# whwu95/MVFNet

Hardware: AMD Instinct MI355X
Metric: clips/sec (fwd+bwd) MVFNet-R50 8x8 224^2 (higher is better)
Workload: dtype bf16; 1 GPU; MVFNet-ResNet50 8x8, 32 clips/GPU of 8x3x224x224, bf16, train step: fwd (batch-stat BN) + loss + bwd + clip + SGD-nesterov; all through the HIP C ABI (stem + 16 bottlenecks + MVF + TSN head); clips_per_gpu=32, frames_per_clip=8, parallelism=dp1: replicas, one flat gradient all-reduce per step

## Files before the change

include/mvfnet_hip.h:

```cpp
#ifndef MVFNET_HIP_H
#define MVFNET_HIP_H

#include <stddef.h>
#include <stdint.h>

#ifdef __cplusplus
extern "C" {
#endif

#define MVF_ABI_VERSION 2

enum { MVF_OK = 0, MVF_EINVAL = -1, MVF_ESHAPE = -2, MVF_EWS = -3, MVF_EHIP = -4, MVF_EUNSUPPORTED = -5 };
enum { MVF_F32 = 0, MVF_BF16 = 1 };
enum { MVF_NCHW = 0, MVF_NHWC = 1 };
enum { MVF_VIEW_T = 1, MVF_VIEW_H = 2, MVF_VIEW_W = 4 };

int mvf_abi_version(void);
const char* mvf_last_error(void);

typedef struct {
    int32_t nt, c, h, w;
    int32_t n_segment;
    int32_t cs;
    int32_t mode;
// ... 54 lines not shown
                                   size_t ws_bytes, void* stream);
int mvf_conv2d_nhwc_fwd_bnbwd_apply(const mvf_conv_desc_t* d, const void* x, const void* x2, const void* w_packed, const void* g,
                                    const unsigned char* sign_bits, const float* bn_gamma, const float* bn_mean, const float* bn_invstd,
                                    const float* dgamma, const float* dbeta, void* dz, void* ws, size_t ws_bytes, void* stream);
int mvf_conv2d_nhwc_fwd_resmask(const mvf_conv_desc_t* d, const void* x, const void* x2, const void* w_packed,
                                const float* bias, const void* residual, const unsigned char* res_sign_bits, void* y,
                                void* ws, size_t ws_bytes, void* stream);
int mvf_conv2d_nhwc_fwd_resmask_gate(const mvf_conv_desc_t* d, const void* x, const void* x2, const void* w_packed, const float* bias,
                                     const void* residual, const unsigned char* res_sign_bits, const unsigned char* out_gate_bits, void* y,
                                     void* ws, size_t ws_bytes, void* stream);
int mvf_conv2d_nhwc_fwd_resmask_gate_colsums(const mvf_conv_desc_t* d, const void* x, const void* x2, const void* w_packed, const void* residual,
                                             const unsigned char* res_sign_bits, const unsigned char* out_gate_bits, void* y, float* sums_part, void* ws,
                                             size_t ws_bytes, void* stream);
int mvf_conv2d_nhwc_dgrad_bnsums(const mvf_conv_desc_t* d, const void* dz, const void* w_packed_dgrad, void* y, const void* bn_z,
                                 const float* bn_mean, const float* bn_invstd, const float* bn_scale, const float* bn_shift,
                                 float* sums_part, void* ws, size_t ws_bytes, void* stream);
int mvf_bn_bwd_finalize(const float* sums_part, int nblk, int c, float* dgamma, float* dbeta, void* stream);
int mvf_conv2d_stats_rows(const mvf_conv_desc_t* d);
int mvf_conv2d_nhwc_fwd_stats(const mvf_conv_desc_t* d, const void* x, const void* x2, const void* w_packed, void* y,
                              float* stats_part, const float* stats_shift, void* ws, size_t ws_bytes, void* stream);

enum {
    MVF_CONV_FAM_NONE = 0,
    MVF_CONV_FAM_REG = 1,
    MVF_CONV_FAM_X3 = 2,
    MVF_CONV_FAM_LDS_DMA = 3,
    MVF_CONV_FAM_T256_2B = 4,
    MVF_CONV_FAM_T256_P4 = 5,
    MVF_CONV_FAM_DBUF = 6,
    MVF_CONV_FAM_DBUF_PF2 = 7,
    MVF_CONV_FAM_STREAMK = 8,
    MVF_CONV_FAM_GENERIC = 9,
    MVF_CONV_FAM_MVF_LOADER = 10,
    MVF_CONV_FAM_STEM_DIRECT = 11,
    MVF_CONV_FAM_PW_SUMS = 12,
    MVF_CONV_FAM_C3X3_C64 = 13
};
typedef struct {
    int32_t family;
    int32_t epi_asked;
    int32_t epi_run;
    int32_t pointwise;
    int32_t buffers;
    int32_t tile_m, tile_n;
    int32_t dtype;
    int32_t k_chunks;
    int32_t half_k;
    int32_t launches;
} mvf_conv_launch_info_t;
int mvf_conv2d_last_launch(mvf_conv_launch_info_t* out);

int mvf_pack_conv_weight(const float* w_oihw, int cout, int cin, int kh, int kw, int kw_pad, int cin_pad,
                         const float* scale, void* w_packed, int dtype, void* stream);
int mvf_bn_fold(const float* gamma, const float* beta, const float* mean, const float* var, float eps, int c,
                float* scale, float* shift, void* stream);

int mvf_stem_prep(const float* x_nchw, int n, int c, int h, int w, int pad, int wp, void* out, int dtype, void* stream);

int mvf_frames_prep_u8(const unsigned char* frames_hwc, int n, int hs, int ws, const int* window, int h, int w,
                       const float* mean3, const float* std3, int to_rgb, int div_255, int pad, int wp, void* out_stem,
                       float* out_nchw, int dtype, void* stream);
int mvf_frames_resample_u8(const unsigned char* frames_hwc, int n, int hs, int ws, const int* rows, int h, int w,
                           const float* mean3, const float* std3, int to_rgb, int div_255, int pad, int wp, void* out_stem,
                           float* out_nchw, int dtype, void* stream);
int mvf_frames_resample_color_u8(const unsigned char* frames_hwc, int n, int hs, int ws, const int* rows, const float* color, int h, int w,
                                 const float* mean3, const float* std3, int to_rgb, int div_255, int pad, int wp, void* out_stem,
                                 float* out_nchw, int dtype, void* stream);
int mvf_frames_gather_resample_u8(const unsigned char* frames_hwc, int n_src, int hs, int ws, const int* src_index, int n_out, const int* rows,
                                  const float* color, int h, int w, const float* mean3, const float* std3, int to_rgb, int div_255, int pad,
                                  int wp, void* out_stem, float* out_nchw, int dtype, void* stream);
int mvf_frames_yuv420_gather_resample_u8(const unsigned char* frames, int n_src, int hs, int ws, int pitch, int layout, int standard, int order,
                                         const int* src_index, int n_out, const int* rows, const float* color, int h, int w, const float* mean3,
                                         const float* std3, int to_rgb, int div_255, int pad, int wp, void* out_stem, float* out_nchw, int dtype,
                                         void* stream);
int mvf_frames_addressed_resample_u8(const unsigned char* frames, long long frames_bytes, int format, int standard, int order,
                                     int n_out, const int* rows, const int* addr, const float* color, int h, int w,
                                     const float* mean3, const float* std3, int to_rgb, int div_255, int pad, int wp,
                                     void* out_stem, float* out_nchw, int dtype, void* stream);

int mvf_maxpool3x3s2_nhwc(const void* x, int n, int h, int w, int c, void* y, int dtype, void* stream);

int mvf_head_pool_fc(const void* feat, int clips, int t, int hw, int c, const float* fc_w, const float* fc_b,
                     int classes, float* pooled_ws, float* scores, int dtype, void* stream);
int mvf_average_clip(const float* scores, int clips, int classes, int kind, float* out, void* stream);

int mvf_conv2d_nhwc_dgrad_bnsums_split(const mvf_conv_desc_t* d, const void* x, const void* x2, const void* w_packed, const float* bias, void* y,
                                       const void* bn_z, const float* bn_mean, const float* bn_invstd, const float* bn_scale, const float* bn_shift,
                                       float* sums_part, void* ws, size_t ws_bytes, void* stream);
int mvf_bn_bwd_dzfree_prep(const void* w_packed_dgrad, int c, int k, const float* gamma, const float* mean, const float* invstd, const float* dgamma,
                           const float* dbeta, long m, void* w_out, float* bias_out, int dtype, void* stream);
int mvf_bn_bwd_dzfree_wgrad(float* dw, const void* w_packed, const float* gram, const float* a_mean, const float* gamma, const float* mean,
                            const float* invstd, const float* dgamma, const float* dbeta, long m, int c, int k, int dtype, void* stream);
int mvf_bn_bwd_dzfree_sums(const float* q, const void* w_packed, int c, int k, const float* mean, const float* invstd, const float* part_lo, int rows_lo,
                           int c_split, const float* part_hi, int rows_hi, float* dgamma, float* dbeta, int dtype, void* stream);
size_t mvf_bn_workspace_bytes(long m, int c);
int mvf_bn_train_stats(const void* z, long m, int c, const float* gamma, const float* beta, float eps, float momentum,
                       float* running_mean, float* running_var, float* save_mean, float* save_invstd, float* scale,
                       float* shift, void* ws, size_t ws_bytes, int dtype, void* stream);
int mvf_bn_train_finalize(const float* part, int nblk, long m, int c, const float* gamma, const float* beta, float eps,
                          float momentum, float* running_mean, float* running_var, float* save_mean, float* save_invstd,
                          float* scale, float* shift, void* stream);
int mvf_bn_train_stats_gram(const float* gram, const float* a_mean, const void* w_packed, long m, int c, int k, const float* gamma, const float* beta,
                            float eps, float momentum, float* running_mean, float* running_var, float* save_mean, float* save_invstd, float* scale,
                            float* shift, int dtype, void* stream);
int mvf_bn_apply_colmeans(const void* z, long m, int c, const float* scale, const float* shift, int act, void* out, float* mean_out, void* ws,
                          size_t ws_bytes, int dtype, void* stream);
int mvf_bn_apply(const void* z, long m, int c, const float* scale, const float* shift, const void* residual,
                 const float* rscale, const float* rshift, int act, void* out, int dtype, void* stream);
int mvf_bn_bwd_reduce(const void* g, int g_pitch, const void* z, const void* ymask, long m, int c, const float* mean,
                      const float* invstd, const float* scale, const float* shift, int mask_mode, void* gm_out,
                      float* dgamma, float* dbeta, void* ws, size_t ws_bytes, int dtype, void* stream);
int mvf_bn_bwd_apply(const void* g, int g_pitch, const void* z, long m, int c, const float* gamma, const float* mean,
                     const float* invstd, const float* scale, const float* shift, const float* dgamma,
                     const float* dbeta, int mask_mode, void* dz, int dtype, void* stream);
int mvf_bn_apply_bits(const void* z, long m, int c, const float* scale, const float* shift, const void* residual,
                      const float* rscale, const float* rshift, int relu, void* out, unsigned char* sign_bits, int dtype,
                      void* stream);
int mvf_bn_bwd_apply_masked(const void* g, int g_pitch, const void* z, const void* ymask, long m, int c, const float* gamma,
                            const float* mean, const float* invstd, const float* scale, const float* shift,
                            const float* dgamma, const float* dbeta, int mask_mode, void* dz, int dtype, void* stream);
int mvf_bn_bwd_pair(const void* g, int g_pitch, const void* z_a, const void* z_b, const unsigned char* sign_bits, long m, int c,
                    const float* gamma_a, const float* mean_a, const float* invstd_a, float* dgamma_a, float* dbeta_a,
                    const float* gamma_b, const float* mean_b, const float* invstd_b, float* dgamma_b, float* dbeta_b,
                    void* dz_a, void* dz_b, void* ws, size_t ws_bytes, int dtype, void* stream);
int mvf_bn_bwd_wgrad_splits(long m, int c, int k, int nbn, int mask_mode);
size_t mvf_bn_bwd_wgrad_slab_bytes(long m, int c, int k, int nbn, int mask_mode);
int mvf_bn_bwd_apply_wgrad(const void* g, int g_pitch, const void* z, const void* ymask, long m, int c, const float* gamma, const float* mean,
                           const float* invstd, const float* scale, const float* shift, const float* dgamma, const float* dbeta, int mask_mode,
                           void* dz, const void* x, int x_pitch, int k, float* slabs, size_t slab_bytes, int dtype, void* stream);
int mvf_bn_bwd_pair_wgrad(const void* g, int g_pitch, const void* z_a, const void* z_b, const unsigned char* sign_bits, long m, int c,
                          const float* gamma_a, const float* mean_a, const float* invstd_a, float* dgamma_a, float* dbeta_a,
                          const float* gamma_b, const float* mean_b, const float* invstd_b, float* dgamma_b, float* dbeta_b,
                          void* dz_a, void* dz_b, const void* x_a, int xa_pitch, const void* x_b, int xb_pitch, int k,
                          float* slabs_a, float* slabs_b, size_t slab_bytes, void* ws, size_t ws_bytes, int dtype, void* stream);
int mvf_conv1x1_bwd_fused_splits(long m, int c, int k);
int mvf_conv1x1_bwd_fused(const void* a_in, int a_pitch, const void* w_packed, const void* g, int g_pitch, const unsigned char* sign_bits, long m, int c,
                          int k, const float* gamma, const float* mean, const float* invstd, const float* dgamma, const float* dbeta, const void* z_in,
                          const float* in_mean, const float* in_invstd, const float* in_scale, const float* in_shift, void* dx, float* sums_part,
                          int sums_rows, float* slabs, size_t slab_bytes, int dtype, void* stream);
int mvf_conv1x1_bnbwd_sums_pair(const void* a_in, int a_pitch, const void* w_a, const void* x_in, int x_pitch, const void* w_b, const void* g, int g_pitch,
                                const unsigned char* sign_bits, long m, int c, int k, const float* mean_a, const float* invstd_a, const float* mean_b,
                                const float* invstd_b, float* part_a, float* part_b, int rows, int dtype, void* stream);
int mvf_wgrad_slab_reduce(const float* slabs, int nsplit, int cout, int k, float* dw_oihw, void* stream);
int mvf_maxpool_bn_relu_fwd(const void* z, int n, int h, int w, int c, const float* scale, const float* shift, void* y,
                            unsigned char* argmax, int dtype, void* stream);
int mvf_maxpool_bn_relu_bwd(const unsigned char* argmax, const void* g, int n, int h, int w, int c, void* ga, int dtype,
                            void* stream);
int mvf_maxpool_bwd_sums_rows(int n, int h);
int mvf_maxpool_bn_relu_bwd_apply(const unsigned char* argmax, const void* g, int n, int h, int w, int c, const void* z, const float* gamma,
                                  const float* mean, const float* invstd, const float* scale, const float* shift, const float* dgamma,
                                  const float* dbeta, void* dz, int dtype, void* stream);
int mvf_maxpool_bn_relu_bwd_sums(const unsigned char* argmax, const void* g, int n, int h, int w, int c, void* ga, const void* z, const float* mean,
                                 const float* invstd, const float* scale, const float* shift, float* sums_part, int dtype, void* stream);
int mvf_head_train_fwd(const void* feat, int clips, int t, int hw, int c, const float* fc_w, const float* fc_b, int classes,
                       const long long* labels, const float* drop_mask ,
                       float* pooled, float* scores, float* dscores, float* loss_part, float* loss, int dtype, void* stream);
int mvf_ce_loss(const float* scores, const long long* labels, int clips, int classes, float* dscores, float* loss_part, float* loss,
                void* stream);
int mvf_head_train_bwd(const float* dscores, const float* pooled, const float* fc_w, const float* drop_mask, int clips, int t,
                       int hw, int c, int classes, float* dfc_w, float* dfc_b, float* dpool_ws , void* dfeat, int dtype,
                       void* stream);
int mvf_stem_blend(const void* xp, int clips, int t, int hp, int wp, int pad, const int* rows, const float* wts, void* out, int dtype, void* stream);
int mvf_soft_targets(const long long* labels, const int* rows, const float* wts, int clips, int classes, float eps, float* targets, void* stream);
int mvf_ce_loss_soft(const float* scores, const float* targets, int clips, int classes, float* dscores, float* loss_part, float* loss, void* stream);
int mvf_head_train_fwd_soft(const void* feat, int clips, int t, int hw, int c, const float* fc_w, const float* fc_b, int classes,
                            const float* targets, const float* drop_mask ,
                            float* pooled, float* scores, float* dscores, float* loss_part, float* loss, int dtype, void* stream);
int mvf_distill_loss(const float* scores, const float* teacher_scores, int clips, int classes, float temperature, float alpha,
                     float* dscores , float* loss_part , float* loss , float* terms ,
                     void* stream);
int mvf_stem_erase(void* xp, int planes, int hp, int wp, int pad, const int* boxes, int max_boxes, const float* fill, const unsigned int* key, int dtype,
                   void* stream);
#define MVF_RANDAUG_WS_PER_FRAME (3 * 256 + 16)
int mvf_frames_randaug_u8(const unsigned char* frames_hwc, int n, int hs, int ws, int t, int order, const int* sizes, const int* table, int layers,
                          unsigned stats_layers, unsigned char* out, unsigned char* tmp, void* workspace, long long workspace_bytes, void* stream);
size_t mvf_conv2d_wgrad_workspace_bytes(const mvf_conv_desc_t* d);
int mvf_conv2d_nhwc_wgrad(const mvf_conv_desc_t* d, const void* dz, const void* x, const void* x2, int kw_real,
                          int cin_real, int kw_packed, int cin_packed, float* dw_oihw, void* ws, size_t ws_bytes,
                          void* stream);
int mvf_conv2d_nhwc_wgrad_wgs(const mvf_conv_desc_t* d, const void* dz, const void* x, const void* x2, int kw_real,
                              int cin_real, int kw_packed, int cin_packed, float* dw_oihw, void* ws, size_t ws_bytes, int wgs, void* stream);
enum {
    MVF_WGRAD_FAM_NONE = 0,
    MVF_WGRAD_FAM_F32_REG = 1,
    MVF_WGRAD_FAM_F32_DMA = 2,
    MVF_WGRAD_FAM_X3 = 3,
    MVF_WGRAD_FAM_BF16_WIDEN = 4,
    MVF_WGRAD_FAM_BF16_REG = 5,
    MVF_WGRAD_FAM_BF16_DMA2 = 6,
    MVF_WGRAD_FAM_BF16_PIPE = 7,
    MVF_WGRAD_FAM_T256_2B = 8,
    MVF_WGRAD_FAM_T256_P4 = 9,
    MVF_WGRAD_FAM_C3X3_C64 = 10,
    MVF_WGRAD_FAM_STEM = 11
};
typedef struct {
    int32_t family;
    int32_t stages;
    int32_t tile_co, tile_k;
    int32_t dtype;
    int32_t nsplit;
    int32_t rows_per_split;
    int32_t xcd_rr;
    int32_t split_operand;
    int32_t gram;
    int32_t wgs_target;
    int32_t launches;
} mvf_wgrad_launch_info_t;
int mvf_conv2d_wgrad_last_launch(mvf_wgrad_launch_info_t* out);
typedef struct {
    const float* w;
    void* out;
    int cout, cin, kh, kw, kw_pad, cin_pad;
    int kind, first_block;
} mvf_pack_job_t;
int mvf_pack_conv_weights_batched(const mvf_pack_job_t* jobs_dev, int njobs, int total_blocks, int dtype, void* stream);

int mvf_pack_conv_weight_dgrad(const float* w_oihw, int cout, int cin, int kh, int kw, void* w_packed, int dtype,
                               void* stream);
int mvf_nhwc_stencil(const mvf_desc_t* d, const void* x, int x_c, void* out, int out_c, const float* w_t,
                     const float* w_h, const float* w_w, const float* scale, const float* shift, int flip,
                     const void* addend, int addend_c, const unsigned char* addend_sign_bits, void* stream);
int mvf_nhwc_stencil_gate(const mvf_desc_t* d, const void* x, int x_c, void* out, int out_c, const float* w_t,
                          const float* w_h, const float* w_w, const float* scale, const float* shift, int flip,
                          const void* addend, int addend_c, const unsigned char* addend_sign_bits,
                          const unsigned char* out_gate_bits, void* stream);
int mvf_nhwc_stencil_gate_colsums(const mvf_desc_t* d, const void* x, int x_c, void* out, int out_c, const float* w_t, const float* w_h,
                                  const float* w_w, int flip, const void* addend, int addend_c, const unsigned char* addend_sign_bits,
                                  const unsigned char* out_gate_bits, float* sums_part, void* stream);
int mvf_nhwc_stencil_stats_rows(const mvf_desc_t* d, int x_c, int out_c);
int mvf_nhwc_stencil_tile_plan(const mvf_desc_t* d, int x_c, int out_c, int* rows_per_band, int* chan_per_wg);
int mvf_nhwc_stencil_stats(const mvf_desc_t* d, const void* x, int x_c, void* out, int out_c, const float* w_t, const float* w_h,
                           const float* w_w, float* stats_part, const float* stats_shift, void* stream);
size_t mvf_nhwc_tapgrad_workspace_bytes(const mvf_desc_t* d);
int mvf_nhwc_tapgrad(const mvf_desc_t* d, const void* x, int x_c, const void* dy, int dy_c, float* dw_t, float* dw_h,
                     float* dw_w, void* ws, size_t ws_bytes, void* stream);
size_t mvf_sgd_workspace_bytes(long n);
int mvf_sgd_nesterov_step(float* params, const float* grads, float* momentum_buf, long n, float grad_scale, float max_norm,
                          float lr, float momentum, float weight_decay, int first_step, float* norm_out, void* ws,
                          size_t ws_bytes, void* stream);
typedef struct mvf_sgd_segment {
    long long first;
    float lr_mult, decay_mult;
} mvf_sgd_segment_t;
int mvf_sgd_step_segments(float* params, const float* grads, float* momentum_buf, long n, float grad_scale, float max_norm, float lr,
                          float momentum, float weight_decay, int first_step, int nesterov, const mvf_sgd_segment_t* segments, int nseg,
                          float* norm_out, void* ws, size_t ws_bytes, void* stream);
int mvf_grad_accumulate(float* acc, const float* g, long n, int first, void* stream);
int mvf_sgd_nesterov_step_ema(float* params, const float* grads, float* momentum_buf, long n, float grad_scale, float max_norm, float lr, float momentum,
                              float weight_decay, int first_step, float* ema, float ema_momentum, float* norm_out, void* ws, size_t ws_bytes, void* stream);
int mvf_sgd_step_segments_ema(float* params, const float* grads, float* momentum_buf, long n, float grad_scale, float max_norm, float lr, float momentum,
                              float weight_decay, int first_step, int nesterov, const mvf_sgd_segment_t* segments, int nseg, float* ema, float ema_momentum,
                              float* norm_out, void* ws, size_t ws_bytes, void* stream);
int mvf_ema_update(float* ema, const float* params, long n, float momentum, void* stream);
int mvf_ema_swap(float* a, float* b, long n, void* stream);
typedef struct mvf_stat_segment {
    float* ptr;
    long first;
} mvf_stat_segment_t;
int mvf_bn_stats_accumulate(const mvf_stat_segment_t* seg, int nseg, long n, double* acc, void* stream);
int mvf_bn_stats_finalize(const mvf_stat_segment_t* seg, int nseg, long n, const double* acc, long count, float* dst_flat_or_null, void* stream);
int mvf_bn_stats_exchange(const mvf_stat_segment_t* seg, int nseg, long n, float* flat, int mode, void* stream);
int mvf_sgd_step_guarded(float* params, const float* grads, float* momentum_buf, long n, float grad_scale, float max_norm, float lr, float momentum,
                         float weight_decay, int first_step, int nesterov, const mvf_sgd_segment_t* segments, int nseg, float* ema, float ema_momentum,
                         int* guard, float* norm_out, void* ws, size_t ws_bytes, void* stream);
int mvf_bn_stats_snapshot(const mvf_stat_segment_t* seg, int nseg, long n, float* flat, const long long* counters, long ncount, long long* counters_copy,
                          void* stream);
int mvf_bn_stats_restore(const mvf_stat_segment_t* seg, int nseg, long n, const float* flat, long long* counters, long ncount,
                         const long long* counters_copy, const int* guard, void* stream);
typedef struct mvf_adamw_hyper {
    double lr, beta1, beta2, eps, weight_decay;
    int decoupled;
} mvf_adamw_hyper_t;
size_t mvf_adamw_workspace_bytes(long n);
int mvf_adamw_step(float* params, const float* grads, float* exp_avg, float* exp_avg_sq, long n, float grad_scale, float max_norm,
                   const mvf_adamw_hyper_t* hyper, const mvf_sgd_segment_t* segments, int nseg, float* ema, float ema_momentum, int* guard,
                   long long* applied_steps, float* norm_out, void* ws, size_t ws_bytes, void* stream);
enum { MVF_METRICS_ROWS = 0, MVF_METRICS_BAD_LABEL = 1, MVF_METRICS_NAN_ROWS = 2, MVF_METRICS_HITS = 8, MVF_METRICS_MAX_K = 8, MVF_METRICS_CONFUSION = 16 };
size_t mvf_metrics_state_words(int classes, int with_confusion);
int mvf_metrics_update(const float* scores, int rows, int classes, const long long* labels, const int* ks, int nk, long long* state, int with_confusion,
                       int* rank_out, int* pred_out, void* stream);
typedef struct mvf_flat_stats {
    double sumsq;
    double absmax;
    long long n_nan;
    long long n_inf;
} mvf_flat_stats_t;
size_t mvf_flat_stats_workspace_bytes(long n, int nseg);
int mvf_flat_segment_stats(const float* x, const float* y_or_null, long n, const long long* first, int nseg, mvf_flat_stats_t* out, const int* guard_or_null,
                           long long* step_out_or_null, void* ws, size_t ws_bytes, void* stream);
int mvf_bn_stats_nonfinite(const mvf_stat_segment_t* seg, int nseg, long n, long long* counts, const int* guard_or_null, void* stream);

enum { MVF_PLAN_CALL = 0, MVF_PLAN_RECORD = 1, MVF_PLAN_WAIT = 2 };
typedef struct mvf_plan_op {
    int kind, n_int, n_flt, reserved;
    void* fn;
    long long word0, float0;
} mvf_plan_op_t;
int mvf_plan_run(const mvf_plan_op_t* ops, int n_ops, const unsigned long long* words, const float* floats, int* failed_op);

#ifdef __cplusplus
}
#endif
#endif
```

mvfnet_amd/_lib.py:

```python
import ctypes as C
import os

import torch

_HERE = os.path.dirname(os.path.abspath(__file__))
LIB_PATH = os.environ.get("MVF_LIB_PATH") or os.path.join(_HERE, "libmvfnet_hip.so")

MVF_F32, MVF_BF16 = 0, 1
MVF_NCHW, MVF_NHWC = 0, 1
VIEW_T, VIEW_H, VIEW_W = 1, 2, 4
MODE_BITS = {"T": 1, "TH": 3, "THW": 7}
METRICS_ROWS, METRICS_BAD_LABEL, METRICS_NAN_ROWS, METRICS_HITS, METRICS_MAX_K, METRICS_CONFUSION = 0, 1, 2, 8, 8, 16
ERRNAMES = {-1: "MVF_EINVAL", -2: "MVF_ESHAPE", -3: "MVF_EWS", -4: "MVF_EHIP", -5: "MVF_EUNSUPPORTED"}


class MvfDesc(C.Structure):
    _fields_ = [("nt", C.c_int32), ("c", C.c_int32), ("h", C.c_int32), ("w", C.c_int32), ("n_segment", C.c_int32),
                ("cs", C.c_int32), ("mode", C.c_int32), ("layout", C.c_int32), ("dtype", C.c_int32)]


class ConvDesc(C.Structure):
    _fields_ = [("n", C.c_int32), ("h", C.c_int32), ("w", C.c_int32), ("cin", C.c_int32), ("cout", C.c_int32),
                ("kh", C.c_int32), ("kw", C.c_int32), ("stride", C.c_int32), ("pad", C.c_int32),
                ("ho", C.c_int32), ("wo", C.c_int32), ("x_pix_stride", C.c_int32),
# ... 28 lines not shown

class PlanOp(C.Structure):
    _fields_ = [("kind", C.c_int32), ("n_int", C.c_int32), ("n_flt", C.c_int32), ("reserved", C.c_int32), ("fn", C.c_void_p), ("word0", C.c_longlong),
                ("float0", C.c_longlong)]


class SgdSegment(C.Structure):
    _fields_ = [("first", C.c_int64), ("lr_mult", C.c_float), ("decay_mult", C.c_float)]


class AdamwHyper(C.Structure):
    _fields_ = [("lr", C.c_double), ("beta1", C.c_double), ("beta2", C.c_double), ("eps", C.c_double), ("weight_decay", C.c_double), ("decoupled", C.c_int32)]


class StatSegment(C.Structure):
    _fields_ = [("ptr", C.c_void_p), ("first", C.c_long)]


def _load():
    if not os.path.exists(LIB_PATH):
        raise ImportError(
            "mvfnet_amd: %s not found. Build it with `python -m mvfnet_amd.build` (needs hipcc, "
            "--offload-arch=gfx950). There is no CPU or PyTorch fallback for the hot path." % LIB_PATH)
    lib = C.CDLL(LIB_PATH)
    vp, fp, sz, i32, f32 = C.c_void_p, C.c_void_p, C.c_size_t, C.c_int, C.c_float
    dp = C.POINTER(MvfDesc)
    lib.mvf_abi_version.restype = i32
    lib.mvf_abi_version.argtypes = []
    lib.mvf_last_error.restype = C.c_char_p
    lib.mvf_last_error.argtypes = []
    lib.mvf_fwd_infer.restype = i32
    lib.mvf_fwd_infer.argtypes = [dp, vp, vp, fp, fp, fp, fp, fp, vp]
    lib.mvf_fwd_train_workspace_bytes.restype = sz
    lib.mvf_fwd_train_workspace_bytes.argtypes = [dp]
    lib.mvf_fwd_train.restype = i32
    lib.mvf_fwd_train.argtypes = [dp, vp, vp, fp, fp, fp, fp, fp, f32, f32, fp, fp, fp, fp, vp, sz, vp]
    lib.mvf_bwd_workspace_bytes.restype = sz
    lib.mvf_bwd_workspace_bytes.argtypes = [dp]
    lib.mvf_bwd.restype = i32
    lib.mvf_bwd.argtypes = [dp, vp, vp, fp, fp, fp, fp, fp, fp, fp, i32, vp, fp, fp, fp, fp, fp, vp, sz, vp]
    lib.mvf_fwd_infer_slice.restype = i32
    lib.mvf_fwd_infer_slice.argtypes = [dp, vp, vp, fp, fp, fp, fp, fp, vp]
    cp = C.POINTER(ConvDesc)
    lib.mvf_conv2d_nhwc_fwd.restype = i32
    lib.mvf_conv2d_nhwc_fwd.argtypes = [cp, vp, vp, vp, fp, vp, vp, vp]
    lib.mvf_conv2d_workspace_bytes.restype = sz
    lib.mvf_conv2d_workspace_bytes.argtypes = [cp]
    lib.mvf_conv2d_nhwc_fwd_ws.restype = i32
    lib.mvf_conv2d_nhwc_fwd_ws.argtypes = [cp, vp, vp, vp, fp, vp, vp, vp, sz, vp]
    lib.mvf_conv2d_nhwc_dgrad_bnsums.restype = i32
    lib.mvf_conv2d_nhwc_dgrad_bnsums.argtypes = [cp, vp, vp, vp, vp, fp, fp, fp, fp, fp, vp, sz, vp]
    lib.mvf_bn_bwd_finalize.restype = i32
    lib.mvf_bn_bwd_finalize.argtypes = [fp, i32, i32, fp, fp, vp]
    lib.mvf_conv2d_nhwc_fwd_bnapply.restype = i32
    lib.mvf_conv2d_nhwc_fwd_bnapply.argtypes = [cp, vp, vp, vp, fp, fp, vp, fp, fp, vp, vp, vp, sz, vp]
    lib.mvf_conv2d_nhwc_fwd_bnbwd_sums.restype = i32
    lib.mvf_conv2d_nhwc_fwd_bnbwd_sums.argtypes = [cp, vp, vp, vp, vp, vp, fp, fp, fp, vp, sz, vp]
    lib.mvf_conv2d_nhwc_fwd_bnbwd_apply.restype = i32
    lib.mvf_conv2d_nhwc_fwd_bnbwd_apply.argtypes = [cp, vp, vp, vp, vp, vp, fp, fp, fp, fp, fp, vp, vp, sz, vp]
    lib.mvf_conv2d_nhwc_fwd_resmask.restype = i32
    lib.mvf_conv2d_nhwc_fwd_resmask.argtypes = [cp, vp, vp, vp, fp, vp, vp, vp, vp, sz, vp]
    i64_ = C.c_long
    lib.mvf_conv2d_nhwc_fwd_resmask_gate.restype = i32
    lib.mvf_conv2d_nhwc_fwd_resmask_gate.argtypes = [cp, vp, vp, vp, fp, vp, vp, vp, vp, vp, sz, vp]
    lib.mvf_conv2d_nhwc_fwd_resmask_gate_colsums.restype = i32
    lib.mvf_conv2d_nhwc_fwd_resmask_gate_colsums.argtypes = [cp, vp, vp, vp, vp, vp, vp, vp, fp, vp, sz, vp]
    lib.mvf_nhwc_stencil_gate_colsums.restype = i32
    lib.mvf_nhwc_stencil_gate_colsums.argtypes = [dp, vp, i32, vp, i32, fp, fp, fp, i32, vp, i32, vp, vp, fp, vp]
    lib.mvf_conv2d_nhwc_dgrad_bnsums_split.restype = i32
    lib.mvf_conv2d_nhwc_dgrad_bnsums_split.argtypes = [cp, vp, vp, vp, fp, vp, vp, fp, fp, fp, fp, fp, vp, sz, vp]
    lib.mvf_bn_bwd_dzfree_prep.restype = i32
    lib.mvf_bn_bwd_dzfree_prep.argtypes = [vp, i32, i32, fp, fp, fp, fp, fp, i64_, vp, fp, i32, vp]
    lib.mvf_bn_bwd_dzfree_wgrad.restype = i32
    lib.mvf_bn_bwd_dzfree_wgrad.argtypes = [fp, vp, fp, fp, fp, fp, fp, fp, fp, i64_, i32, i32, i32, vp]
    lib.mvf_bn_bwd_dzfree_sums.restype = i32
    lib.mvf_bn_bwd_dzfree_sums.argtypes = [fp, vp, i32, i32, fp, fp, fp, i32, i32, fp, i32, fp, fp, i32, vp]
    lib.mvf_nhwc_stencil_stats_rows.restype = i32
    lib.mvf_nhwc_stencil_stats_rows.argtypes = [dp, i32, i32]
    lib.mvf_nhwc_stencil_tile_plan.restype = i32
    lib.mvf_nhwc_stencil_tile_plan.argtypes = [dp, i32, i32, C.POINTER(C.c_int), C.POINTER(C.c_int)]
    lib.mvf_nhwc_stencil_stats.restype = i32
    lib.mvf_nhwc_stencil_stats.argtypes = [dp, vp, i32, vp, i32, fp, fp, fp, fp, fp, vp]
    lib.mvf_nhwc_stencil_gate.restype = i32
    lib.mvf_nhwc_stencil_gate.argtypes = [dp, vp, i32, vp, i32, fp, fp, fp, fp, fp, i32, vp, i32, vp, vp, vp]
    lib.mvf_conv2d_stats_rows.restype = i32
    lib.mvf_conv2d_stats_rows.argtypes = [cp]
    lib.mvf_conv2d_nhwc_fwd_stats.restype = i32
    lib.mvf_conv2d_nhwc_fwd_stats.argtypes = [cp, vp, vp, vp, vp, fp, fp, vp, sz, vp]
    lib.mvf_conv2d_last_launch.restype = i32
    lib.mvf_conv2d_last_launch.argtypes = [C.POINTER(ConvLaunchInfo)]
    lib.mvf_pack_conv_weight.restype = i32
    lib.mvf_pack_conv_weight.argtypes = [fp, i32, i32, i32, i32, i32, i32, fp, vp, i32, vp]
    lib.mvf_pack_conv_weights_batched.restype = i32
    lib.mvf_pack_conv_weights_batched.argtypes = [vp, i32, i32, i32, vp]
    lib.mvf_bn_fold.restype = i32
    lib.mvf_bn_fold.argtypes = [fp, fp, fp, fp, f32, i32, fp, fp, vp]
    lib.mvf_stem_prep.restype = i32
    lib.mvf_stem_prep.argtypes = [fp, i32, i32, i32, i32, i32, i32, vp, i32, vp]
    lib.mvf_frames_prep_u8.restype = i32
    lib.mvf_frames_prep_u8.argtypes = [vp, i32, i32, i32, vp, i32, i32, C.POINTER(C.c_float), C.POINTER(C.c_float),
                                       i32, i32, i32, i32, vp, vp, i32, vp]
    lib.mvf_frames_resample_u8.restype = i32
    lib.mvf_frames_resample_u8.argtypes = [vp, i32, i32, i32, vp, i32, i32, C.POINTER(C.c_float), C.POINTER(C.c_float),
                                           i32, i32, i32, i32, vp, vp, i32, vp]
    lib.mvf_frames_resample_color_u8.restype = i32
    lib.mvf_frames_resample_color_u8.argtypes = [vp, i32, i32, i32, vp, vp, i32, i32, C.POINTER(C.c_float), C.POINTER(C.c_float),
                                                 i32, i32, i32, i32, vp, vp, i32, vp]
    lib.mvf_frames_gather_resample_u8.restype = i32
    lib.mvf_frames_gather_resample_u8.argtypes = [vp, i32, i32, i32, vp, i32, vp, vp, i32, i32, C.POINTER(C.c_float), C.POINTER(C.c_float),
                                                  i32, i32, i32, i32, vp, vp, i32, vp]
    lib.mvf_frames_yuv420_gather_resample_u8.restype = i32
    lib.mvf_frames_yuv420_gather_resample_u8.argtypes = [vp, i32, i32, i32, i32, i32, i32, i32, vp, i32, vp, vp, i32, i32, C.POINTER(C.c_float),
                                                         C.POINTER(C.c_float), i32, i32, i32, i32, vp, vp, i32, vp]
    lib.mvf_frames_addressed_resample_u8.restype = i32
    lib.mvf_frames_addressed_resample_u8.argtypes = [vp, C.c_longlong, i32, i32, i32, i32, vp, vp, vp, i32, i32, C.POINTER(C.c_float), C.POINTER(C.c_float),
                                                     i32, i32, i32, i32, vp, vp, i32, vp]
    lib.mvf_maxpool3x3s2_nhwc.restype = i32
    lib.mvf_maxpool3x3s2_nhwc.argtypes = [vp, i32, i32, i32, i32, vp, i32, vp]
    lib.mvf_head_pool_fc.restype = i32
    lib.mvf_head_pool_fc.argtypes = [vp, i32, i32, i32, i32, fp, fp, i32, fp, fp, i32, vp]
    lib.mvf_average_clip.restype = i32
    lib.mvf_average_clip.argtypes = [fp, i32, i32, i32, fp, vp]
    i64, ll = C.c_long, C.c_void_p
    lib.mvf_bn_workspace_bytes.restype = sz
    lib.mvf_bn_workspace_bytes.argtypes = [i64, i32]
    lib.mvf_bn_train_stats.restype = i32
    lib.mvf_bn_train_stats.argtypes = [vp, i64, i32, fp, fp, f32, f32, fp, fp, fp, fp, fp, fp, vp, sz, i32, vp]
    lib.mvf_bn_train_finalize.restype = i32
    lib.mvf_bn_train_finalize.argtypes = [fp, i32, i64, i32, fp, fp, f32, f32, fp, fp, fp, fp, fp, fp, vp]
    lib.mvf_bn_train_stats_gram.restype = i32
    lib.mvf_bn_train_stats_gram.argtypes = [fp, fp, vp, i64, i32, i32, fp, fp, f32, f32, fp, fp, fp, fp, fp, fp, i32, vp]
    lib.mvf_bn_apply_colmeans.restype = i32
    lib.mvf_bn_apply_colmeans.argtypes = [vp, i64, i32, fp, fp, i32, vp, fp, vp, sz, i32, vp]
    lib.mvf_bn_apply.restype = i32
    lib.mvf_bn_apply.argtypes = [vp, i64, i32, fp, fp, vp, fp, fp, i32, vp, i32, vp]
    lib.mvf_bn_apply_bits.restype = i32
    lib.mvf_bn_apply_bits.argtypes = [vp, i64, i32, fp, fp, vp, fp, fp, i32, vp, vp, i32, vp]
    lib.mvf_bn_bwd_apply_masked.restype = i32
    lib.mvf_bn_bwd_apply_masked.argtypes = [vp, i32, vp, vp, i64, i32, fp, fp, fp, fp, fp, fp, fp, i32, vp, i32, vp]
    lib.mvf_bn_bwd_reduce.restype = i32
    lib.mvf_bn_bwd_reduce.argtypes = [vp, i32, vp, vp, i64, i32, fp, fp, fp, fp, i32, vp, fp, fp, vp, sz, i32, vp]
    lib.mvf_bn_bwd_apply.restype = i32
    lib.mvf_bn_bwd_apply.argtypes = [vp, i32, vp, i64, i32, fp, fp, fp, fp, fp, fp, fp, i32, vp, i32, vp]
    lib.mvf_maxpool_bn_relu_fwd.restype = i32
    lib.mvf_maxpool_bn_relu_fwd.argtypes = [vp, i32, i32, i32, i32, fp, fp, vp, vp, i32, vp]
    lib.mvf_maxpool_bn_relu_bwd.restype = i32
    lib.mvf_maxpool_bn_relu_bwd.argtypes = [vp, vp, i32, i32, i32, i32, vp, i32, vp]
    lib.mvf_maxpool_bwd_sums_rows.restype = i32
    lib.mvf_maxpool_bwd_sums_rows.argtypes = [i32, i32]
    lib.mvf_maxpool_bn_relu_bwd_apply.restype = i32
    lib.mvf_maxpool_bn_relu_bwd_apply.argtypes = [vp, vp, i32, i32, i32, i32, vp, fp, fp, fp, fp, fp, fp, fp, vp, i32, vp]
    lib.mvf_maxpool_bn_relu_bwd_sums.restype = i32
    lib.mvf_maxpool_bn_relu_bwd_sums.argtypes = [vp, vp, i32, i32, i32, i32, vp, vp, fp, fp, fp, fp, fp, i32, vp]
    lib.mvf_head_train_fwd.restype = i32
    lib.mvf_head_train_fwd.argtypes = [vp, i32, i32, i32, i32, fp, fp, i32, ll, fp, fp, fp, fp, fp, fp, i32, vp]
    lib.mvf_conv2d_nhwc_fwd_mvf.restype = i32
    lib.mvf_conv2d_nhwc_fwd_mvf.argtypes = [cp, vp, vp, fp, fp, i32, i32, i32, vp, vp, sz, vp]
    lib.mvf_bn_bwd_pair.restype = i32
    lib.mvf_bn_bwd_pair.argtypes = [vp, i32, vp, vp, vp, i64, i32, fp, fp, fp, fp, fp, fp, fp, fp, fp, fp, vp, vp, vp, sz, i32, vp]
    lib.mvf_bn_bwd_wgrad_splits.restype = i32
    lib.mvf_bn_bwd_wgrad_splits.argtypes = [i64, i32, i32, i32, i32]
    lib.mvf_bn_bwd_wgrad_slab_bytes.restype = sz
    lib.mvf_bn_bwd_wgrad_slab_bytes.argtypes = [i64, i32, i32, i32, i32]
    lib.mvf_bn_bwd_apply_wgrad.restype = i32
    lib.mvf_bn_bwd_apply_wgrad.argtypes = [vp, i32, vp, vp, i64, i32, fp, fp, fp, fp, fp, fp, fp, i32, vp, vp, i32, i32, fp, sz, i32, vp]
    lib.mvf_bn_bwd_pair_wgrad.restype = i32
    lib.mvf_bn_bwd_pair_wgrad.argtypes = [vp, i32, vp, vp, vp, i64, i32, fp, fp, fp, fp, fp, fp, fp, fp, fp, fp, vp, vp, vp, i32, vp, i32, i32,
                                          fp, fp, sz, vp, sz, i32, vp]
    lib.mvf_conv1x1_bwd_fused_splits.restype = i32
    lib.mvf_conv1x1_bwd_fused_splits.argtypes = [i64, i32, i32]
    lib.mvf_conv1x1_bwd_fused.restype = i32
    lib.mvf_conv1x1_bwd_fused.argtypes = [vp, i32, vp, vp, i32, vp, i64, i32, i32, fp, fp, fp, fp, fp, vp, fp, fp, fp, fp, vp, fp, i32, fp, sz, i32, vp]
    lib.mvf_conv1x1_bnbwd_sums_pair.restype = i32
    lib.mvf_conv1x1_bnbwd_sums_pair.argtypes = [vp, i32, vp, vp, i32, vp, vp, i32, vp, i64, i32, i32, fp, fp, fp, fp, fp, fp, i32, i32, vp]
    lib.mvf_wgrad_slab_reduce.restype = i32
    lib.mvf_wgrad_slab_reduce.argtypes = [fp, i32, i32, i32, fp, vp]
    lib.mvf_ce_loss.restype = i32
    lib.mvf_ce_loss.argtypes = [fp, ll, i32, i32, fp, fp, fp, vp]
    lib.mvf_stem_blend.restype = i32
    lib.mvf_stem_blend.argtypes = [vp, i32, i32, i32, i32, i32, vp, fp, vp, i32, vp]
    lib.mvf_stem_erase.restype = i32
    lib.mvf_stem_erase.argtypes = [vp, i32, i32, i32, i32, vp, i32, fp, vp, i32, vp]
    lib.mvf_frames_randaug_u8.restype = i32
    lib.mvf_frames_randaug_u8.argtypes = [vp, i32, i32, i32, i32, i32, vp, vp, i32, C.c_uint, vp, vp, vp, C.c_longlong, vp]
    lib.mvf_soft_targets.restype = i32
    lib.mvf_soft_targets.argtypes = [ll, vp, fp, i32, i32, f32, fp, vp]
    lib.mvf_ce_loss_soft.restype = i32
    lib.mvf_ce_loss_soft.argtypes = [fp, fp, i32, i32, fp, fp, fp, vp]
    lib.mvf_head_train_fwd_soft.restype = i32
    lib.mvf_head_train_fwd_soft.argtypes = [vp, i32, i32, i32, i32, fp, fp, i32, fp, fp, fp, fp, fp, fp, fp, i32, vp]
    lib.mvf_distill_loss.restype = i32
    lib.mvf_distill_loss.argtypes = [fp, fp, i32, i32, f32, f32, fp, fp, fp, fp, vp]
    lib.mvf_head_train_bwd.restype = i32
    lib.mvf_head_train_bwd.argtypes = [fp, fp, fp, fp, i32, i32, i32, i32, i32, fp, fp, fp, vp, i32, vp]
    lib.mvf_conv2d_wgrad_workspace_bytes.restype = sz
    lib.mvf_conv2d_wgrad_workspace_bytes.argtypes = [cp]
    lib.mvf_conv2d_nhwc_wgrad.restype = i32
    lib.mvf_conv2d_nhwc_wgrad.argtypes = [cp, vp, vp, vp, i32, i32, i32, i32, fp, vp, sz, vp]
    lib.mvf_conv2d_nhwc_wgrad_wgs.restype = i32
    lib.mvf_conv2d_nhwc_wgrad_wgs.argtypes = [cp, vp, vp, vp, i32, i32, i32, i32, fp, vp, sz, i32, vp]
    lib.mvf_conv2d_wgrad_last_launch.restype = i32
    lib.mvf_conv2d_wgrad_last_launch.argtypes = [C.POINTER(WgradLaunchInfo)]
    lib.mvf_pack_conv_weight_dgrad.restype = i32
    lib.mvf_pack_conv_weight_dgrad.argtypes = [fp, i32, i32, i32, i32, vp, i32, vp]
    lib.mvf_nhwc_stencil.restype = i32
    lib.mvf_nhwc_stencil.argtypes = [dp, vp, i32, vp, i32, fp, fp, fp, fp, fp, i32, vp, i32, vp, vp]
    lib.mvf_nhwc_tapgrad_workspace_bytes.restype = sz
    lib.mvf_nhwc_tapgrad_workspace_bytes.argtypes = [dp]
    lib.mvf_nhwc_tapgrad.restype = i32
    lib.mvf_nhwc_tapgrad.argtypes = [dp, vp, i32, vp, i32, fp, fp, fp, vp, sz, vp]
    lib.mvf_sgd_workspace_bytes.restype = sz
    lib.mvf_sgd_workspace_bytes.argtypes = [i64]
    lib.mvf_sgd_nesterov_step.restype = i32
    lib.mvf_sgd_nesterov_step.argtypes = [fp, fp, fp, i64, f32, f32, f32, f32, f32, i32, fp, vp, sz, vp]
    lib.mvf_sgd_step_segments.restype = i32
    lib.mvf_sgd_step_segments.argtypes = [fp, fp, fp, i64, f32, f32, f32, f32, f32, i32, i32, vp, i32, fp, vp, sz, vp]
    lib.mvf_grad_accumulate.restype = i32
    lib.mvf_grad_accumulate.argtypes = [fp, fp, i64, i32, vp]
    lib.mvf_sgd_nesterov_step_ema.restype = i32
    lib.mvf_sgd_nesterov_step_ema.argtypes = [fp, fp, fp, i64, f32, f32, f32, f32, f32, i32, fp, f32, fp, vp, sz, vp]
    lib.mvf_sgd_step_segments_ema.restype = i32
    lib.mvf_sgd_step_segments_ema.argtypes = [fp, fp, fp, i64, f32, f32, f32, f32, f32, i32, i32, vp, i32, fp, f32, fp, vp, sz, vp]
    lib.mvf_ema_update.restype = i32
    lib.mvf_ema_update.argtypes = [fp, fp, i64, f32, vp]
    lib.mvf_ema_swap.restype = i32
    lib.mvf_ema_swap.argtypes = [fp, fp, i64, vp]
    lib.mvf_bn_stats_accumulate.restype = i32
    lib.mvf_bn_stats_accumulate.argtypes = [vp, i32, i64, vp, vp]
    lib.mvf_bn_stats_finalize.restype = i32
    lib.mvf_bn_stats_finalize.argtypes = [vp, i32, i64, vp, i64, fp, vp]
    lib.mvf_bn_stats_exchange.restype = i32
    lib.mvf_bn_stats_exchange.argtypes = [vp, i32, i64, fp, i32, vp]
    lib.mvf_sgd_step_guarded.restype = i32
    lib.mvf_sgd_step_guarded.argtypes = [fp, fp, fp, i64, f32, f32, f32, f32, f32, i32, i32, vp, i32, fp, f32, vp, fp, vp, sz, vp]
    lib.mvf_bn_stats_snapshot.restype = i32
    lib.mvf_bn_stats_snapshot.argtypes = [vp, i32, i64, fp, vp, i64, vp, vp]
    lib.mvf_bn_stats_restore.restype = i32
    lib.mvf_bn_stats_restore.argtypes = [vp, i32, i64, fp, vp, i64, vp, vp, vp]
    lib.mvf_adamw_workspace_bytes.restype = sz
    lib.mvf_adamw_workspace_bytes.argtypes = [i64]
    lib.mvf_adamw_step.restype = i32
    lib.mvf_adamw_step.argtypes = [fp, fp, fp, fp, i64, f32, f32, C.POINTER(AdamwHyper), vp, i32, fp, f32, vp, vp, fp, vp, sz, vp]
    lib.mvf_metrics_state_words.restype = sz
    lib.mvf_metrics_state_words.argtypes = [i32, i32]
    lib.mvf_metrics_update.restype = i32
    lib.mvf_metrics_update.argtypes = [fp, i32, i32, ll, vp, i32, ll, i32, vp, vp, vp]
    lib.mvf_flat_stats_workspace_bytes.restype = sz
    lib.mvf_flat_stats_workspace_bytes.argtypes = [i64, i32]
    lib.mvf_flat_segment_stats.restype = i32
    lib.mvf_flat_segment_stats.argtypes = [fp, fp, i64, vp, i32, vp, vp, vp, vp, sz, vp]
    lib.mvf_bn_stats_nonfinite.restype = i32
    lib.mvf_bn_stats_nonfinite.argtypes = [vp, i32, i64, vp, vp, vp]
    lib.mvf_plan_run.restype = i32
    lib.mvf_plan_run.argtypes = [C.POINTER(PlanOp), i32, C.POINTER(C.c_ulonglong), C.POINTER(C.c_float), C.POINTER(C.c_int)]
    missing = [n for n in declared_symbols() if hasattr(lib, n) and getattr(lib, n).argtypes is None]
    if missing:
        raise ImportError("mvfnet_amd._lib: no argtypes declared for %s" % missing)
    return lib


def check(rc, what=""):
    if rc != 0:
        msg = lib.mvf_last_error().decode("utf-8", "replace")
        raise RuntimeError("%s failed: %s (%s)" % (what or "libmvfnet_hip", ERRNAMES.get(rc, rc), msg))


def declared_symbols():
    import re
    hdr = os.path.join(os.path.dirname(_HERE), "include", "mvfnet_hip.h")
    txt = open(hdr).read()
    txt = re.sub(r"/\*.*?\*/", "", txt, flags=re.S)
    return sorted(set(re.findall(r"\b((?:mvf|mvfnet)_[a-z0-9_]+)\s*\(", txt)))


lib = _load()
```

mvfnet_amd/csrc/common.h:

```cpp
#pragma once
#include <hip/hip_runtime.h>
#include <stdlib.h>
#include <string.h>
#include <strings.h>
#include <stdint.h>
#include <stdio.h>

#include "mvfnet_hip.h"

void mvf_set_error(const char* fmt, ...);

#define MVF_HIP_OK(call)                                                                        \
    do {                                                                                        \
        hipError_t e__ = (call);                                                                \
        if (e__ != hipSuccess) {                                                                \
            mvf_set_error("%s:%d: %s -> %s", __FILE__, __LINE__, #call, hipGetErrorString(e__)); \
            return MVF_EHIP;                                                                    \
        }                                                                                       \
    } while (0)

#define MVF_REQUIRE(cond, code, ...)    \
    do {                                \
        if (!(cond)) {                  \
            mvf_set_error(__VA_ARGS__); \
            return (code);              \
        }                               \
    } while (0)

#define MVF_LAUNCH_CHECK()                                                              \
    do {                                                                                \
        hipError_t e__ = hipGetLastError();                                             \
        if (e__ != hipSuccess) {                                                        \
            mvf_set_error("%s:%d: launch -> %s", __FILE__, __LINE__, hipGetErrorString(e__)); \
            return MVF_EHIP;                                                            \
        }                                                                               \
    } while (0)

struct bf16_t {
    uint16_t v;
};

__device__ __forceinline__ float bf16_to_f32(uint16_t v) { return __uint_as_float(((uint32_t)v) << 16); }
typedef __bf16 mvf_bf16x2 __attribute__((ext_vector_type(2)));
typedef float mvf_f32x2 __attribute__((ext_vector_type(2)));
__device__ __forceinline__ uint32_t pack_bf16x2(float lo, float hi) {
    const mvf_f32x2 v = {lo, hi};
    const mvf_bf16x2 b = __builtin_convertvector(v, mvf_bf16x2);
    uint32_t u;
    __builtin_memcpy(&u, &b, 4);
    return u;
}
__device__ __forceinline__ uint16_t f32_to_bf16(float f) { return (uint16_t)(pack_bf16x2(f, 0.f) & 0xffffu); }

__device__ __forceinline__ float ldf(const float* p) { return *p; }
__device__ __forceinline__ float ldf(const bf16_t* p) { return bf16_to_f32(p->v); }
__device__ __forceinline__ void stf(float* p, float v) { *p = v; }
__device__ __forceinline__ void stf(bf16_t* p, float v) { p->v = f32_to_bf16(v); }

__device__ __forceinline__ float4 ld4(const float* p) { return *reinterpret_cast<const float4*>(p); }
__device__ __forceinline__ float4 ld4(const bf16_t* p) {
    uint2 r = *reinterpret_cast<const uint2*>(p);
    return make_float4(__uint_as_float(r.x << 16), __uint_as_float(r.x & 0xffff0000u),
                       __uint_as_float(r.y << 16), __uint_as_float(r.y & 0xffff0000u));
}
__device__ __forceinline__ void st4(float* p, float4 v) { *reinterpret_cast<float4*>(p) = v; }
__device__ __forceinline__ void st4(bf16_t* p, float4 v) {
    uint2 r;
    r.x = pack_bf16x2(v.x, v.y);
    r.y = pack_bf16x2(v.z, v.w);
    *reinterpret_cast<uint2*>(p) = r;
}

__device__ __forceinline__ float ema_step(float e, float p, float m) { return m >= 1.0f ? p : fmaf(m, p - e, e); }

__device__ __forceinline__ float hswish_f(float u) { return u * fminf(fmaxf(u + 3.0f, 0.0f), 6.0f) * (1.0f / 6.0f); }
__device__ __forceinline__ float hswish_grad_f(float u) {
    float r6 = fminf(fmaxf(u + 3.0f, 0.0f), 6.0f);
    float inner = (u > -3.0f && u < 3.0f) ? 1.0f : 0.0f;
    return r6 * (1.0f / 6.0f) + u * inner * (1.0f / 6.0f);
}

static inline size_t align_up(size_t v, size_t a) { return (v + a - 1) / a * a; }

static inline bool mvf_policy_lookup(const char* name, long* out) {
    const char* p = getenv("MVF_POLICY");
    if (!p) return false;
    const size_t n = strlen(name);
    while (*p) {
        while (*p == ',' || *p == ';' || *p == ' ') ++p;
        const char* e = p;
        while (*e && *e != ',' && *e != ';') ++e;
        const char* eq = (const char*)memchr(p, '=', (size_t)(e - p));
        if (eq && (size_t)(eq - p) == n && strncasecmp(p, name, n) == 0) {
            *out = strtol(eq + 1, nullptr, 10);
            return true;
        }
        p = e;
    }
    return false;
}
static inline int mvf_policy_int(const char* name, int dflt) {
    long v;
    return mvf_policy_lookup(name, &v) ? (int)v : dflt;
}
static inline bool mvf_policy_has(const char* name) {
    long v;
    return mvf_policy_lookup(name, &v);
}

struct StemDirectArgs {
    const void* x;
    const void* w;
    void* y;
    const float* bias;
    float* stats_part;
    const float* stats_shift;
    int stats_rows, epi;
    int N, H, W, Ho, Wo;
    long wK;
};
struct Conv3x3C64Args {
    const void* x;
    const void* w;
    void* y;
    const float* bias;
    float* stats_part;
    const float* stats_shift;
    const void* bn_z;
    const float *bn_mean, *bn_invstd, *bn_scale, *bn_shift;
    int stats_rows, epi;
    int N, H, W, xps;
    long wK;
};
struct PwSumsArgs {
    const void* a;
    const void* w;
    const void* g;
    const unsigned char* bits;
    const float* c0;
    const float* c1;
    float* part;
    int rows, mode, M, N, K, xps;
};
struct Wgrad3x3C64Args {
    const void* dz;
    const void* x;
    float* part;
    int N, H, W, xps, nwg;
};
struct WgradStemArgs {
    const void* dz;
    const void* x;
    float* part;
    int N, H, W, Ho, Wo, nwg;
};
namespace mvf_internal {
struct BnBwdWgradArgs {
    const void* g;
    const void* z[2];
    const void* bits;
    const float *gamma[2], *mean[2], *invstd[2], *dgamma[2], *dbeta[2];
    const float *scale, *shift;
    void* dz[2];
    const void* x[2];
    int xps[2];
    float* part[2];
    int g_pitch, M, C, K;
    int rows_per_split, nsplit, ctiles, ktiles;
};
struct PwBwdFusedArgs {
    const void* a;
    const void* w;
    const void* g;
    const unsigned char* bits;
    const float *gamma, *mean, *invstd, *dgamma, *dbeta;
    const void* z_in;
    const float *in_scale, *in_shift, *in_mean, *in_invstd;
    void* dx;
    float* sums_part;
    float* part;
    int aps, g_pitch, M, sums_rows, rows_per_split, nsplit;
    int ablate;
};
struct PwSumsPairArgs {
    const void *a, *x;
    const void *w_a, *w_b;
    const void* g;
    const unsigned char* bits;
    const float *mean_a, *invstd_a, *mean_b, *invstd_b;
    float *part_a, *part_b;
    int aps, xps, g_pitch, M, rows, rows_per_split, nsplit;
};
int pw_sums_pair_launch(const PwSumsPairArgs& a, hipStream_t st);
int pw_bwd_fused_plan(long m, int c, int k, int* rows_per_split);
int pw_bwd_fused_launch(const PwBwdFusedArgs& a, hipStream_t st);
bool bnbwd_wgrad_tile(int c, int k, int nbn, int mask_mode, int* ct, int* kt);
int bnbwd_wgrad_plan(long m, int c, int k, int nbn, int mask_mode, int* rows_per_split, int* ctiles, int* ktiles);
int bnbwd_wgrad_launch(const BnBwdWgradArgs& a, int nbn, int mask_mode, hipStream_t st);
int wgrad_slab_reduce_launch(const float* part, int nsplit, int cout, int k, float* dw_oihw, hipStream_t st);
bool wgrad3x3_c64_ok(int n, int h, int w, int xps);
int wgrad3x3_c64_wgs(int n, int h);
int wgrad3x3_c64_launch(const Wgrad3x3C64Args& a, hipStream_t st);
bool wgrad_stem_ok(int n, int h, int w, int ho, int wo);
int wgrad_stem_wgs(int n, int ho);
int wgrad_stem_launch(const WgradStemArgs& a, hipStream_t st);
int stem_direct_launch(const StemDirectArgs& a, hipStream_t st);
int conv3x3_c64_launch(const Conv3x3C64Args& a, hipStream_t st);
int pw_sums_launch(const PwSumsArgs& a, hipStream_t st);
}

#ifdef __HIPCC__
typedef int i32x4 __attribute__((ext_vector_type(4)));
__device__ __forceinline__ i32x4 rsrc_words(const void* base, unsigned nbytes) {
    const unsigned long p = (unsigned long)base;
    i32x4 r;
    r.x = __builtin_amdgcn_readfirstlane((int)(unsigned)p);
    r.y = __builtin_amdgcn_readfirstlane((int)((unsigned)(p >> 32) & 0xffffu));
    r.z = __builtin_amdgcn_readfirstlane((int)nbytes);
    r.w = 0x00020000;
    return r;
}
__device__ __forceinline__ void glds16(const i32x4 rs, const unsigned lds_dst, const unsigned voff) {
    unsigned keep;
    asm volatile("s_mov_b32 %0, m0\n\ts_mov_b32 m0, %2\n\ts_nop 0\n\tbuffer_load_dwordx4 %1, %3, 0 offen lds\n\ts_mov_b32 m0, %0"
                 : "=&s"(keep) : "v"(voff), "s"(lds_dst), "s"(rs) : "memory");
}

#endif
```

mvfnet_amd/csrc/train_ops.hip:

```cpp
#include <algorithm>
#include <math.h>
#include <stdlib.h>

#include "common.h"

namespace {

constexpr int kThreads = 256;

struct ColPlan {
    int cqb;
    int rl;
    int gx;
    int gy;
    int rows;
};

ColPlan col_plan(long M, int C, int vn = 4, int blocks = 2048) {
    ColPlan p;
    const int cq = C / vn;
    int cqb = 1;
    while (cqb < cq && cqb < 64) cqb <<= 1;
    p.cqb = cqb;
    p.rl = kThreads / cqb;
// ... 566 lines not shown
    const float inv_m = 1.0f / (float)M;
    float aa[VN], da[VN], ka[VN], mua[VN], ab[VN], db_[VN], kb[VN], mub[VN];
    {
        float ga[VN], rs[VN], dg[VN], db[VN];
        ldp<VN>(gamma_a, c, ga); ldp<VN>(invstd_a, c, rs); ldp<VN>(dgamma_a, c, dg); ldp<VN>(dbeta_a, c, db); ldp<VN>(mean_a, c, mua);
#pragma unroll
        for (int j = 0; j < VN; ++j) { aa[j] = ga[j] * rs[j]; da[j] = db[j] * inv_m; ka[j] = rs[j] * dg[j] * inv_m; }
        ldp<VN>(gamma_b, c, ga); ldp<VN>(invstd_b, c, rs); ldp<VN>(dgamma_b, c, dg); ldp<VN>(dbeta_b, c, db); ldp<VN>(mean_b, c, mub);
#pragma unroll
        for (int j = 0; j < VN; ++j) { ab[j] = ga[j] * rs[j]; db_[j] = db[j] * inv_m; kb[j] = rs[j] * dg[j] * inv_m; }
    }
    const long r0 = (long)blockIdx.y * rows, r1 = min(M, r0 + rows);
    auto one = [&](long row, float (&gv)[VN], const float (&zav)[VN], const float (&zbv)[VN]) {
        bn_mask<ET, VN>(gv, zav, zav, mua, mua, 4, ld_maskbits<VN>(bits, row, C, c));
        float oa[VN], ob[VN];
#pragma unroll
        for (int j = 0; j < VN; ++j) {
            oa[j] = aa[j] * (gv[j] - da[j] - (zav[j] - mua[j]) * ka[j]);
            ob[j] = ab[j] * (gv[j] - db_[j] - (zbv[j] - mub[j]) * kb[j]);
        }
        stv<ET, VN>(dza + row * C + c, oa);
        stv<ET, VN>(dzb + row * C + c, ob);
    };
    long row = r0 + lane_r;
    for (; row + rl < r1; row += 2 * rl) {
        float g0[VN], g1[VN], x0[VN], x1[VN], y0[VN], y1[VN];
        ldv<ET, VN>(g + row * g_pitch + c, g0);
        ldv<ET, VN>(g + (row + rl) * g_pitch + c, g1);
        ldv<ET, VN>(za + row * C + c, x0);
        ldv<ET, VN>(za + (row + rl) * C + c, x1);
        ldv<ET, VN>(zb + row * C + c, y0);
        ldv<ET, VN>(zb + (row + rl) * C + c, y1);
        one(row, g0, x0, y0);
        one(row + rl, g1, x1, y1);
    }
    for (; row < r1; row += rl) {
        float g0[VN], x0[VN], y0[VN];
        ldv<ET, VN>(g + row * g_pitch + c, g0);
        ldv<ET, VN>(za + row * C + c, x0);
        ldv<ET, VN>(zb + row * C + c, y0);
        one(row, g0, x0, y0);
    }
}

template <typename ET>
__global__ void maxpool_bn_fwd_kernel(const ET* z, int n, int h, int w, int c, int ho, int wo, const float* scale,
                                      const float* shift, ET* y, unsigned char* amax) {
    const int c4 = c >> 2;
    const long total = (long)n * ho * wo * c4;
    for (long i = (long)blockIdx.x * blockDim.x + threadIdx.x; i < total; i += (long)gridDim.x * blockDim.x) {
        int cq, ow, oh, img;
        if (total <= 0x7fffffffL) {
            unsigned t = (unsigned)i;
            cq = (int)(t % (unsigned)c4); t /= (unsigned)c4;
            ow = (int)(t % (unsigned)wo); t /= (unsigned)wo;
            oh = (int)(t % (unsigned)ho);
            img = (int)(t / (unsigned)ho);
        } else {
            cq = (int)(i % c4);
            long t = i / c4;
            ow = (int)(t % wo); t /= wo;
            oh = (int)(t % ho);
            img = (int)(t / ho);
        }
        const float4 s = *reinterpret_cast<const float4*>(scale + cq * 4), b = *reinterpret_cast<const float4*>(shift + cq * 4);
        float4 m = make_float4(-INFINITY, -INFINITY, -INFINITY, -INFINITY);
        unsigned am[4] = {0, 0, 0, 0};
        float4 win[9];
#pragma unroll
        for (int k = 0; k < 9; ++k) {
            const int ih = oh * 2 - 1 + k / 3, iw = ow * 2 - 1 + k % 3;
            const int ihc = min(max(ih, 0), h - 1), iwc = min(max(iw, 0), w - 1);
            win[k] = ld4(z + (((long)img * h + ihc) * w + iwc) * c + cq * 4);
        }
#pragma unroll
        for (int k = 0; k < 9; ++k) {
            const int ih = oh * 2 - 1 + k / 3, iw = ow * 2 - 1 + k % 3;
            const bool in = (unsigned)ih < (unsigned)h && (unsigned)iw < (unsigned)w;
            float4 v = win[k];
            v.x = fmaxf(v.x * s.x + b.x, 0.f); v.y = fmaxf(v.y * s.y + b.y, 0.f);
            v.z = fmaxf(v.z * s.z + b.z, 0.f); v.w = fmaxf(v.w * s.w + b.w, 0.f);
            if (in && v.x > m.x) { m.x = v.x; am[0] = k; }
            if (in && v.y > m.y) { m.y = v.y; am[1] = k; }
            if (in && v.z > m.z) { m.z = v.z; am[2] = k; }
            if (in && v.w > m.w) { m.w = v.w; am[3] = k; }
        }
        const long oidx = (((long)img * ho + oh) * wo + ow) * c + cq * 4;
        st4(y + oidx, m);
        if (amax) *reinterpret_cast<unsigned*>(amax + oidx) = am[0] | (am[1] << 8) | (am[2] << 16) | (am[3] << 24);
    }
}

template <typename ET>
__global__ __launch_bounds__(256) void maxpool_bn_fwd_blk_kernel(const ET* z, int n, int h, int w, int c, int ho, int wo, const float* scale,
                                                                 const float* shift, ET* y, unsigned char* amax) {
    constexpr int VC = 16 / (int)sizeof(ET);
    const int ncg = c / VC, bwn = wo >> 1, bhn = ho >> 1;
    const long total = (long)n * bhn * bwn * ncg;
    for (long i = (long)blockIdx.x * blockDim.x + threadIdx.x; i < total; i += (long)gridDim.x * blockDim.x) {
        const int cq = (int)(i % ncg);
        long t = i / ncg;
        const int bw = (int)(t % bwn); t /= bwn;
        const int bh = (int)(t % bhn);
        const int img = (int)(t / bhn);
        float sc[VC], sh[VC];
#pragma unroll
        for (int j = 0; j < VC; ++j) { sc[j] = scale[cq * VC + j]; sh[j] = shift[cq * VC + j]; }
        float a[5][5][VC];
#pragma unroll
        for (int r = 0; r < 5; ++r)
#pragma unroll
            for (int q = 0; q < 5; ++q) {
                const int ih = 4 * bh - 1 + r, iw = 4 * bw - 1 + q;
                const int ihc = min(max(ih, 0), h - 1), iwc = min(max(iw, 0), w - 1);
                const uint4 u = *reinterpret_cast<const uint4*>(z + (((long)img * h + ihc) * w + iwc) * c + cq * VC);
                float f[VC];
                if constexpr (sizeof(ET) == 4) {
                    f[0] = __uint_as_float(u.x); f[1] = __uint_as_float(u.y); f[2] = __uint_as_float(u.z); f[3] = __uint_as_float(u.w);
                } else {
                    f[0] = __uint_as_float(u.x << 16); f[1] = __uint_as_float(u.x & 0xffff0000u); f[2] = __uint_as_float(u.y << 16); f[3] = __uint_as_float(u.y & 0xffff0000u);
                    f[4] = __uint_as_float(u.z << 16); f[5] = __uint_as_float(u.z & 0xffff0000u); f[6] = __uint_as_float(u.w << 16); f[7] = __uint_as_float(u.w & 0xffff0000u);
                }
#pragma unroll
                for (int j = 0; j < VC; ++j) a[r][q][j] = fmaxf(f[j] * sc[j] + sh[j], 0.f);
            }
#pragma unroll
        for (int p = 0; p < 4; ++p) {
            const int oh = 2 * bh + (p >> 1), ow = 2 * bw + (p & 1);
            float m[VC];
            unsigned am[VC];
#pragma unroll
            for (int j = 0; j < VC; ++j) { m[j] = -INFINITY; am[j] = 0; }
#pragma unroll
            for (int k = 0; k < 9; ++k) {
                const int r = 2 * (p >> 1) + k / 3, q = 2 * (p & 1) + k % 3;
                const int ih = oh * 2 - 1 + k / 3, iw = ow * 2 - 1 + k % 3;
                const bool in = (unsigned)ih < (unsigned)h && (unsigned)iw < (unsigned)w;
#pragma unroll
                for (int j = 0; j < VC; ++j)
                    if (in && a[r][q][j] > m[j]) { m[j] = a[r][q][j]; am[j] = k; }
            }
            const long oidx = (((long)img * ho + oh) * wo + ow) * c + cq * VC;
            uint4 u;
            if constexpr (sizeof(ET) == 4) u = make_uint4(__float_as_uint(m[0]), __float_as_uint(m[1]), __float_as_uint(m[2]), __float_as_uint(m[3]));
            else u = make_uint4(pack_bf16x2(m[0], m[1]), pack_bf16x2(m[2], m[3]), pack_bf16x2(m[4], m[5]), pack_bf16x2(m[6], m[7]));
            *reinterpret_cast<uint4*>(y + oidx) = u;
            if (amax) {
                if constexpr (VC == 8)
                    *reinterpret_cast<uint2*>(amax + oidx) = make_uint2(am[0] | (am[1] << 8) | (am[2] << 16) | (am[3] << 24), am[4] | (am[5] << 8) | (am[6] << 16) | (am[7] << 24));
                else
                    *reinterpret_cast<unsigned*>(amax + oidx) = am[0] | (am[1] << 8) | (am[2] << 16) | (am[3] << 24);
            }
        }
    }
}

template <typename ET>
__global__ void maxpool_bn_bwd_rows_kernel(const unsigned char* amax, const ET* g, int n, int h, int w, int c, int ho, int wo, ET* ga) {
    const int c4 = c >> 2;
    const int row = blockIdx.x, img = row / h, ih = row - img * h;
    const int per = w * c4;
    for (int i = threadIdx.x; i < per; i += blockDim.x) {
        const int iw = i / c4, cq = i - iw * c4;
        float acc[4] = {0.f, 0.f, 0.f, 0.f};
        unsigned amv[4];
        float4 gvv[4];
        bool okv[4];
        unsigned mev[4];
#pragma unroll
        for (int k = 0; k < 4; ++k) {
            const int oh = (ih + (k >> 1)) >> 1, ow = (iw + (k & 1)) >> 1;
            okv[k] = oh < ho && ow < wo && ((k >> 1) == 0 || (ih & 1)) && ((k & 1) == 0 || (iw & 1));
            const int ohc = min(oh, ho - 1), owc = min(ow, wo - 1);
            mev[k] = (unsigned)(ih - (oh * 2 - 1)) * 3u + (unsigned)(iw - (ow * 2 - 1));
            const long oidx = (((long)img * ho + ohc) * wo + owc) * c + cq * 4;
            amv[k] = *reinterpret_cast<const unsigned*>(amax + oidx);
            gvv[k] = ld4(g + oidx);
        }
#pragma unroll
        for (int k = 0; k < 4; ++k) {
            const unsigned am = amv[k], me = mev[k];
            if (okv[k] && (am & 255u) == me) acc[0] += gvv[k].x;
            if (okv[k] && ((am >> 8) & 255u) == me) acc[1] += gvv[k].y;
            if (okv[k] && ((am >> 16) & 255u) == me) acc[2] += gvv[k].z;
            if (okv[k] && (am >> 24) == me) acc[3] += gvv[k].w;
        }
        st4(ga + ((long)row * w + iw) * c + cq * 4, make_float4(acc[0], acc[1], acc[2], acc[3]));
    }
}

constexpr int kPoolRB = 8;
template <typename ET>
__global__ __launch_bounds__(256) void maxpool_bn_bwd_rows_sums_kernel(const unsigned char* amax, const ET* g, int n, int h, int w, int c, int ho, int wo, ET* ga,
                                                                       const ET* z, const float* mean, const float* invstd, const float* scale, const float* shift,
                                                                       float* part, int nblk) {
    __shared__ float red[256 * 8];
    const int c4 = c >> 2;
    const int per = w * c4;
    const int cq = threadIdx.x % c4;
    const float4 sc = *reinterpret_cast<const float4*>(scale + cq * 4), sh = *reinterpret_cast<const float4*>(shift + cq * 4);
    const float4 mu = *reinterpret_cast<const float4*>(mean + cq * 4), rs = *reinterpret_cast<const float4*>(invstd + cq * 4);
    float s1[4] = {0.f, 0.f, 0.f, 0.f}, s2[4] = {0.f, 0.f, 0.f, 0.f};
    const int row_end = min(n * h, ((int)blockIdx.x + 1) * kPoolRB);
    for (int row = blockIdx.x * kPoolRB; row < row_end; ++row) {
        const int img = row / h, ih = row - img * h;
        for (int i = threadIdx.x; i < per; i += 256) {
            const int iw = i / c4;
            float acc[4] = {0.f, 0.f, 0.f, 0.f};
            unsigned amv[4];
            float4 gvv[4];
            bool okv[4];
            unsigned mev[4];
            const long zi = ((long)row * w + iw) * c + cq * 4;
            const float4 zv = ld4(z + zi);
#pragma unroll
            for (int k = 0; k < 4; ++k) {
                const int oh = (ih + (k >> 1)) >> 1, ow = (iw + (k & 1)) >> 1;
                okv[k] = oh < ho && ow < wo && ((k >> 1) == 0 || (ih & 1)) && ((k & 1) == 0 || (iw & 1));
                const int ohc = min(oh, ho - 1), owc = min(ow, wo - 1);
                mev[k] = (unsigned)(ih - (oh * 2 - 1)) * 3u + (unsigned)(iw - (ow * 2 - 1));
                const long oidx = (((long)img * ho + ohc) * wo + owc) * c + cq * 4;
                amv[k] = *reinterpret_cast<const unsigned*>(amax + oidx);
                gvv[k] = ld4(g + oidx);
            }
#pragma unroll
            for (int k = 0; k < 4; ++k) {
                const unsigned am = amv[k], me = mev[k];
                if (okv[k] && (am & 255u) == me) acc[0] += gvv[k].x;
                if (okv[k] && ((am >> 8) & 255u) == me) acc[1] += gvv[k].y;
                if (okv[k] && ((am >> 16) & 255u) == me) acc[2] += gvv[k].z;
                if (okv[k] && (am >> 24) == me) acc[3] += gvv[k].w;
            }
            if (ga) st4(ga + zi, make_float4(acc[0], acc[1], acc[2], acc[3]));
            if constexpr (sizeof(ET) == 2) {
#pragma unroll
                for (int j = 0; j < 4; ++j) acc[j] = bf16_to_f32(f32_to_bf16(acc[j]));
            }
            const float zz[4] = {zv.x, zv.y, zv.z, zv.w};
            const float scv[4] = {sc.x, sc.y, sc.z, sc.w}, shv[4] = {sh.x, sh.y, sh.z, sh.w};
            const float muv[4] = {mu.x, mu.y, mu.z, mu.w}, rsv[4] = {rs.x, rs.y, rs.z, rs.w};
#pragma unroll
            for (int j = 0; j < 4; ++j) {
                const float gm = (zz[j] * scv[j] + shv[j]) > 0.f ? acc[j] : 0.f;
                s1[j] += gm;
                s2[j] += gm * ((zz[j] - muv[j]) * rsv[j]);
            }
        }
    }
#pragma unroll
    for (int j = 0; j < 4; ++j) {
        red[(2 * j) * 256 + threadIdx.x] = s1[j];
        red[(2 * j + 1) * 256 + threadIdx.x] = s2[j];
    }
    __syncthreads();
    if ((int)threadIdx.x < c4 * 4) {
        const int q = threadIdx.x >> 2, j = threadIdx.x & 3;
        float a = 0.f, b = 0.f;
        for (int t = q; t < 256; t += c4) {
            a += red[(2 * j) * 256 + t];
            b += red[(2 * j + 1) * 256 + t];
        }
        reinterpret_cast<float2*>(part)[(long)(q * 4 + j) * nblk + blockIdx.x] = make_float2(a, b);
    }
}

template <typename ET>
__global__ __launch_bounds__(256) void maxpool_bn_bwd_rows_apply_kernel(const unsigned char* amax, const ET* g, int n, int h, int w, int c, int ho, int wo,
                                                                        const ET* z, const float* gamma, const float* mean, const float* invstd,
                                                                        const float* scale, const float* shift, const float* dgamma, const float* dbeta,
                                                                        float inv_m, ET* dz) {
    const int c4 = c >> 2;
    const int per = w * c4;
    const int cq = threadIdx.x % c4;
    float av[4], d0[4], kx[4], muv[4], scv[4], shv[4];
    {
        const float4 ga_ = *reinterpret_cast<const float4*>(gamma + cq * 4), rs = *reinterpret_cast<const float4*>(invstd + cq * 4);
        const float4 dg = *reinterpret_cast<const float4*>(dgamma + cq * 4), db = *reinterpret_cast<const float4*>(dbeta + cq * 4);
        const float4 mu = *reinterpret_cast<const float4*>(mean + cq * 4);
        const float4 sc = *reinterpret_cast<const float4*>(scale + cq * 4), sh = *reinterpret_cast<const float4*>(shift + cq * 4);
        const float gav[4] = {ga_.x, ga_.y, ga_.z, ga_.w}, rsv[4] = {rs.x, rs.y, rs.z, rs.w}, dgv[4] = {dg.x, dg.y, dg.z, dg.w}, dbv[4] = {db.x, db.y, db.z, db.w};
        const float mu_[4] = {mu.x, mu.y, mu.z, mu.w}, sc_[4] = {sc.x, sc.y, sc.z, sc.w}, sh_[4] = {sh.x, sh.y, sh.z, sh.w};
#pragma unroll
        for (int j = 0; j < 4; ++j) {
            av[j] = gav[j] * rsv[j];
            d0[j] = dbv[j] * inv_m;
            kx[j] = rsv[j] * dgv[j] * inv_m;
            muv[j] = mu_[j]; scv[j] = sc_[j]; shv[j] = sh_[j];
        }
    }
    const int row_end = min(n * h, ((int)blockIdx.x + 1) * kPoolRB);
    for (int row = blockIdx.x * kPoolRB; row < row_end; ++row) {
        const int img = row / h, ih = row - img * h;
        for (int i = threadIdx.x; i < per; i += 256) {
            const int iw = i / c4;
            float acc[4] = {0.f, 0.f, 0.f, 0.f};
            unsigned amv[4];
            float4 gvv[4];
            bool okv[4];
            unsigned mev[4];
            const long zi = ((long)row * w + iw) * c + cq * 4;
            const float4 zv = ld4(z + zi);
#pragma unroll
            for (int k = 0; k < 4; ++k) {
                const int oh = (ih + (k >> 1)) >> 1, ow = (iw + (k & 1)) >> 1;
                okv[k] = oh < ho && ow < wo && ((k >> 1) == 0 || (ih & 1)) && ((k & 1) == 0 || (iw & 1));
                const int ohc = min(oh, ho - 1), owc = min(ow, wo - 1);
// ... 822 lines not shown
    MVF_LAUNCH_CHECK();
    return MVF_OK;
}

int mvf_bn_bwd_wgrad_splits(long m, int c, int k, int nbn, int mask_mode) {
    int rows, ct, kt;
    if (m <= 0 || c <= 0 || k <= 0 || m * (long)std::max(c, k) * 2 >= 0x7ffffff0L) return 0;
    return mvf_internal::bnbwd_wgrad_plan(m, c, k, nbn, mask_mode, &rows, &ct, &kt);
}

size_t mvf_bn_bwd_wgrad_slab_bytes(long m, int c, int k, int nbn, int mask_mode) {
    return align_up((size_t)mvf_bn_bwd_wgrad_splits(m, c, k, nbn, mask_mode) * c * k * sizeof(float), 256);
}

static int bnwg_fill(mvf_internal::BnBwdWgradArgs& a, long m, int c, int k, int nbn, int mask_mode, size_t slab_bytes) {
    a.M = (int)m; a.C = c; a.K = k;
    a.nsplit = mvf_internal::bnbwd_wgrad_plan(m, c, k, nbn, mask_mode, &a.rows_per_split, &a.ctiles, &a.ktiles);
    MVF_REQUIRE(a.nsplit > 0, MVF_EUNSUPPORTED, "bn backward + weight gradient: shape c=%d k=%d (BatchNorms %d, mask mode %d) is not built; use the separate calls", c, k, nbn, mask_mode);
    MVF_REQUIRE(slab_bytes >= (size_t)a.nsplit * c * k * sizeof(float), MVF_EWS, "bn backward + weight gradient: slab buffer too small (mvf_bn_bwd_wgrad_slab_bytes)");
    return MVF_OK;
}

int mvf_bn_bwd_apply_wgrad(const void* g, int g_pitch, const void* z, const void* ymask, long m, int c, const float* gamma, const float* mean,
                           const float* invstd, const float* scale, const float* shift, const float* dgamma, const float* dbeta, int mask_mode,
                           void* dz, const void* x, int x_pitch, int k, float* slabs, size_t slab_bytes, int dtype, void* stream) {
    MVF_REQUIRE(g && z && gamma && mean && invstd && dgamma && dbeta && dz && x && slabs && m > 0 && c > 0 && k > 0 && g_pitch >= c && x_pitch >= k,
                MVF_EINVAL, "bn_bwd_apply_wgrad: bad argument");
    MVF_REQUIRE(dtype == MVF_BF16, MVF_EUNSUPPORTED, "bn_bwd_apply_wgrad: bf16 storage only");
    MVF_REQUIRE(mask_mode == 2 || mask_mode == 4, MVF_EUNSUPPORTED, "bn_bwd_apply_wgrad: mask mode 2 (scale * z + shift > 0) or 4 (sign bits)");
    MVF_REQUIRE(mask_mode == 2 ? (scale && shift) : (ymask != nullptr), MVF_EINVAL, "bn_bwd_apply_wgrad: the mask operand of mode %d is missing", mask_mode);
    MVF_REQUIRE(g_pitch % 8 == 0 && x_pitch % 8 == 0 && al16(g) && al16(z) && al16(dz) && al16(x) && ((uintptr_t)ymask & 1) == 0 &&
                    m * (long)std::max(g_pitch, x_pitch) * 2 < 0x7ffffff0L, MVF_ESHAPE, "bn_bwd_apply_wgrad: alignment / 2 GB addressing");
    mvf_internal::BnBwdWgradArgs a = {};
    if (int rc = bnwg_fill(a, m, c, k, 1, mask_mode, slab_bytes)) return rc;
    a.g = g; a.g_pitch = g_pitch; a.z[0] = z; a.bits = ymask;
    a.gamma[0] = gamma; a.mean[0] = mean; a.invstd[0] = invstd; a.dgamma[0] = dgamma; a.dbeta[0] = dbeta;
    a.scale = scale; a.shift = shift;
    a.dz[0] = dz; a.x[0] = x; a.xps[0] = x_pitch; a.part[0] = slabs;
    return mvf_internal::bnbwd_wgrad_launch(a, 1, mask_mode, (hipStream_t)stream);
}

int mvf_bn_bwd_pair_wgrad(const void* g, int g_pitch, const void* z_a, const void* z_b, const unsigned char* sign_bits, long m, int c,
                          const float* gamma_a, const float* mean_a, const float* invstd_a, float* dgamma_a, float* dbeta_a,
                          const float* gamma_b, const float* mean_b, const float* invstd_b, float* dgamma_b, float* dbeta_b,
                          void* dz_a, void* dz_b, const void* x_a, int xa_pitch, const void* x_b, int xb_pitch, int k,
                          float* slabs_a, float* slabs_b, size_t slab_bytes, void* ws, size_t ws_bytes, int dtype, void* stream) {
    MVF_REQUIRE(g && z_a && z_b && sign_bits && gamma_a && mean_a && invstd_a && dgamma_a && dbeta_a && gamma_b && mean_b && invstd_b && dgamma_b && dbeta_b &&
                    dz_a && dz_b && x_a && slabs_a && (!x_b || slabs_b) && m > 0 && c > 0 && k > 0 && g_pitch >= c && xa_pitch >= k && (!x_b || xb_pitch >= k),
                MVF_EINVAL, "bn_bwd_pair_wgrad: bad argument");
    MVF_REQUIRE(dtype == MVF_BF16, MVF_EUNSUPPORTED, "bn_bwd_pair_wgrad: bf16 storage only");
    MVF_REQUIRE(ws && ws_bytes >= 2 * mvf_bn_workspace_bytes(m, c), MVF_EWS, "bn_bwd_pair_wgrad: workspace too small (2 x mvf_bn_workspace_bytes)");
    MVF_REQUIRE(g_pitch % 8 == 0 && xa_pitch % 8 == 0 && (!x_b || xb_pitch % 8 == 0) && al16(g) && al16(z_a) && al16(z_b) && al16(dz_a) && al16(dz_b) &&
                    al16(x_a) && (!x_b || al16(x_b)) && ((uintptr_t)sign_bits & 1) == 0 &&
                    m * (long)std::max(g_pitch, std::max(xa_pitch, x_b ? xb_pitch : 0)) * 2 < 0x7ffffff0L, MVF_ESHAPE, "bn_bwd_pair_wgrad: alignment / 2 GB addressing");
    mvf_internal::BnBwdWgradArgs a = {};
    if (int rc = bnwg_fill(a, m, c, k, 2, 4, slab_bytes)) return rc;
    MVF_REQUIRE(x_b || a.ktiles == 1, MVF_EUNSUPPORTED, "bn_bwd_pair_wgrad: k tiles");
    int kt_, ct_;
    MVF_REQUIRE(mvf_internal::bnbwd_wgrad_tile(c, k, 2, 4, &ct_, &kt_) && (!x_b || kt_ == 64), MVF_EUNSUPPORTED,
                "bn_bwd_pair_wgrad: both convs are contracted for k = 64 only (k = 128: pass x_b = NULL)");
    hipStream_t st = (hipStream_t)stream;
    float* part_a = (float*)ws;
    float* part_b = (float*)((char*)ws + mvf_bn_workspace_bytes(m, c));
    {
        const bool wide = false;
        const int gy = col_plan(m, c, 4).gy;
        MVF_BN_DISPATCH(bn_bwd_reduce2_kernel, wide, 2048, (const ET*)g, g_pitch, (const ET*)z_a, (const ET*)z_b, (const void*)sign_bits, m, c, mean_a, invstd_a,
                        mean_b, invstd_b, p.cqb, p.rows, part_a, part_b);
        MVF_LAUNCH_CHECK();
        const int gA = (c + kFinCh - 1) / kFinCh;
        hipLaunchKernelGGL(bn_bwd_finalize2_kernel, dim3(2 * gA), dim3(256), 0, st, c, gy, part_a, part_b, dgamma_a, dbeta_a, dgamma_b, dbeta_b);
        MVF_LAUNCH_CHECK();
    }
    a.g = g; a.g_pitch = g_pitch; a.z[0] = z_a; a.z[1] = z_b; a.bits = sign_bits;
    a.gamma[0] = gamma_a; a.mean[0] = mean_a; a.invstd[0] = invstd_a; a.dgamma[0] = dgamma_a; a.dbeta[0] = dbeta_a;
    a.gamma[1] = gamma_b; a.mean[1] = mean_b; a.invstd[1] = invstd_b; a.dgamma[1] = dgamma_b; a.dbeta[1] = dbeta_b;
    a.dz[0] = dz_a; a.dz[1] = dz_b; a.x[0] = x_a; a.x[1] = x_b; a.xps[0] = xa_pitch; a.xps[1] = xb_pitch;
    a.part[0] = slabs_a; a.part[1] = slabs_b;
    return mvf_internal::bnbwd_wgrad_launch(a, 2, 4, st);
}

int mvf_conv1x1_bwd_fused_splits(long m, int c, int k) { return mvf_internal::pw_bwd_fused_plan(m, c, k, nullptr); }

int mvf_conv1x1_bwd_fused(const void* a_in, int a_pitch, const void* w_packed, const void* g, int g_pitch, const unsigned char* sign_bits, long m, int c,
                          int k, const float* gamma, const float* mean, const float* invstd, const float* dgamma, const float* dbeta, const void* z_in,
                          const float* in_mean, const float* in_invstd, const float* in_scale, const float* in_shift, void* dx, float* sums_part,
                          int sums_rows, float* slabs, size_t slab_bytes, int dtype, void* stream) {
    MVF_REQUIRE(a_in && w_packed && g && sign_bits && gamma && mean && invstd && dgamma && dbeta && dx && slabs && m > 0 && a_pitch >= k && g_pitch >= c &&
                    (!z_in || (in_mean && in_invstd && in_scale && in_shift && sums_part)), MVF_EINVAL, "conv1x1_bwd_fused: bad argument");
    MVF_REQUIRE(dtype == MVF_BF16, MVF_EUNSUPPORTED, "conv1x1_bwd_fused: bf16 storage only");
    mvf_internal::PwBwdFusedArgs a = {};
    a.nsplit = mvf_internal::pw_bwd_fused_plan(m, c, k, &a.rows_per_split);
    MVF_REQUIRE(a.nsplit > 0, MVF_EUNSUPPORTED, "conv1x1_bwd_fused: built for 64 -> 256 channels (c=%d k=%d); use the separate calls", c, k);
    MVF_REQUIRE(!z_in || sums_rows == 2 * a.nsplit, MVF_EINVAL, "conv1x1_bwd_fused: sums_rows must be 2 x mvf_conv1x1_bwd_fused_splits (%d), got %d", 2 * a.nsplit, sums_rows);
    MVF_REQUIRE(slab_bytes >= (size_t)a.nsplit * c * k * sizeof(float), MVF_EWS, "conv1x1_bwd_fused: slab buffer too small (splits x c x k floats)");
    MVF_REQUIRE(a_pitch % 8 == 0 && g_pitch % 8 == 0 && al16(a_in) && al16(w_packed) && al16(g) && (!z_in || al16(z_in)) && al16(dx) && ((uintptr_t)sign_bits & 15) == 0 &&
                    m * (long)std::max(g_pitch, a_pitch) * 2 < 0x7ffffff0L, MVF_ESHAPE, "conv1x1_bwd_fused: alignment / 2 GB addressing");
    a.a = a_in; a.aps = a_pitch; a.w = w_packed; a.g = g; a.g_pitch = g_pitch; a.bits = sign_bits; a.M = (int)m;
    a.gamma = gamma; a.mean = mean; a.invstd = invstd; a.dgamma = dgamma; a.dbeta = dbeta;
    a.z_in = z_in; a.in_mean = in_mean; a.in_invstd = in_invstd; a.in_scale = in_scale; a.in_shift = in_shift;
    a.dx = dx; a.sums_part = sums_part; a.sums_rows = sums_rows; a.part = slabs;
    return mvf_internal::pw_bwd_fused_launch(a, (hipStream_t)stream);
}

int mvf_conv1x1_bnbwd_sums_pair(const void* a_in, int a_pitch, const void* w_a, const void* x_in, int x_pitch, const void* w_b, const void* g, int g_pitch,
                                const unsigned char* sign_bits, long m, int c, int k, const float* mean_a, const float* invstd_a, const float* mean_b,
                                const float* invstd_b, float* part_a, float* part_b, int rows, int dtype, void* stream) {
    MVF_REQUIRE(a_in && w_a && g && sign_bits && mean_a && invstd_a && part_a && m > 0 && a_pitch >= k && g_pitch >= c &&
                    (!x_in || (w_b && mean_b && invstd_b && part_b && x_pitch >= k)), MVF_EINVAL, "conv1x1_bnbwd_sums_pair: bad argument");
    MVF_REQUIRE(dtype == MVF_BF16, MVF_EUNSUPPORTED, "conv1x1_bnbwd_sums_pair: bf16 storage only");
    mvf_internal::PwSumsPairArgs a = {};
    a.nsplit = mvf_internal::pw_bwd_fused_plan(m, c, k, &a.rows_per_split);
    MVF_REQUIRE(a.nsplit > 0, MVF_EUNSUPPORTED, "conv1x1_bnbwd_sums_pair: built for 64 -> 256 channels (c=%d k=%d); use the separate calls", c, k);
    MVF_REQUIRE(rows == 2 * a.nsplit, MVF_EINVAL, "conv1x1_bnbwd_sums_pair: rows must be 2 x mvf_conv1x1_bwd_fused_splits (%d), got %d", 2 * a.nsplit, rows);
    MVF_REQUIRE(a_pitch % 8 == 0 && g_pitch % 8 == 0 && al16(a_in) && al16(w_a) && al16(g) && (!x_in || (x_pitch % 8 == 0 && al16(x_in) && al16(w_b))) &&
                    ((uintptr_t)sign_bits & 15) == 0 && m * (long)std::max(g_pitch, std::max(a_pitch, x_in ? x_pitch : 0)) * 2 < 0x7ffffff0L, MVF_ESHAPE,
                "conv1x1_bnbwd_sums_pair: alignment / 2 GB addressing");
    a.a = a_in; a.aps = a_pitch; a.x = x_in; a.xps = x_pitch; a.w_a = w_a; a.w_b = w_b; a.g = g; a.g_pitch = g_pitch; a.bits = sign_bits; a.M = (int)m;
    a.mean_a = mean_a; a.invstd_a = invstd_a; a.mean_b = mean_b; a.invstd_b = invstd_b; a.part_a = part_a; a.part_b = part_b; a.rows = rows;
    return mvf_internal::pw_sums_pair_launch(a, (hipStream_t)stream);
}

int mvf_wgrad_slab_reduce(const float* slabs, int nsplit, int cout, int k, float* dw_oihw, void* stream) {
    MVF_REQUIRE(slabs && dw_oihw && nsplit > 0 && cout > 0 && k > 0, MVF_EINVAL, "wgrad_slab_reduce: bad argument");
    return mvf_internal::wgrad_slab_reduce_launch(slabs, nsplit, cout, k, dw_oihw, (hipStream_t)stream);
}

int mvf_maxpool_bn_relu_fwd(const void* z, int n, int h, int w, int c, const float* scale, const float* shift, void* y,
                            unsigned char* argmax, int dtype, void* stream) {
    MVF_REQUIRE(z && y && scale && shift && n > 0 && h > 0 && w > 0 && c > 0 && c % 4 == 0, MVF_EINVAL, "maxpool_bn_relu_fwd: bad argument");
    const int ho = (h - 1) / 2 + 1, wo = (w - 1) / 2 + 1;
    const long total = (long)n * ho * wo * (c / 4);
    {
        static const int blk_on = mvf_policy_int("pool_fwd_block", 1);
        const int vc = dtype == MVF_F32 ? 4 : 8;
        if (blk_on && h % 4 == 0 && w % 4 == 0 && c % vc == 0 && ((uintptr_t)z | (uintptr_t)y) % 16 == 0 && (uintptr_t)argmax % 8 == 0) {
            const long tb = (long)n * (ho / 2) * (wo / 2) * (c / vc);
            if (dtype == MVF_F32)
                hipLaunchKernelGGL(maxpool_bn_fwd_blk_kernel<float>, dim3(grid_for(tb, 256 * 8)), dim3(256), 0, (hipStream_t)stream, (const float*)z, n, h, w, c, ho, wo, scale, shift, (float*)y, argmax);
            else
                hipLaunchKernelGGL(maxpool_bn_fwd_blk_kernel<bf16_t>, dim3(grid_for(tb, 256 * 8)), dim3(256), 0, (hipStream_t)stream, (const bf16_t*)z, n, h, w, c, ho, wo, scale, shift, (bf16_t*)y, argmax);
            MVF_LAUNCH_CHECK();
            return MVF_OK;
        }
    }
    if (dtype == MVF_F32)
        hipLaunchKernelGGL(maxpool_bn_fwd_kernel<float>, dim3(grid_for(total, 256 * 32)), dim3(256), 0, (hipStream_t)stream, (const float*)z, n, h, w, c, ho, wo, scale, shift, (float*)y, argmax);
    else
        hipLaunchKernelGGL(maxpool_bn_fwd_kernel<bf16_t>, dim3(grid_for(total, 256 * 32)), dim3(256), 0, (hipStream_t)stream, (const bf16_t*)z, n, h, w, c, ho, wo, scale, shift, (bf16_t*)y, argmax);
    MVF_LAUNCH_CHECK();
    return MVF_OK;
}

int mvf_maxpool_bn_relu_bwd(const unsigned char* argmax, const void* g, int n, int h, int w, int c, void* ga, int dtype, void* stream) {
    MVF_REQUIRE(argmax && g && ga && n > 0 && h > 0 && w > 0 && c > 0 && c % 4 == 0, MVF_EINVAL, "maxpool_bn_relu_bwd: bad argument");
    const int ho = (h - 1) / 2 + 1, wo = (w - 1) / 2 + 1;
    const long total = (long)n * h * w * (c / 4);
    if ((long)n * h < (1L << 31) && (long)w * (c / 4) >= 256) {
        if (dtype == MVF_F32)
            hipLaunchKernelGGL(maxpool_bn_bwd_rows_kernel<float>, dim3(n * h), dim3(256), 0, (hipStream_t)stream, argmax, (const float*)g, n, h, w, c, ho, wo, (float*)ga);
        else
            hipLaunchKernelGGL(maxpool_bn_bwd_rows_kernel<bf16_t>, dim3(n * h), dim3(256), 0, (hipStream_t)stream, argmax, (const bf16_t*)g, n, h, w, c, ho, wo, (bf16_t*)ga);
        MVF_LAUNCH_CHECK();
        return MVF_OK;
    }
    if (dtype == MVF_F32)
        hipLaunchKernelGGL(maxpool_bn_bwd_kernel<float>, dim3(grid_for(total, 256 * 64)), dim3(256), 0, (hipStream_t)stream, argmax, (const float*)g, n, h, w, c, ho, wo, (float*)ga);
    else
        hipLaunchKernelGGL(maxpool_bn_bwd_kernel<bf16_t>, dim3(grid_for(total, 256 * 64)), dim3(256), 0, (hipStream_t)stream, argmax, (const bf16_t*)g, n, h, w, c, ho, wo, (bf16_t*)ga);
    MVF_LAUNCH_CHECK();
    return MVF_OK;
}

static bool pool_blk_ok(const void* amax, const void* g, const void* ga, const void* z, const void* dz, int h, int w, int c, int dtype) {
    static const int on = mvf_policy_int("pool_bwd_block", 1);
    const int vc = dtype == MVF_F32 ? 4 : 8;
    return on && h % 2 == 0 && w % 2 == 0 && c % vc == 0 && 256 % (c / vc) == 0 && c <= 256 && (uintptr_t)amax % 8 == 0 &&
           ((uintptr_t)g | (uintptr_t)(ga ? ga : g) | (uintptr_t)z | (uintptr_t)(dz ? dz : z)) % 16 == 0;
}

int mvf_maxpool_bwd_sums_rows(int n, int h) { return n > 0 && h > 0 ? (int)(((long)n * h + kPoolRB - 1) / kPoolRB) : 0; }

int mvf_maxpool_bn_relu_bwd_sums(const unsigned char* argmax, const void* g, int n, int h, int w, int c, void* ga, const void* z, const float* mean,
                                 const float* invstd, const float* scale, const float* shift, float* sums_part, int dtype, void* stream) {
    MVF_REQUIRE(argmax && g && z && mean && invstd && scale && shift && sums_part && n > 0 && h > 0 && w > 0 && c > 0 && c % 4 == 0, MVF_EINVAL,
                "maxpool_bn_relu_bwd_sums: bad argument");
    MVF_REQUIRE(256 % (c / 4) == 0 && (long)n * h < (1L << 31), MVF_EUNSUPPORTED, "maxpool_bn_relu_bwd_sums: needs c/4 to divide 256 (use the two-pass form)");
    const int ho = (h - 1) / 2 + 1, wo = (w - 1) / 2 + 1, nblk = mvf_maxpool_bwd_sums_rows(n, h);
    if (pool_blk_ok(argmax, g, ga, z, nullptr, h, w, c, dtype)) {
        if (dtype == MVF_F32)
            hipLaunchKernelGGL((maxpool_bn_bwd_blk_kernel<float, 0>), dim3(nblk), dim3(256), 0, (hipStream_t)stream, argmax, (const float*)g, n, h, w, c, ho, wo, (float*)ga,
                               (const float*)z, nullptr, mean, invstd, scale, shift, nullptr, nullptr, 0.f, sums_part, nblk, nullptr);
        else
            hipLaunchKernelGGL((maxpool_bn_bwd_blk_kernel<bf16_t, 0>), dim3(nblk), dim3(256), 0, (hipStream_t)stream, argmax, (const bf16_t*)g, n, h, w, c, ho, wo, (bf16_t*)ga,
                               (const bf16_t*)z, nullptr, mean, invstd, scale, shift, nullptr, nullptr, 0.f, sums_part, nblk, nullptr);
        MVF_LAUNCH_CHECK();
        return MVF_OK;
    }
    if (dtype == MVF_F32)
        hipLaunchKernelGGL(maxpool_bn_bwd_rows_sums_kernel<float>, dim3(nblk), dim3(256), 0, (hipStream_t)stream, argmax, (const float*)g, n, h, w, c, ho, wo, (float*)ga,
                           (const float*)z, mean, invstd, scale, shift, sums_part, nblk);
    else
        hipLaunchKernelGGL(maxpool_bn_bwd_rows_sums_kernel<bf16_t>, dim3(nblk), dim3(256), 0, (hipStream_t)stream, argmax, (const bf16_t*)g, n, h, w, c, ho, wo, (bf16_t*)ga,
                           (const bf16_t*)z, mean, invstd, scale, shift, sums_part, nblk);
    MVF_LAUNCH_CHECK();
    return MVF_OK;
}

int mvf_maxpool_bn_relu_bwd_apply(const unsigned char* argmax, const void* g, int n, int h, int w, int c, const void* z, const float* gamma,
                                  const float* mean, const float* invstd, const float* scale, const float* shift, const float* dgamma,
                                  const float* dbeta, void* dz, int dtype, void* stream) {
    MVF_REQUIRE(argmax && g && z && gamma && mean && invstd && scale && shift && dgamma && dbeta && dz && n > 0 && h > 0 && w > 0 && c > 0 && c % 4 == 0,
                MVF_EINVAL, "maxpool_bn_relu_bwd_apply: bad argument");
    MVF_REQUIRE(256 % (c / 4) == 0 && (long)n * h < (1L << 31), MVF_EUNSUPPORTED, "maxpool_bn_relu_bwd_apply: needs c/4 to divide 256 (use the two-pass form)");
    const int ho = (h - 1) / 2 + 1, wo = (w - 1) / 2 + 1, nblk = mvf_maxpool_bwd_sums_rows(n, h);
    const float inv_m = 1.0f / (float)((long)n * h * w);
    if (pool_blk_ok(argmax, g, nullptr, z, dz, h, w, c, dtype)) {
        if (dtype == MVF_F32)
            hipLaunchKernelGGL((maxpool_bn_bwd_blk_kernel<float, 1>), dim3(nblk), dim3(256), 0, (hipStream_t)stream, argmax, (const float*)g, n, h, w, c, ho, wo, (float*)nullptr,
                               (const float*)z, gamma, mean, invstd, scale, shift, dgamma, dbeta, inv_m, nullptr, nblk, (float*)dz);
        else
            hipLaunchKernelGGL((maxpool_bn_bwd_blk_kernel<bf16_t, 1>), dim3(nblk), dim3(256), 0, (hipStream_t)stream, argmax, (const bf16_t*)g, n, h, w, c, ho, wo, (bf16_t*)nullptr,
                               (const bf16_t*)z, gamma, mean, invstd, scale, shift, dgamma, dbeta, inv_m, nullptr, nblk, (bf16_t*)dz);
        MVF_LAUNCH_CHECK();
        return MVF_OK;
    }
    if (dtype == MVF_F32)
        hipLaunchKernelGGL(maxpool_bn_bwd_rows_apply_kernel<float>, dim3(nblk), dim3(256), 0, (hipStream_t)stream, argmax, (const float*)g, n, h, w, c, ho, wo,
                           (const float*)z, gamma, mean, invstd, scale, shift, dgamma, dbeta, inv_m, (float*)dz);
    else
        hipLaunchKernelGGL(maxpool_bn_bwd_rows_apply_kernel<bf16_t>, dim3(nblk), dim3(256), 0, (hipStream_t)stream, argmax, (const bf16_t*)g, n, h, w, c, ho, wo,
                           (const bf16_t*)z, gamma, mean, invstd, scale, shift, dgamma, dbeta, inv_m, (bf16_t*)dz);
    MVF_LAUNCH_CHECK();
    return MVF_OK;
}

int mvf_head_train_fwd(const void* feat, int clips, int t, int hw, int c, const float* fc_w, const float* fc_b, int classes,
                       const long long* labels, const float* drop_mask, float* pooled, float* scores, float* dscores, float* loss_part, float* loss,
                       int dtype, void* stream);
int mvf_head_train_bwd(const float* dscores, const float* pooled, const float* fc_w, const float* drop_mask, int clips, int t, int hw, int c, int classes,
                       float* dfc_w, float* dfc_b, float* dpool_ws, void* dfeat, int dtype, void* stream);

}

namespace {
constexpr int kHeadSplit = 25;
__global__ __launch_bounds__(256) void head_fc_seg_kernel(const float* pooled, const float* w, const float* b, int clips, int T, int c, int classes, float* scores) {
    extern __shared__ float pc[];
    const int clip = blockIdx.x, part = blockIdx.y, tid = threadIdx.x, lane = tid & 63, wave = tid >> 6;
    const float inv = 1.f / (float)T;
    for (int i = tid; i < c; i += 256) {
        float s = 0.f;
        for (int t = 0; t < T; ++t) s += pooled[((long)clip * T + t) * c + i];
        pc[i] = s * inv;
    }
    __syncthreads();
    const int per = (classes + kHeadSplit - 1) / kHeadSplit;
    const int k_end = min(classes, (part + 1) * per);
    const int kb = part * per + wave;
    float s[4] = {0.f, 0.f, 0.f, 0.f};
    for (int i = lane; i < c; i += 64) {
        const float f = pc[i];
#pragma unroll
        for (int u = 0; u < 4; ++u) {
            const int k = kb + 4 * u;
            s[u] += f * w[(long)(k < k_end ? k : kb < k_end ? kb : 0) * c + i];
        }
    }
    for (int u0 = 0; u0 * 16 < per; ++u0) {
        if (u0 > 0) {
#pragma unroll
            for (int u = 0; u < 4; ++u) s[u] = 0.f;
            for (int i = lane; i < c; i += 64) {
                const float f = pc[i];
#pragma unroll
                for (int u = 0; u < 4; ++u) {
                    const int k = kb + 16 * u0 + 4 * u;
                    s[u] += f * w[(long)(k < k_end ? k : 0) * c + i];
                }
            }
        }
#pragma unroll
        for (int u = 0; u < 4; ++u) {
            float v = s[u];
            for (int off = 32; off > 0; off >>= 1) v += __shfl_xor(v, off, 64);
            const int k = kb + 16 * u0 + 4 * u;
            if (lane == 0 && k < k_end) scores[(long)clip * classes + k] = v + (b ? b[k] : 0.f);
        }
    }
}
}

extern "C" {

int mvf_head_train_fwd(const void* feat, int clips, int t, int hw, int c, const float* fc_w, const float* fc_b, int classes,
                       const long long* labels, const float* drop_mask, float* pooled, float* scores, float* dscores, float* loss_part, float* loss,
                       int dtype, void* stream) {
    MVF_REQUIRE(feat && fc_w && labels && pooled && scores && dscores && loss_part && loss && clips > 0 && t > 0 && hw > 0 && c > 0 && classes > 0, MVF_EINVAL, "head_train_fwd: bad argument");
    hipStream_t st = (hipStream_t)stream;
    dim3 g((c + 255) / 256, clips * t);
    if (dtype == MVF_F32) hipLaunchKernelGGL(frame_pool_kernel<float>, g, dim3(256), 0, st, (const float*)feat, hw, c, drop_mask, pooled);
    else hipLaunchKernelGGL(frame_pool_kernel<bf16_t>, g, dim3(256), 0, st, (const bf16_t*)feat, hw, c, drop_mask, pooled);
    MVF_LAUNCH_CHECK();
    MVF_REQUIRE((size_t)c * sizeof(float) <= 160 * 1024, MVF_EUNSUPPORTED, "head_train_fwd: c=%d does not fit the LDS feature buffer", c);
    hipLaunchKernelGGL(head_fc_seg_kernel, dim3(clips, kHeadSplit), dim3(256), (size_t)c * sizeof(float), st, pooled, fc_w, fc_b, clips, t, c, classes, scores);
    MVF_LAUNCH_CHECK();
// ... 177 lines not shown
```

mvfnet_amd/csrc/wgrad_nhwc.hip:

```cpp
#include <algorithm>

#include <stdlib.h>

#include "common.h"

namespace {

constexpr int kThreads = 256;
constexpr int BMR = 32;
typedef float f32x16 __attribute__((ext_vector_type(16)));

struct WgArgs {
    const void* dz;
    const void* x;
    const void* x2;
    float* part;
    int N, H, W, Cin, Cout, KH, KW, stride, pad, Ho, Wo, xps, split_c, x2ps;
    int M, K, rows_per_split, tiles_k;
    int tiles, nsplit;
    unsigned fd_hw_mul, fd_hw_shr, fd_w_mul, fd_w_shr;
    int xcd_rr;
    int abl;
};

// ... 1135 lines not shown

static bool wg_direct3x3(const mvf_conv_desc_t* d) {
    return d->dtype == MVF_BF16 && d->cin == 64 && d->cout == 64 && d->kh == 3 && d->kw == 3 && d->stride == 1 && d->pad == 1 && d->split_c == 0 &&
           d->ho == d->h && d->wo == d->w && mvf_internal::wgrad3x3_c64_ok(d->n, d->h, d->w, d->x_pix_stride);
}

static bool wg_direct_stem(const mvf_conv_desc_t* d) {
    return d->dtype == MVF_BF16 && d->cin == 32 && d->cout == 64 && d->kh == 7 && d->kw == 1 && d->stride == 2 && d->pad == 0 && d->split_c == 0 &&
           d->x_pix_stride == 4 && mvf_internal::wgrad_stem_ok(d->n, d->h, d->w, d->ho, d->wo);
}

size_t mvf_conv2d_wgrad_workspace_bytes(const mvf_conv_desc_t* d) {
    if (!d || d->cout <= 0 || d->cin <= 0) return 0;
    const int M = d->n * d->ho * d->wo, K = d->kh * d->kw * d->cin;
    const WgTile t = pick_tile(d->cout, K);
    const int tiles = ((d->cout + t.bco - 1) / t.bco) * ((K + t.bk - 1) / t.bk);
    const int rows = plan_split(M, tiles);
    int nsplit = (M + rows - 1) / rows;
    if (wg_big_shape(d)) nsplit = std::max(nsplit, (M + wg_big_rows(d) - 1) / wg_big_rows(d));
    if (wg_direct3x3(d)) nsplit = std::max(nsplit, mvf_internal::wgrad3x3_c64_wgs(d->n, d->h));
    if (wg_direct_stem(d)) nsplit = std::max(nsplit, mvf_internal::wgrad_stem_wgs(d->n, d->ho));
    return align_up((size_t)nsplit * d->cout * K * sizeof(float), 256);
}

}
static int wgrad_impl(const mvf_conv_desc_t* d, const void* dz, const void* x, const void* x2, int kw_real, int cin_real,
                      int kw_packed, int cin_packed, float* dw_oihw, void* ws, size_t ws_bytes, void* stream, int wgs_target) {
    t_last_wgrad = mvf_wgrad_launch_info_t{};
    MVF_REQUIRE(d && dz && x && dw_oihw, MVF_EINVAL, "wgrad: NULL argument");
    MVF_REQUIRE(d->dtype == MVF_F32 || d->dtype == MVF_BF16, MVF_EINVAL, "wgrad: bad dtype");
    MVF_REQUIRE(d->cin % 4 == 0 && d->cout % 4 == 0 && d->x_pix_stride > 0, MVF_ESHAPE, "wgrad: cin/cout must be multiples of 4");
    MVF_REQUIRE(kw_packed * cin_packed == d->kw * d->cin && kw_real <= kw_packed && cin_real <= cin_packed, MVF_EINVAL, "wgrad: packed extents inconsistent");
    MVF_REQUIRE(ws && ws_bytes >= mvf_conv2d_wgrad_workspace_bytes(d), MVF_EWS, "wgrad: workspace too small");
    if (d->split_c) MVF_REQUIRE(x2 && d->kh == 1 && d->kw == 1 && d->split_c % 4 == 0, MVF_EINVAL, "wgrad: bad split_c");
    hipStream_t st0 = (hipStream_t)stream;
    if (wg_direct3x3(d) && kw_real == 3 && cin_real == 64 && kw_packed == 3 && cin_packed == 64 && ((uintptr_t)dz | (uintptr_t)x) % 16 == 0) {
        Wgrad3x3C64Args w = {dz, x, (float*)ws, d->n, d->h, d->w, d->x_pix_stride, mvf_internal::wgrad3x3_c64_wgs(d->n, d->h)};
        const int rc = mvf_internal::wgrad3x3_c64_launch(w, st0);
        if (rc != MVF_OK) return rc;
        t_last_wgrad = mvf_wgrad_launch_info_t{MVF_WGRAD_FAM_C3X3_C64, 0, 64, 576, MVF_BF16, w.nwg, 0, 0, 0, 0, 0, 1};
        const int rr = launch_wgrad_reduce((const float*)ws, w.nwg, 64, 64, 3, 3, 3, 64, dw_oihw, st0);
        if (rr == MVF_OK) t_last_wgrad.launches = 2;
        return rr;
    }
    if (wg_direct_stem(d) && kw_real == 7 && cin_real == 3 && kw_packed == 8 && cin_packed == 4 && ((uintptr_t)dz | (uintptr_t)x) % 16 == 0) {
        WgradStemArgs w = {dz, x, (float*)ws, d->n, d->h, d->w, d->ho, d->wo, mvf_internal::wgrad_stem_wgs(d->n, d->ho)};
        const int rc = mvf_internal::wgrad_stem_launch(w, st0);
        if (rc != MVF_OK) return rc;
        t_last_wgrad = mvf_wgrad_launch_info_t{MVF_WGRAD_FAM_STEM, 0, 64, 224, MVF_BF16, w.nwg, 0, 0, 0, 0, 0, 1};
        const int rr = launch_wgrad_reduce((const float*)ws, w.nwg, 64, 3, 7, 7, 8, 4, dw_oihw, st0);
        if (rr == MVF_OK) t_last_wgrad.launches = 2;
        return rr;
    }
    WgArgs a = {};
    a.dz = dz; a.x = x; a.x2 = x2; a.part = (float*)ws;
    a.N = d->n; a.H = d->h; a.W = d->w; a.Cin = d->cin; a.Cout = d->cout; a.KH = d->kh; a.KW = d->kw;
    a.stride = d->stride; a.pad = d->pad; a.Ho = d->ho; a.Wo = d->wo; a.xps = d->x_pix_stride;
    a.split_c = d->split_c; a.x2ps = d->x2_pix_stride;
    a.M = d->n * d->ho * d->wo; a.K = d->kh * d->kw * d->cin;
    WgTile t = pick_tile(d->cout, a.K);
    static const int gram_env = std::max(8, mvf_policy_int("gram_wgs", 32));
    const bool gram = wgs_target <= 0 && dz == x && !x2 && d->kh == 1 && d->kw == 1 && d->cin == d->cout;
    const int gram_wgs = wgs_target > 0 ? wgs_target : gram ? gram_env : 0;
    bool big = wg_big_shape(d) && wgs_target <= 0 && ((uintptr_t)dz | (uintptr_t)x | (uintptr_t)(x2 ? x2 : x)) % 16 == 0 &&
               (long)a.N * a.H * a.W * std::max(a.xps, a.x2ps) * 2 < 0x7ffffff0L;
    if (big) {
        const int rows = wg_big_rows(d, gram_wgs);
        big = rows >= 4 * 64 && ((long)rows + 6 * 64) * d->cout * 2 < 0x7ffffff0L;
        if (big) t = WgTile{256, 256};
    }
    a.tiles_k = (a.K + t.bk - 1) / t.bk;
    const int tiles = ((d->cout + t.bco - 1) / t.bco) * a.tiles_k;
    static const int x3_env = (mvf_policy_int("f32_x3", 1) != 0) && (mvf_policy_int("wgrad_x3", 1) != 0);
    bool x3 = d->dtype == MVF_F32 && x3_env && d->cin % 4 == 0 && d->cout % 4 == 0 && d->x_pix_stride % 4 == 0 && d->split_c % 4 == 0 &&
              (d->x2_pix_stride % 4 == 0 || !d->split_c) && ((uintptr_t)dz | (uintptr_t)x | (uintptr_t)(x2 ? x2 : x)) % 16 == 0;
    static const bool wgs_forced = mvf_policy_has("wgrad_wgs");
    const int bf16_wgs = (d->dtype == MVF_BF16 && !wgs_forced) ? 256 : 0;
    int target_used = 0;
    a.rows_per_split = big ? wg_big_rows(d, gram_wgs, &target_used) : plan_split(a.M, tiles, gram_wgs ? gram_wgs : (x3 && !wgs_forced ? 768 : bf16_wgs), &target_used);
    if (wgs_target > 0) {
        const long fit = std::max<long>(1, (long)(mvf_conv2d_wgrad_workspace_bytes(d) / ((size_t)d->cout * a.K * sizeof(float))));
        if ((a.M + a.rows_per_split - 1) / a.rows_per_split > fit) a.rows_per_split = std::max(a.rows_per_split, (int)(((a.M + fit - 1) / fit + 63) / 64 * 64));
    }
    x3 = x3 && ((long)a.rows_per_split + 64) * d->cout * 4 < 0x7ffffff0L;
    if (d->dtype == MVF_F32 && !x3 && !wgs_forced && !gram_wgs) a.rows_per_split = plan_split(a.M, tiles, 0, &target_used);
    const int nsplit = (a.M + a.rows_per_split - 1) / a.rows_per_split;
    MVF_REQUIRE(ws_bytes >= (size_t)nsplit * d->cout * a.K * sizeof(float), MVF_EWS, "wgrad: workspace too small for %d slabs", nsplit);
    a.tiles = tiles;
    a.nsplit = nsplit;
    a.xcd_rr = nsplit % 8 == 0;
#ifdef MVF_WGRAD_ABLATE
    a.abl = mvf_policy_int("wgrad_abl", 0);
#endif
    wg_fd_make((unsigned)(a.Ho * a.Wo), a.fd_hw_mul, a.fd_hw_shr);
    wg_fd_make((unsigned)a.Wo, a.fd_w_mul, a.fd_w_shr);
    hipStream_t st = (hipStream_t)stream;
    static const int dma32_env = mvf_policy_int("wgrad_dma_f32", 1);
    const bool dma32 = d->dtype == MVF_F32 && dma32_env && d->cin % 4 == 0 && d->cout % 4 == 0 && d->x_pix_stride % 4 == 0 &&
                       (a.split_c == 0 || (a.split_c % t.bk == 0 && a.Cin % t.bk == 0)) &&
                       ((uintptr_t)dz | (uintptr_t)x | (uintptr_t)(x2 ? x2 : x)) % 16 == 0 &&
                       (long)a.N * a.H * a.W * std::max(a.xps, a.x2ps) * 4 < 0x7ffffff0L && ((long)a.rows_per_split + 64) * d->cout * 4 < 0x7ffffff0L;
    int fam = MVF_WGRAD_FAM_NONE, stages = 0;
    if (x3) {
        fam = MVF_WGRAD_FAM_X3;
        if (t.bco == 64) hipLaunchKernelGGL((wgrad_x3_kernel<1, 2>), dim3(nsplit * tiles), dim3(256), 0, st, a);
        else if (t.bk == 64) hipLaunchKernelGGL((wgrad_x3_kernel<2, 1>), dim3(nsplit * tiles), dim3(256), 0, st, a);
        else hipLaunchKernelGGL((wgrad_x3_kernel<2, 2>), dim3(nsplit * tiles), dim3(256), 0, st, a);
    } else if (dma32) {
        fam = MVF_WGRAD_FAM_F32_DMA; stages = 2;
        if (t.bco == 64) hipLaunchKernelGGL((wgrad_kernel<float, 1, 2, true>), dim3(nsplit * tiles), dim3(kThreads), 0, st, a);
        else if (t.bk == 64) hipLaunchKernelGGL((wgrad_kernel<float, 2, 1, true>), dim3(nsplit * tiles), dim3(kThreads), 0, st, a);
        else hipLaunchKernelGGL((wgrad_kernel<float, 2, 2, true>), dim3(nsplit * tiles), dim3(kThreads), 0, st, a);
    } else if (d->dtype == MVF_F32) {
        fam = MVF_WGRAD_FAM_F32_REG;
        if (t.bco == 64) hipLaunchKernelGGL((wgrad_kernel<float, 1, 2>), dim3(nsplit * tiles), dim3(kThreads), 0, st, a);
        else if (t.bk == 64) hipLaunchKernelGGL((wgrad_kernel<float, 2, 1>), dim3(nsplit * tiles), dim3(kThreads), 0, st, a);
        else hipLaunchKernelGGL((wgrad_kernel<float, 2, 2>), dim3(nsplit * tiles), dim3(kThreads), 0, st, a);
    } else if (d->cin % 8 == 0 && d->cout % 8 == 0 && d->x_pix_stride % 4 == 0 && (d->split_c % 8) == 0 &&
               ((uintptr_t)dz | (uintptr_t)x | (uintptr_t)(x2 ? x2 : x)) % 16 == 0 &&
               ((long)a.rows_per_split + 6 * 64) * d->cout * 2 < 0x7ffffff0L) {
        int rc;
        if (big) rc = launch_wgrad_bf16_big(a, tiles, nsplit, st, fam, stages);
        else if (t.bco == 64) rc = launch_wgrad_bf16<1, 2>(a, tiles, nsplit, st, fam, stages);
        else if (t.bk == 64) rc = launch_wgrad_bf16<2, 1>(a, tiles, nsplit, st, fam, stages);
        else rc = launch_wgrad_bf16<2, 2>(a, tiles, nsplit, st, fam, stages);
        if (rc) return rc;
    } else {
        fam = MVF_WGRAD_FAM_BF16_WIDEN;
        if (t.bco == 64) hipLaunchKernelGGL((wgrad_kernel<bf16_t, 1, 2>), dim3(nsplit * tiles), dim3(kThreads), 0, st, a);
        else if (t.bk == 64) hipLaunchKernelGGL((wgrad_kernel<bf16_t, 2, 1>), dim3(nsplit * tiles), dim3(kThreads), 0, st, a);
        else hipLaunchKernelGGL((wgrad_kernel<bf16_t, 2, 2>), dim3(nsplit * tiles), dim3(kThreads), 0, st, a);
    }
    MVF_LAUNCH_CHECK();
    t_last_wgrad = mvf_wgrad_launch_info_t{fam, stages, t.bco, t.bk, d->dtype, nsplit, a.rows_per_split, a.xcd_rr, a.split_c > 0 ? 1 : 0, gram ? 1 : 0, target_used, 1};
    const int kh_p = d->kh * d->kw * d->cin / (kw_packed * cin_packed);
    const int rr = launch_wgrad_reduce(a.part, nsplit, d->cout, cin_real, kh_p, kw_real, kw_packed, cin_packed, dw_oihw, st);
    if (rr == MVF_OK) t_last_wgrad.launches = 2;
    return rr;
}
extern "C" {

int mvf_conv2d_nhwc_wgrad(const mvf_conv_desc_t* d, const void* dz, const void* x, const void* x2, int kw_real, int cin_real,
                          int kw_packed, int cin_packed, float* dw_oihw, void* ws, size_t ws_bytes, void* stream) {
    return wgrad_impl(d, dz, x, x2, kw_real, cin_real, kw_packed, cin_packed, dw_oihw, ws, ws_bytes, stream, 0);
}

int mvf_conv2d_nhwc_wgrad_wgs(const mvf_conv_desc_t* d, const void* dz, const void* x, const void* x2, int kw_real, int cin_real,
                              int kw_packed, int cin_packed, float* dw_oihw, void* ws, size_t ws_bytes, int wgs, void* stream) {
    t_last_wgrad = mvf_wgrad_launch_info_t{};
    MVF_REQUIRE(wgs >= 8 && wgs <= 4096, MVF_EINVAL, "wgrad_wgs: wgs=%d outside 8 .. 4096", wgs);
    return wgrad_impl(d, dz, x, x2, kw_real, cin_real, kw_packed, cin_packed, dw_oihw, ws, ws_bytes, stream, wgs);
}

int mvf_conv2d_wgrad_last_launch(mvf_wgrad_launch_info_t* out) {
    MVF_REQUIRE(out, MVF_EINVAL, "conv2d_wgrad_last_launch: NULL argument");
    *out = t_last_wgrad;
    return MVF_OK;
}

int mvf_pack_conv_weights_batched(const mvf_pack_job_t* jobs_dev, int njobs, int total_blocks, int dtype, void* stream) {
    MVF_REQUIRE(jobs_dev && njobs > 0 && total_blocks > 0 && (dtype == MVF_F32 || dtype == MVF_BF16), MVF_EINVAL, "pack_conv_weights_batched: bad argument");
    if (dtype == MVF_F32)
        hipLaunchKernelGGL(pack_batched_kernel<float>, dim3(total_blocks), dim3(256), 0, (hipStream_t)stream, jobs_dev, njobs);
    else
        hipLaunchKernelGGL(pack_batched_kernel<bf16_t>, dim3(total_blocks), dim3(256), 0, (hipStream_t)stream, jobs_dev, njobs);
    MVF_LAUNCH_CHECK();
    return MVF_OK;
}

int mvf_pack_conv_weight_dgrad(const float* w_oihw, int cout, int cin, int kh, int kw, void* w_packed, int dtype, void* stream) {
    MVF_REQUIRE(w_oihw && w_packed && cout > 0 && cin > 0 && kh > 0 && kw > 0, MVF_EINVAL, "pack_conv_weight_dgrad: bad argument");
    const long total = (long)cout * cin * kh * kw;
    const int blocks = (int)std::min<long>((total + 255) / 256, 4096);
    if (dtype == MVF_F32)
        hipLaunchKernelGGL(pack_dgrad_weight_kernel<float>, dim3(blocks), dim3(256), 0, (hipStream_t)stream, w_oihw, cout, cin, kh, kw, (float*)w_packed);
    else
        hipLaunchKernelGGL(pack_dgrad_weight_kernel<bf16_t>, dim3(blocks), dim3(256), 0, (hipStream_t)stream, w_oihw, cout, cin, kh, kw, (bf16_t*)w_packed);
    MVF_LAUNCH_CHECK();
    return MVF_OK;
}

}
```

mvfnet_amd/csrc/wgrad_stem.hip:

```cpp
#include <algorithm>
#include <stdlib.h>

#include "common.h"

namespace {

typedef float f32x16 __attribute__((ext_vector_type(16)));
typedef short bf16x8_t __attribute__((ext_vector_type(8)));

struct KArgs {
    const char* dz;
    const char* x;
    float* part;
    int N, H, W, Ho, Wo;
    int bands_per_frame, bands;
    int rowb;
    int xbytes, dpix;
    int ksr;
    unsigned fd_bpf_mul, fd_bpf_shr, fd_ksr_mul, fd_ksr_shr;
};

__device__ __forceinline__ int fdiv(int n, unsigned mul, unsigned shr) { return (int)((__umulhi((unsigned)n, mul) + (unsigned)n) >> shr); }
__device__ __forceinline__ int swzf(int pixel) { return ((pixel >> 1) & 1) << 2; }

template <int kR>
__global__ __launch_bounds__(256, 2) void wgrad_stem_kernel(KArgs a) {
    extern __shared__ __attribute__((aligned(16))) char smem[];
    char* Xs = smem;
    char* Ds = smem + (a.xbytes + 1023) / 1024 * 1024;
    const int tid = threadIdx.x, lane = tid & 63;
    const int wave = __builtin_amdgcn_readfirstlane(tid >> 6);
    const int wm = wave & 1, kg = wave >> 1;
    constexpr unsigned kOOB = 0x80000000u;
    const i32x4 gs_x = rsrc_words(a.x, (unsigned)((long)a.N * a.H * a.rowb));
    const i32x4 gs_d = rsrc_words(a.dz, (unsigned)((long)a.N * a.Ho * a.Wo * 128));
    const unsigned lds_x = (unsigned)__builtin_amdgcn_readfirstlane((int)(unsigned)(size_t)(__attribute__((address_space(3))) char*)Xs);
    const unsigned lds_d = (unsigned)__builtin_amdgcn_readfirstlane((int)(unsigned)(size_t)(__attribute__((address_space(3))) char*)Ds);
    const int nx = (a.xbytes + 1023) >> 10, nd = a.dpix >> 3;
    const int lp = lane >> 3, lu = lane & 7;

    const int tg = lane >> 4, ti = lane & 15;
    const int trow = (ti >> 2) + 8 * (tg >> 1);
    const int tunit = 2 * (tg & 1) + ((ti & 3) >> 1), thalf = ti & 1;
    const int offA = trow * 128 + (((wm * 4 + tunit) ^ swzf(trow)) << 4) + thalf * 8;
    const int offB = 16 * trow + 32 * (tg & 1) + 8 * (ti & 3);
    typedef short v4s __attribute__((ext_vector_type(4)));
    typedef __attribute__((address_space(3))) v4s* lds_v4s;
    auto gather = [&](const char* lo_p, const char* hi_p) {
        const v4s lo = __builtin_amdgcn_ds_read_tr16_b64_v4i16((lds_v4s)(lo_p));
        const v4s hi = __builtin_amdgcn_ds_read_tr16_b64_v4i16((lds_v4s)(hi_p));
        bf16x8_t v;
        v[0] = lo[0]; v[1] = lo[1]; v[2] = lo[2]; v[3] = lo[3];
        v[4] = hi[0]; v[5] = hi[1]; v[6] = hi[2]; v[7] = hi[3];
        return v;
    };

    f32x16 acc[4];
#pragma unroll
    for (int t = 0; t < 4; ++t)
#pragma unroll
        for (int r = 0; r < 16; ++r) acc[t][r] = 0.f;

    const int nks = a.dpix >> 4;
    for (int b = blockIdx.x; b < a.bands; b += gridDim.x) {
        const int img = fdiv(b, a.fd_bpf_mul, a.fd_bpf_shr);
        const int oh0 = (b - img * a.bands_per_frame) * kR;
        __syncthreads();
        {
            const long xbase = ((long)img * a.H + 2 * oh0) * a.rowb;
            for (int i = wave; i < nx; i += 4) {
                const int o = i * 1024 + lane * 16;
                glds16(gs_x, lds_x + (unsigned)(i * 1024), o < a.xbytes ? (unsigned)(xbase + o) : kOOB);
            }
            const long dbase = ((long)img * a.Ho + oh0) * a.Wo * 128;
            for (int i = wave; i < nd; i += 4) {
                const int p = i * 8 + lp;
                glds16(gs_d, lds_d + (unsigned)(i * 1024), (unsigned)(dbase + p * 128 + ((lu ^ swzf(p)) << 4)));
            }
        }
        asm volatile("s_waitcnt vmcnt(0)" ::: "memory");
        __syncthreads();
        for (int ks = 0; ks < nks; ++ks) {
            const int r = fdiv(ks, a.fd_ksr_mul, a.fd_ksr_shr), ow0 = (ks - r * a.ksr) * 16;
            const bf16x8_t fa = gather(Ds + ks * 2048 + offA, Ds + ks * 2048 + offA + 4 * 128);
            const char* xb = Xs + (2 * r + 4 * kg) * a.rowb + ow0 * 16 + offB;
            bf16x8_t fb[4];
#pragma unroll
            for (int t = 0; t < 4; ++t) {
                if (t < 3 || kg == 0) fb[t] = gather(xb + t * a.rowb, xb + t * a.rowb + 64);
            }
#pragma unroll
            for (int t = 0; t < 4; ++t) {
                if (t < 3 || kg == 0) acc[t] = __builtin_amdgcn_mfma_f32_32x32x16_bf16(fa, fb[t], acc[t], 0, 0, 0);
            }
        }
    }
    const int lr = lane >> 5, lc = lane & 31;
    float* out = a.part + (long)blockIdx.x * 64 * 224;
#pragma unroll
    for (int t = 0; t < 4; ++t) {
        if (t < 3 || kg == 0) {
            const int col = (4 * kg + t) * 32 + lc;
#pragma unroll
            for (int r = 0; r < 16; ++r) {
                const int row = wm * 32 + (r & 3) + 8 * (r >> 2) + 4 * lr;
                out[row * 224 + col] = acc[t][r];
            }
        }
    }
}

inline void fd_make(unsigned d, unsigned& mul, unsigned& shr) {
    unsigned l = 0;
    while ((1ull << l) < d) ++l;
    mul = (unsigned)((((1ull << l) - d) << 32) / d + 1);
    shr = l;
}

static int band_rows() {
    static const int r = mvf_policy_int("wgrad_stem_r", 2);
    return r == 1 ? 1 : 2;
}

}

namespace mvf_internal {

bool wgrad_stem_ok(int n, int h, int w, int ho, int wo) {
    static const bool on = (mvf_policy_int("wgrad_stem_direct", 1) != 0);
    return on && n > 0 && wo >= 16 && wo % 16 == 0 && ho % 2 == 0 && (w * 8) % 16 == 0 && 2 * (ho - 1) + 6 < h && 2 * (wo - 1) + 7 < w &&
           (long)n * h * w * 8 < 0x7ffffff0L && (long)n * ho * wo * 128 < 0x7ffffff0L &&
           (2 * 2 + 5) * w * 8 + 1024 + 2 * wo * 128 <= 72 * 1024;
}

int wgrad_stem_wgs(int n, int ho) {
    static const int env = std::max(1, mvf_policy_int("wgrad_stem_wgs", 768));
    return (int)std::min<long>(env, (long)n * (ho / band_rows()));
}

int wgrad_stem_launch(const WgradStemArgs& w, hipStream_t st) {
    KArgs a = {};
    a.dz = (const char*)w.dz; a.x = (const char*)w.x; a.part = w.part;
    a.N = w.N; a.H = w.H; a.W = w.W; a.Ho = w.Ho; a.Wo = w.Wo;
    const int kR = band_rows();
    a.bands_per_frame = w.Ho / kR;
    a.bands = w.N * a.bands_per_frame;
    a.rowb = w.W * 8;
    a.xbytes = (2 * kR + 5) * a.rowb;
    a.dpix = kR * w.Wo;
    a.ksr = w.Wo / 16;
    fd_make((unsigned)a.bands_per_frame, a.fd_bpf_mul, a.fd_bpf_shr);
    fd_make((unsigned)a.ksr, a.fd_ksr_mul, a.fd_ksr_shr);
    const int lds = (a.xbytes + 1023) / 1024 * 1024 + a.dpix * 128;
    static bool attr = false;
    if (!attr) {
        MVF_HIP_OK(hipFuncSetAttribute((const void*)wgrad_stem_kernel<1>, hipFuncAttributeMaxDynamicSharedMemorySize, 72 * 1024));
        MVF_HIP_OK(hipFuncSetAttribute((const void*)wgrad_stem_kernel<2>, hipFuncAttributeMaxDynamicSharedMemorySize, 72 * 1024));
        attr = true;
    }
    if (kR == 1) hipLaunchKernelGGL(wgrad_stem_kernel<1>, dim3(w.nwg), dim3(256), lds, st, a);
    else hipLaunchKernelGGL(wgrad_stem_kernel<2>, dim3(w.nwg), dim3(256), lds, st, a);
    MVF_LAUNCH_CHECK();
    return MVF_OK;
}

}
```

mvfnet_amd/train_engine.py:

```python
import ctypes as C
import os

import torch

from . import _lib
from ._lib import ConvDesc, MvfDesc, check, lib

F32 = _lib.MVF_F32

_ConvDescT, _MvfDescT = ConvDesc, MvfDesc
_DESC_CACHE = {}


def ConvDesc(*a):
    d = _DESC_CACHE.get(a)
    if d is None:
        d = _DESC_CACHE[a] = _ConvDescT(*a)
    return d


def MvfDesc(*a):
    k = ("mvf",) + a
    d = _DESC_CACHE.get(k)
    if d is None:
# ... 817 lines not shown
            self.gated_out, self.sums_out = og is not None, (gs["sums"] if gs is not None else False)
            if self.split_ok:
                self.c1.wgrad(dz1, s["x"], nt, h, w, h, w, eng, x_pitch=c, x2=s["o"], split_c=self.mvf.cs)
            else:
                self.c1.wgrad(dz1, s["xin"], nt, h, w, h, w, eng, x_pitch=c)
            self.mvf.backward(dxp, s["x"], s["y"], nt, h, w, c, eng, addend=resid if fuse else None, addend_bits=rbits if fuse else None, out_gate=og, gsum=gs)
            if not fuse:
                if rbits is not None:
                    resid = resid * (s["out"] > 0).to(resid.dtype)
                dx = eng.add(dxp, resid, key=id(self))
            else:
                dx = dxp
        if eng.keep_io:
            self.io = dict(x=s["x"], out=s["out"], g=g, dx=dx, h=h, w=w, c=c, ho=ho, wo=wo, g_gated=g_gated, dx_gated=self.gated_out)
        self.saved = None
        eng.flush_side(late=True)
        return dx


class _StatTable(object):

    def __init__(self, eng, bns):
        names = {id(m_): n_ for n_, m_ in eng.model.named_modules()}
        segs, self.keys, self.slices, first = [], [], [], 0
        for bn in bns:
            for attr in ("running_mean", "running_var"):
                t = getattr(bn.mod, attr)
                segs.append(_lib.StatSegment(t.data_ptr(), first))
                self.keys.append("%s.%s" % (names[id(bn.mod)], attr))
                self.slices.append((first, t.numel(), tuple(t.shape)))
                first += t.numel()
        self.bns, self.nseg, self.n = list(bns), len(segs), first
        arr = (_lib.StatSegment * len(segs))(*segs)
        self.dev = torch.frombuffer(bytearray(bytes(arr)), dtype=torch.uint8).to(eng.device)
        self.acc = torch.zeros(first, dtype=torch.float64, device=eng.device)
        self.shadow = torch.empty(first, dtype=torch.float32, device=eng.device)

    def accumulate(self):
        check(lib.mvf_bn_stats_accumulate(_p(self.dev), self.nseg, self.n, _p(self.acc), _st()), "bn stats accumulate")

    def finalize(self, count, dst=None):
        check(lib.mvf_bn_stats_finalize(_p(self.dev), self.nseg, self.n, _p(self.acc), count, _p(dst), _st()), "bn stats finalize")

    def exchange(self, flat, mode):
        check(lib.mvf_bn_stats_exchange(_p(self.dev), self.nseg, self.n, _p(flat), mode, _st()), "bn stats exchange")


class _ParamStore(object):

    def _init_store(self, model, dtype=torch.float32, rehome=True):
        if dtype not in (torch.float32, torch.bfloat16):
            raise TypeError("training dtype must be float32 or bfloat16 (activation storage; weights/statistics/gradients stay fp32)")
        self.tdtype = dtype
        self.dt = _lib.MVF_F32 if dtype == torch.float32 else _lib.MVF_BF16
        dev = next(model.parameters()).device
        if dev.type != "cuda":
            raise RuntimeError("the HIP training engine needs the model on an MI355X device; no CPU fallback")
        self.model, self.device = model, dev
        self._side_pending = []
        self._side_keep = []
        params = [p for p in model.parameters()]
        n = sum(p.numel() for p in params)
        pad = lambda k: (k + 3) // 4 * 4
        total = sum(pad(p.numel()) for p in params)
        self.rehomed = bool(rehome)
        self.flat_params = torch.zeros(total, device=dev) if rehome else None
        self.flat_grads = torch.zeros(total, device=dev)
        self.flat_mom = torch.zeros(total, device=dev) if rehome else None
        self._grad_view = {}
        off = 0
        with torch.no_grad():
            for p in params:
                k = p.numel()
                if rehome:
                    v = self.flat_params[off:off + k].view(p.shape)
                    v.copy_(p.data.float())
                    p.data = v
                elif p.dtype != torch.float32 or not p.is_contiguous() or p.device != dev:
                    raise TypeError("stand-alone block: parameters must be contiguous float32 tensors on %s" % dev)
                gv = self.flat_grads[off:off + k].view(p.shape)
                self._grad_view[id(p)] = gv
                off += pad(k)
        self.n_params = n
        if rehome:
            for m_ in model.modules():
                if hasattr(m_, "invalidate_engine"):
                    m_.invalidate_engine()
        self._ws = None
        self.norm_out = torch.zeros(2, device=dev)
        self.steps = 0
        self.ema_momentum, self.ema_warmup_steps, self.ema_updates = None, 0, 0
        self._ones = {}
        self._bufs = {}
        self._caps = {}
        self._last_shape = {}

    def grad_of(self, p):
        return self._grad_view[id(p)]

    def buf(self, key, shape, dtype=None):
        dt = dtype or self.tdtype
        shape = tuple(shape)
        k = (key, shape, dt)
        step = getattr(self, "forward_count", None)
        if step is not None:
            last = self._last_shape.get((key, dt))
            if last is not None and last[0] == step and last[1] != shape:
                raise RuntimeError("engine buffer %r requested with shapes %s and %s inside one step: they would share storage" % (key, last[1], shape))
            self._last_shape[(key, dt)] = (step, shape)
        t = self._bufs.get(k)
        if t is None:
            n = 1
            for v in shape:
                n *= int(v)
            ck = (key, dt)
            flat = self._caps.get(ck)
            if flat is None or flat.numel() < n:
                if flat is not None:
                    self._side_keep.append(flat)
                    self._storage_epoch += 1
                    for kk in [kk for kk in self._bufs if kk[0] == key and kk[2] == dt]:
                        del self._bufs[kk]
                flat = torch.empty(max(n, 1), device=self.device, dtype=dt)
                self._caps[ck] = flat
            t = flat[:n].view(shape)
            self._bufs[k] = t
        return t

    def workspace(self, nbytes, side=False):
        key = "_ws_side" if side else "_ws"
        ws = getattr(self, key, None)
        if ws is None or ws.numel() < nbytes:
            if ws is not None:
                self._storage_epoch += 1
            ws = torch.empty(max(int(nbytes), 1 << 20), dtype=torch.uint8, device=self.device)
            setattr(self, key, ws)
        return ws

    _storage_epoch = 0

    overlap_wgrad = True
    keep_io = False
    fuse_stats = True
    overlap_downsample = _policy("side_downsample", 1) != 0
    z3_free = _policy("z3_free", 1)
    fuse_bn3_apply = _policy("fuse_bn3_apply", 1)
    fuse_bn_bwd_sums = _policy("fuse_bn_bwd", 1) != 0
    fuse_bn_bwd_strided = _policy("fuse_bn_bwd_strided", 1) != 0
    pair_bn_bwd = _policy("pair_bn_bwd", 1) != 0
    fuse_bnwg = _policy("fuse_bnwg", 7)
    pair_ds_sums = _policy("pair_ds_sums", 3)
    z3_free_ds = _policy("z3_free_ds", 1)
    fuse_c3_bwd = _policy("fuse_c3_bwd", 1)
    fuse_mvf_stats = _policy("fuse_mvf_stats", 1) != 0
    dzfree = _policy("dzfree", 2)
    gate_producer = _policy("gate_producer", 1) != 0
    dzfree_q = _policy("dzfree_q", 1)
    dzfree_q_wgs = _policy("dzfree_q_wgs", 256)
    dzfree_q_maxk = _policy("dzfree_q_maxk", 256)
    dzfree_q_mink = _policy("dzfree_q_mink", 0)
    gram_stats = _policy("gram_stats", 1) != 0
    gram_stats_wgs = _policy("gram_stats_wgs", 256)
    gram_colsums = _policy("gram_colsums", 1) != 0

    def side_stream(self):
        if not self.overlap_wgrad:
            return None
        if getattr(self, "_side", None) is None:
            from .streams import concurrent_stream
            self._side = concurrent_stream(self.main_stream())
        return self._side

    def main_stream(self):
        ms = getattr(self, "_main", None)
        return ms if ms is not None else torch.cuda.current_stream()

    _rec = None

    def _wait(self, dst, src):
        if self._rec is not None:
            self._rec.wait(dst, src)
        else:
            dst.wait_stream(src)

    def _mark(self, stream):
        if self._rec is not None:
            return self._rec.mark(stream)
        ev = torch.cuda.Event()
        ev.record(stream)
        return ev

    def _wait_mark(self, stream, ev):
        if self._rec is not None:
            self._rec.wait_mark(stream, ev)
        else:
            stream.wait_event(ev)

    def on_side(self, launch):
        self._side_keep.append(launch)
        self._side_pending.append(launch)


    def flush_side(self, late=False):
        pend = getattr(self, "_side_pending", None)
        marked = getattr(self, "_side_marked", None)
        if late and pend:
            ev = self._mark(self.main_stream())
            if marked is None:
                marked = self._side_marked = []
            marked.append((ev, list(pend)))
            del pend[:]
            return
        self.issue_marked()
        if pend:
            self._wait(self._side, self.main_stream())
            with _on_stream(self._side):
                for launch in pend:
                    launch()
            del pend[:]

    def issue_marked(self):
        marked = getattr(self, "_side_marked", None)
        if marked:
            for ev, launches in marked:
                self._wait_mark(self._side, ev)
                with _on_stream(self._side):
                    for launch in launches:
                        launch()
            del marked[:]

    def join_side(self):
        self.flush_side()
        if getattr(self, "_side", None) is not None:
            self._wait(self.main_stream(), self._side)
        del self._side_keep[:]

    def add(self, a, b, key=None):
        m, c = a.shape
        if c not in self._ones:
            self._ones[c] = (torch.ones(c, device=a.device), torch.zeros(c, device=a.device))
        one, zero = self._ones[c]
        out = self.buf((key or id(a), "add"), a.shape, a.dtype) if key is not None else torch.empty_like(a)
        check(lib.mvf_bn_apply(_p(a), m, c, _p(one), _p(zero), _p(b), None, None, 0, _p(out), self.dt, _st()), "add")
        return out

    lr, momentum, weight_decay, max_norm = 0.015, 0.9, 1e-4, 40.0

    def trainable_offset(self):
        params = list(self.model.parameters())
        flags = [p.requires_grad for p in params]
        k = flags.index(True) if True in flags else len(flags)
        self._scattered_frozen = not all(flags[k:])
        return self._grad_view[id(params[k])].storage_offset() if k < len(params) else self.flat_grads.numel()

    nesterov = True
    param_options = None

    def set_param_options(self, options):
        self.param_options = {id(p): (float(a), float(b)) for p, (a, b) in options.items()} if options else None
        self._seg_tables = {}

    def _segments(self, off):
        tabs = self.__dict__.setdefault("_seg_tables", {})
        key = (off, tuple(p.requires_grad for p in self.model.parameters()))
        if key not in tabs:
            segs, last = [], None
            for p in self.model.parameters():
                first = self._grad_view[id(p)].storage_offset()
                if first + p.numel() <= off:
                    continue
                mult = (self.param_options or {}).get(id(p), (1.0, 1.0)) if p.requires_grad else (-1.0, 0.0)
                if mult != last:
                    segs.append(_lib.SgdSegment(max(first - off, 0) if segs else 0, mult[0], mult[1]))
                    last = mult
            arr = (_lib.SgdSegment * len(segs))(*segs)
            tabs[key] = (torch.frombuffer(bytearray(bytes(arr)), dtype=torch.uint8).to(self.device), len(segs))
        return tabs[key]

    def apply_sgd(self, lr=None, world=1):
        return self._apply_optimizer(self.flat_grads, 1.0 / world, lr)

    def _apply_optimizer(self, grads, grad_scale, lr=None):
        ls = self._lstats
        if ls is not None:
            ls["grads"], ls["scale"] = grads, float(grad_scale)
            measured = self._layer_stats_before(grads)
        if self._adam is not None:
            out = self._apply_adamw(grads, grad_scale, lr)
        else:
            out = self._apply_sgd(grads, grad_scale, lr)
        if ls is not None:
            ls["grads"] = None
            if measured and out is not None:
                self._layer_stats_after()
        return out

    _lstats = None

    def _flat_stats(self, x, y, out, guard=None, step_out=None):
        ls = self._lstats
        check(lib.mvf_flat_segment_stats(_p(x), _p(y), x.numel(), _p(ls["first"]), ls["nseg"], _p(out), _p(guard), _p(step_out), _p(ls["ws"]), ls["ws"].numel(),
                                         _st()), "flat segment stats")

    def _layer_stats_before(self, grads):
        ls = self._lstats
        if not ls["armed"] or not self.rehomed:
# ... 513 lines not shown
            if self.input_pipeline is None:
                raise RuntimeError("uint8 frames need engine.input_pipeline = preprocess.FramePipeline(...)")
            h, w = self.input_pipeline.crop_hw
        else:
            h, w = imgs.shape[3:]
        return int(h), int(w)

    _TABLE_STAGES = 4

    def _upload_table(self, name, parts):
        import numpy as np
        n = sum(int(p.size) for p in parts)
        table = self.buf(name, (n,), torch.int32)
        ring = self.__dict__.setdefault("_table_stages", {}).get((name, n))
        if ring is None:
            ring = self._table_stages[(name, n)] = dict(next=0, used=set(), slots=[(torch.empty(n, dtype=torch.int32).pin_memory(), torch.cuda.Event())
                                                                                   for _ in range(self._TABLE_STAGES)])
        k = ring["next"]
        ring["next"] = (k + 1) % self._TABLE_STAGES
        host, ev = ring["slots"][k]
        if k in ring["used"]:
            ev.synchronize()
        hn = host.numpy()
        views, off = [], 0
        for p in parts:
            hn[off:off + p.size] = p.reshape(-1).view(np.int32)
            views.append(table[off:off + p.size])
            off += p.size
        table.copy_(host, non_blocking=True)
        ev.record()
        ring["used"].add(k)
        return views

    def _upload_blend_table(self, rows, wts, b):
        import numpy as np
        rows_d, wts_d = self._upload_table("blend_table", [np.ascontiguousarray(rows, dtype=np.int32), np.ascontiguousarray(wts, dtype=np.float32)])
        return rows_d.view(b, 5), wts_d.view(torch.float32).view(b, 2)

    def _upload_erase_table(self, boxes, fill, key):
        import numpy as np
        key_d, boxes_d, fill_d = self._upload_table("erase_table", [np.ascontiguousarray(key, dtype=np.uint32), np.ascontiguousarray(boxes, dtype=np.int32),
                                                                    np.ascontiguousarray(fill, dtype=np.float32)])
        return boxes_d, fill_d, key_d, int(boxes.shape[1])

    def _randaug_refusals(self, imgs):
        from .preprocess import AddressedFramePipeline, Yuv420FramePipeline
        if imgs.dtype != torch.uint8:
            raise ValueError("TrainEngine: randaug augments uint8 frames (engine.input_pipeline = preprocess.FramePipeline(...)); float images are "
                             "normalised already -- augment them before Normalize, or set engine.randaug = None")
        pipe = self.input_pipeline
        if isinstance(pipe, (Yuv420FramePipeline, AddressedFramePipeline)):
            raise ValueError("TrainEngine: randaug takes packed (B, T, Hs, Ws, 3) frames; %s input (decoder-native planes) is out of scope" % type(pipe).__name__)
        if pipe is not None and (imgs.dim() != 5 or imgs.shape[-1] != 3):
            raise ValueError("TrainEngine: randaug takes (B, T, Hs, Ws, 3) uint8 frames, got %s" % (tuple(imgs.shape),))

    def _distill_refusals(self):
        chk = getattr(self.distill, "check_step", None)
        if chk is not None:
            chk(self.model, self.tdtype)

    def _draw_randaug(self, imgs):
        import numpy as np
        from .preprocess import ResamplingFramePipeline, JITTER_COLS, RESAMPLE_COLS
        from .randaug import check_randaug_table, stats_mask
        self._randaug_refusals(imgs)
        self._input_hw(imgs)
        pipe = self.input_pipeline
        b, t, hs, ws = (int(v) for v in imgs.shape[:4])
        order = 0 if pipe.to_rgb else 1
        sizes_d, sizes_h = None, (hs, ws)
        if isinstance(pipe, ResamplingFramePipeline):
            rows = pipe._as_table(self.input_window)
            if rows.shape[1] not in (RESAMPLE_COLS, JITTER_COLS) or rows.shape[0] != b * t:
                raise ValueError("TrainEngine: randaug needs one 11- / 23-column row per frame (%d frames), got a table %s" % (b * t, tuple(rows.shape)))
            sizes_d = rows[:, :2].contiguous()
            sizes_h = sizes_d.cpu().numpy()
            if (sizes_h < 1).any() or (sizes_h[:, 0] > hs).any() or (sizes_h[:, 1] > ws).any():
                raise ValueError("TrainEngine: a frame size of the window table lies outside the %dx%d frames" % (hs, ws))
        table, _ = self.randaug.draw(b, t, sizes_h, order)
        check_randaug_table(table, b)
        table = np.ascontiguousarray(table, dtype=np.int32)
        (table_d,) = self._upload_table("randaug_table", [table])
        return table_d, sizes_d, int(table.shape[1]), stats_mask(table), order

    def _randaug_frames(self, imgs):
        from .randaug import WS_PER_FRAME
        table_d, sizes_d, layers, mask, order = self._randaug_table
        f = imgs.reshape((-1,) + tuple(imgs.shape[-3:])).contiguous()
        n, hs, ws = (int(v) for v in f.shape[:3])
        out, tmp = self.buf("randaug_out", tuple(f.shape), torch.uint8), self.buf("randaug_tmp", tuple(f.shape), torch.uint8)
        wsb = self.buf("randaug_ws", (n * WS_PER_FRAME,), torch.uint8)
        check(lib.mvf_frames_randaug_u8(_p(f), n, hs, ws, int(imgs.shape[1]), order, _p(sizes_d), _p(table_d), layers, mask, _p(out), _p(tmp), _p(wsb),
                                        wsb.numel(), _st()), "frames_randaug")
        return out.view(imgs.shape)

    def _soft_labels(self, imgs, labels):
        return labels.is_floating_point() and labels.dim() == 2 and tuple(labels.shape) == (imgs.shape[0], self.num_classes)

    def _uses_soft_head(self, lab):
        return self.blending is not None or self.label_smooth_eps > 0.0 or lab.is_floating_point()

    def set_options(self, lr=None, momentum=None, weight_decay=None, max_norm=None, dtype=None, optimizer=None, betas=None, eps=None):
        if dtype is not None and dtype != self.tdtype:
            raise RuntimeError("the model's train engine was built with dtype %s; it cannot be switched to %s" % (self.tdtype, dtype))
        for k, v in (("lr", lr), ("momentum", momentum), ("weight_decay", weight_decay), ("max_norm", max_norm)):
            if v is not None:
                setattr(self, k, v)
        if optimizer is not None or betas is not None or eps is not None:
            self.set_optimizer(optimizer if optimizer is not None else self.optimizer, betas=betas, eps=eps)

    def _forward(self, imgs, labels, stages=None, prepared=None):
        b, t = imgs.shape[0], imgs.shape[1]
        lab, mask, loss = prepared if prepared is not None else self._step_tensors(imgs, labels)
        u8 = imgs.dtype == torch.uint8
        h, w = self._input_hw(imgs)
        if u8:
            x = None
            nt = b * t
        else:
            x = imgs.reshape((-1, 3) + tuple(imgs.shape[3:])).contiguous()
            nt = x.shape[0]
        self._pack_all(0)
        side = self.side_stream()
        if side is not None:
            self._wait(side, self.main_stream())
        with _on_stream(side if side is not None else self.main_stream()):
            self._pack_all(1)
        self._packs_on_side = side is not None
        hp, wp = h + 6, (w + 6 + 2 + 1) // 2 * 2
        xp = self.buf("xp", (nt, hp, wp, 4))
        if u8:
            if self.randaug is not None:
                imgs = self._randaug_frames(imgs)
            self.input_pipeline.to_stem(imgs, self.input_window, 3, wp, self.tdtype, out=xp)
        else:
            check(lib.mvf_stem_prep(_p(x), nt, 3, h, w, 3, wp, _p(xp), self.dt, _st()), "stem_prep")
        if self.erasing is not None:
            boxes_d, fill_d, key_d, max_boxes = self._erase_table
            check(lib.mvf_stem_erase(_p(xp), nt, hp, wp, 3, _p(boxes_d), max_boxes, _p(fill_d), _p(key_d), self.dt, _st()), "stem_erase")
        if self.blending is not None:
            rows_d, wts_d = self._blend_table
            xb = self.buf("xp_blend", (nt, hp, wp, 4))
            check(lib.mvf_stem_blend(_p(xp), b, t, hp, wp, 3, _p(rows_d), _p(wts_d), _p(xb), self.dt, _st()), "stem_blend")
            xp = xb
        teacher_scores = None
        if self.distill is not None:
            teacher_scores = self.buf("teacher_scores", (b, self.num_classes), torch.float32)
            self.distill.teacher_scores(xp, b, t, h, w, out=teacher_scores)
        ho, wo = (h + 6 - 7) // 2 + 1, (w + 6 - 7) // 2 + 1
        z0, _, _ = self.stem.forward(xp, nt, hp, wp, ho=ho, wo=wo, bn=self.stem_bn)
        h2, w2 = (ho - 1) // 2 + 1, (wo - 1) // 2 + 1
        p0 = self.buf("p0", (nt * h2 * w2, 64))
        amax = self.buf("amax", (nt * h2 * w2, 64), torch.uint8)
        check(lib.mvf_maxpool_bn_relu_fwd(_p(z0), nt, ho, wo, 64, _p(self.stem_bn.scale), _p(self.stem_bn.shift), _p(p0), _p(amax), self.dt, _st()), "maxpool fwd")
        self.saved = dict(xp=xp, z0=z0, amax=amax, nt=nt, hp=hp, wp=wp, ho=ho, wo=wo, t=t, b=b)
        if stages is not None:
            stages["maxpool"] = p0.view(nt, h2, w2, 64)
        xcur, hc, wc, cc = p0, h2, w2, 64
        ends, k = [], 0
        for name in self.model.backbone.res_layers:
            k += len(getattr(self.model.backbone, name))
            ends.append(k)
        for i, blk in enumerate(self.blocks):
            xcur, hc, wc, cc = blk.forward(xcur, nt, hc, wc, cc, self)
            if stages is not None and (i + 1) in ends:
                stages["layer%d" % (ends.index(i + 1) + 1)] = xcur.view(nt, hc, wc, cc)
        dev = imgs.device
        f32 = torch.float32
        pooled = self.buf("pooled", (nt, cc), f32)
        scores = self.buf("scores", (b, self.num_classes), f32)
        dscores = self.buf("dscores", (b, self.num_classes), f32)
        loss_part = self.buf("loss_part", (b,), f32)
        if self._uses_soft_head(lab):
            if lab.is_floating_point():
                targets = lab
            else:
                rows_d, wts_d = self._blend_table if self.blending is not None else (None, None)
                targets = self.buf("soft_targets", (b, self.num_classes), f32)
                check(lib.mvf_soft_targets(_p(lab), _p(rows_d), _p(wts_d), b, self.num_classes, C.c_float(self.label_smooth_eps), _p(targets), _st()),
                      "soft_targets")
            check(lib.mvf_head_train_fwd_soft(_p(xcur), b, t, hc * wc, cc, _p(self.fc_w), _p(self.fc_b), self.num_classes, _p(targets), _p(mask), _p(pooled),
                                              _p(scores), _p(dscores), _p(loss_part), _p(loss), self.dt, _st()), "head fwd (soft targets)")
        else:
            check(lib.mvf_head_train_fwd(_p(xcur), b, t, hc * wc, cc, _p(self.fc_w), _p(self.fc_b), self.num_classes, _p(lab), _p(mask), _p(pooled),
                                         _p(scores), _p(dscores), _p(loss_part), _p(loss), self.dt, _st()), "head fwd")
        if teacher_scores is not None:
            terms = self._distill_terms = self.buf("distill_terms", (2,), f32)
            check(lib.mvf_distill_loss(_p(scores), _p(teacher_scores), b, self.num_classes, C.c_float(self.distill.temperature), C.c_float(self.distill.alpha),
                                       _p(dscores), _p(loss_part), _p(loss), _p(terms), _st()), "distill loss")
            self.saved.update(teacher_scores=teacher_scores)
        self.saved.update(pooled=pooled, dscores=dscores, mask=mask, hw=hc * wc, c=cc, feat_shape=xcur.shape, scores=scores)
        if self._nbt_touched:
            self._count_batches()
        return loss

    def distill_terms(self):
        if self._distill_terms is None:
            raise RuntimeError("distill_terms: no step has run with engine.distill set (train_cfg['distill'], distill.KnowledgeDistillation)")
        ce, kd = self._distill_terms.tolist()
        return dict(loss_ce=ce, loss_kd=kd)

    def _count_batches(self):
        key = tuple(m_.training for m_ in self._nbt_mods)
        if all(key):
            self._nbt_flat += 1
        else:
            if key not in self._nbt_inc:
                self._nbt_inc[key] = torch.tensor([int(k) for k in key] or [0], dtype=torch.int64, device=self.device)
            self._nbt_flat += self._nbt_inc[key]
        self._nbt_touched = False

    def backward(self, exchange=False):
        self._main = torch.cuda.current_stream()
        self._exchange = bool(exchange)
        with _on_stream(self._main, main=True):
            self._backward()

    def _backward(self):
        s = self.saved
        if getattr(self, "_packs_on_side", False):
            self._wait(self.main_stream(), self._side)
        nt, b, t = s["nt"], s["b"], s["t"]
        dpool = self.buf("dpool", (b, s["c"]), torch.float32)
        g = self.buf("gfeat", tuple(s["feat_shape"]))
        check(lib.mvf_head_train_bwd(_p(s["dscores"]), _p(s["pooled"]), _p(self.fc_w), _p(s["mask"]), b, t, s["hw"], s["c"], self.num_classes,
                                     _p(self.dfc_w), _p(self.dfc_b), _p(dpool), _p(g), self.dt, _st()), "head bwd")
        gated = sums = False
        for i in range(len(self.blocks) - 1, -1, -1):
            req = self.blocks[i - 1].wants_gated_gradient(self) if i > 0 else None
            g = self.blocks[i].backward(g, nt, self, g_gated=gated, gate=req, sums_done=sums)
            gated, sums = self.blocks[i].gated_out, self.blocks[i].sums_out
            if i == self._tail_block:
                self._launch_tail_allreduce()
        ho, wo = s["ho"], s["wo"]
        bn = self.stem_bn
        rows = lib.mvf_maxpool_bwd_sums_rows(nt, ho)
        part = self.buf("stem_bnsums", (64, rows, 2), torch.float32)
        check(lib.mvf_maxpool_bn_relu_bwd_sums(_p(s["amax"]), _p(g), nt, ho, wo, 64, None, _p(s["z0"]), _p(bn.mean), _p(bn.invstd),
                                               _p(bn.scale), _p(bn.shift), _p(part), self.dt, _st()), "maxpool bwd + bn sums")
        check(lib.mvf_bn_bwd_finalize(_p(part), rows, 64, _p(bn.dgamma), _p(bn.dbeta), _st()), "bn bwd finalize")
        dz0 = self.buf((id(bn), "dz"), s["z0"].shape, s["z0"].dtype)
        sg, sb = (bn._zero, bn._zero) if bn.frozen else (bn.dgamma, bn.dbeta)
        check(lib.mvf_maxpool_bn_relu_bwd_apply(_p(s["amax"]), _p(g), nt, ho, wo, 64, _p(s["z0"]), _p(bn.gamma), _p(bn.mean), _p(bn.invstd), _p(bn.scale),
                                                _p(bn.shift), _p(sg), _p(sb), _p(dz0), self.dt, _st()), "maxpool bwd + bn apply")
        self.flush_side()
        self.stem.wgrad(dz0, s["xp"], nt, s["hp"], s["wp"], ho, wo, self, on_main=True)
        self.join_side()
        if self.keep_io:
            self.io = dict(p0=self.buf("p0", (g.shape[0], 64)), g_p0=g, gfeat=self.buf("gfeat", tuple(s["feat_shape"])), nt=nt, b=b, t=t)
        self.saved = None

    exchange_enabled = True

    def _ddp_active(self):
        import torch.distributed as dist
        return self.exchange_enabled and dist.is_available() and dist.is_initialized() and (dist.get_world_size() > 1 or self.force_allreduce)

    overlap_allreduce = _policy("ddp_overlap", 1) != 0

    def _launch_tail_allreduce(self):
        self._tail_launched = False
        if not (getattr(self, "_exchange", False) and self.overlap_allreduce and self._tail_off and self._ddp_active() and self.overlap_wgrad):
            return
        import torch.distributed as dist
        side = self.side_stream()
        self.flush_side()
        if getattr(self, "_comm", None) is None:
            from .streams import concurrent_stream
            self._comm = concurrent_stream(self.main_stream(), avoid=[side])

        def exchange():
            comm = self._comm
            comm.wait_stream(side)
            comm.wait_stream(self.main_stream())
            with torch.cuda.stream(comm):
                dist.all_reduce(self.flat_grads[self._tail_off:])
            self._tail_launched = True
        if self._rec is not None:
            self._rec.py_op(exchange)
        else:
            exchange()

    def allreduce_grads(self):
        import torch.distributed as dist
        if not self._ddp_active():
            return 1
        if self._tail_launched:
            torch.cuda.current_stream().wait_stream(self._comm)
            dist.all_reduce(self.flat_grads[:self._tail_off])
            self._tail_launched = False
        else:
            dist.all_reduce(self.flat_grads)
        return dist.get_world_size()

    force_allreduce = False

    def step(self, lr=None):
        with _on_stream(torch.cuda.current_stream(), main=True):
            return self._step(lr)

    def _step(self, lr=None):
        world = self.allreduce_grads()
        if self.apply_sgd(lr, world) is None:
            return self.norm_out
        for m_ in (self.model.backbone, self.model.cls_head):
            if hasattr(m_, "invalidate_engine"):
                m_.invalidate_engine()
        return self.norm_out

    use_plan = _policy("plan", 1) != 0
    plan_warmup = 2

    def _plan_key(self, imgs, labels):
        if not (self.use_plan and imgs.dtype == torch.float32 and imgs.is_contiguous() and not self.keep_io and self.input_pipeline is None):
            return None
        if not all(m_.training for m_ in self._nbt_mods):
            return None
        if self.erasing is not None and getattr(self.erasing, "max_boxes", None) is None:
            return None
        if self.distill is not None:
            return None
        sw = self.__dict__.get("_switch_names")
        if sw is None:
            sw = self._switch_names = sorted(k for c_ in type(self).__mro__ for k, v in vars(c_).items()
                                             if not k.startswith("_") and isinstance(v, (bool, int, float, str)) and k not in ("lr", "momentum", "weight_decay", "max_norm"))
        return (tuple(imgs.shape), tuple(labels.shape), labels.dtype, str(imgs.device), torch.cuda.current_stream().cuda_stream, self._ddp_active(),
                self.dropout > 0.0, tuple(p.requires_grad for p in self.model.parameters()), tuple(getattr(self, k) for k in sw),
                self.blending is not None, float(self.label_smooth_eps), self._soft_labels(imgs, labels)) + (
                    (("erasing", int(self.erasing.max_boxes)),) if self.erasing is not None else ())

    def _record_step(self, imgs, labels, prepared):
        from . import launch_plan
        import sys
        mod = sys.modules[__name__]
        rec = launch_plan.Recorder()
        allocs0 = torch.cuda.memory_stats(imgs.device).get("allocation.all.allocated", 0)
        real_lib, self._rec = mod.lib, rec
        mod.lib = launch_plan.RecordingLib(rec)
        try:
            loss = self.forward(imgs, labels, _prepared=prepared)
            self.backward(exchange=True)
        finally:
            mod.lib, self._rec = real_lib, None
        if torch.cuda.memory_stats(imgs.device).get("allocation.all.allocated", 0) != allocs0:
            rec.unsupported = "the step allocates device memory"
        if rec.unsupported:
            return loss, None
        lab, mask, _ = prepared
        plan = launch_plan.Plan(rec, dict(imgs=imgs.data_ptr(), labels=lab.data_ptr(), mask=mask.data_ptr() if mask is not None else 0, loss=loss.data_ptr()))
        plan.storage_epoch = self._storage_epoch
        return loss, plan

    def train_step(self, imgs, labels, lr=None):
        loss = self._forward_backward(imgs, labels, exchange=True)
        self.step(lr)
        return loss

    def _forward_backward(self, imgs, labels, exchange):
        if self.randaug is not None:
            self._randaug_refusals(imgs)
        if self.distill is not None:
            self._distill_refusals()
        if self._ema_swapped:
            self._ema_live("a training step")
        if self._guard is not None:
            self._guard_snapshot()
        key = self._plan_key(imgs, labels) if imgs.is_cuda else None
        if not exchange and self._ddp_active():
            key = None
        if key is None:
            loss = self.forward(imgs, labels)
            self.backward(exchange=exchange)
        else:
            loss = self._planned_forward_backward(imgs, labels, key)
        if self._train_acc is not None:
            self._count_train_accuracy(imgs, labels)
        return loss

    def _planned_forward_backward(self, imgs, labels, key):
        st = self.__dict__.setdefault("_plans", {}).setdefault(key, dict(eager=0, tries=0, cand=None, plan=None))
        prepared = self._step_tensors(imgs, labels)
        plan = st["plan"]
        if plan is not None and plan.storage_epoch != self._storage_epoch:
            plan = st["plan"] = st["cand"] = None
            st["tries"] = 0
        if plan is not None:
            lab, mask, loss = prepared
            self._main = torch.cuda.current_stream()
            self.forward_count += 1
            self._exchange = True
            self._count_batches()
            plan.run(dict(imgs=imgs.data_ptr(), labels=lab.data_ptr(), mask=mask.data_ptr() if mask is not None else 0, loss=loss.data_ptr()))
        elif st["eager"] < self.plan_warmup or st["tries"] >= 4:
            st["eager"] += 1
            loss = self.forward(imgs, labels, _prepared=prepared)
            self.backward(exchange=True)
        else:
            st["tries"] += 1
            loss, cand = self._record_step(imgs, labels, prepared)
# ... 323 lines not shown
```

Before: 1787 clips/s.

## Compute stem BN backward sums from pooled tensors; add fused stem wgrad+BN apply

```diff
diff --git a/include/mvfnet_hip.h b/include/mvfnet_hip.h
--- a/include/mvfnet_hip.h
+++ b/include/mvfnet_hip.h
@@ -230,6 +230,15 @@
                                   const float* dbeta, void* dz, int dtype, void* stream);
 int mvf_maxpool_bn_relu_bwd_sums(const unsigned char* argmax, const void* g, int n, int h, int w, int c, void* ga, const void* z, const float* mean,
                                  const float* invstd, const float* scale, const float* shift, float* sums_part, int dtype, void* stream);
+int mvf_maxpool_bwd_sums_pooled_rows(int n, int h, int w, int c, int dtype);
+int mvf_maxpool_bn_relu_fwd_pz(const void* z, int n, int h, int w, int c, const float* scale, const float* shift, void* y, unsigned char* argmax, void* pz, int dtype,
+                               void* stream);
+int mvf_maxpool_bn_relu_bwd_sums_pooled(const void* g, const void* pz, int n, int h, int w, int c, const float* mean, const float* invstd, const float* scale,
+                                        const float* shift, float* sums_part, int dtype, void* stream);
+size_t mvf_stem_wgrad_bnapply_workspace_bytes(int n, int h, int w, int ho, int wo, int c, int dtype);
+int mvf_stem_wgrad_bnapply(const unsigned char* argmax, const void* g, const void* z, const void* x, int n, int h, int w, int ho, int wo, int c, const float* gamma,
+                           const float* mean, const float* invstd, const float* scale, const float* shift, const float* dgamma, const float* dbeta, float* dw_oihw,
+                           void* ws, size_t ws_bytes, int dtype, void* stream);
 int mvf_head_train_fwd(const void* feat, int clips, int t, int hw, int c, const float* fc_w, const float* fc_b, int classes,
                        const long long* labels, const float* drop_mask ,
                        float* pooled, float* scores, float* dscores, float* loss_part, float* loss, int dtype, void* stream);
diff --git a/mvfnet_amd/_lib.py b/mvfnet_amd/_lib.py
--- a/mvfnet_amd/_lib.py
+++ b/mvfnet_amd/_lib.py
@@ -204,6 +204,16 @@
     lib.mvf_maxpool_bn_relu_bwd_apply.argtypes = [vp, vp, i32, i32, i32, i32, vp, fp, fp, fp, fp, fp, fp, fp, vp, i32, vp]
     lib.mvf_maxpool_bn_relu_bwd_sums.restype = i32
     lib.mvf_maxpool_bn_relu_bwd_sums.argtypes = [vp, vp, i32, i32, i32, i32, vp, vp, fp, fp, fp, fp, fp, i32, vp]
+    lib.mvf_maxpool_bwd_sums_pooled_rows.restype = i32
+    lib.mvf_maxpool_bwd_sums_pooled_rows.argtypes = [i32, i32, i32, i32, i32]
+    lib.mvf_maxpool_bn_relu_fwd_pz.restype = i32
+    lib.mvf_maxpool_bn_relu_fwd_pz.argtypes = [vp, i32, i32, i32, i32, fp, fp, vp, vp, vp, i32, vp]
+    lib.mvf_maxpool_bn_relu_bwd_sums_pooled.restype = i32
+    lib.mvf_maxpool_bn_relu_bwd_sums_pooled.argtypes = [vp, vp, i32, i32, i32, i32, fp, fp, fp, fp, fp, i32, vp]
+    lib.mvf_stem_wgrad_bnapply_workspace_bytes.restype = sz
+    lib.mvf_stem_wgrad_bnapply_workspace_bytes.argtypes = [i32, i32, i32, i32, i32, i32, i32]
+    lib.mvf_stem_wgrad_bnapply.restype = i32
+    lib.mvf_stem_wgrad_bnapply.argtypes = [vp, vp, vp, vp, i32, i32, i32, i32, i32, i32, fp, fp, fp, fp, fp, fp, fp, fp, vp, sz, i32, vp]
     lib.mvf_head_train_fwd.restype = i32
     lib.mvf_head_train_fwd.argtypes = [vp, i32, i32, i32, i32, fp, fp, i32, ll, fp, fp, fp, fp, fp, fp, i32, vp]
     lib.mvf_conv2d_nhwc_fwd_mvf.restype = i32
diff --git a/mvfnet_amd/csrc/common.h b/mvfnet_amd/csrc/common.h
--- a/mvfnet_amd/csrc/common.h
+++ b/mvfnet_amd/csrc/common.h
@@ -154,6 +154,11 @@
     float* part;
     int N, H, W, Ho, Wo, nwg;
 };
+struct WgradStemBnArgs {
+    const unsigned char* amax;
+    const void* g;
+    const float *gamma, *mean, *invstd, *scale, *shift, *dgamma, *dbeta;
+};
 namespace mvf_internal {
 struct BnBwdWgradArgs {
     const void* g;
@@ -204,6 +209,8 @@
 bool wgrad_stem_ok(int n, int h, int w, int ho, int wo);
 int wgrad_stem_wgs(int n, int ho);
 int wgrad_stem_launch(const WgradStemArgs& a, hipStream_t st);
+bool wgrad_stem_bn_ok(int n, int h, int w, int ho, int wo);
+int wgrad_stem_bn_launch(const WgradStemArgs& a, const WgradStemBnArgs* bn, hipStream_t st);
 int stem_direct_launch(const StemDirectArgs& a, hipStream_t st);
 int conv3x3_c64_launch(const Conv3x3C64Args& a, hipStream_t st);
 int pw_sums_launch(const PwSumsArgs& a, hipStream_t st);
diff --git a/mvfnet_amd/csrc/train_ops.hip b/mvfnet_amd/csrc/train_ops.hip
--- a/mvfnet_amd/csrc/train_ops.hip
+++ b/mvfnet_amd/csrc/train_ops.hip
@@ -742,6 +742,143 @@
                     *reinterpret_cast<unsigned*>(amax + oidx) = am[0] | (am[1] << 8) | (am[2] << 16) | (am[3] << 24);
             }
         }
+    }
+}
+
+template <typename ET>
+__global__ __launch_bounds__(256) void maxpool_bn_fwd_blk_pz_kernel(const ET* z, int n, int h, int w, int c, int ho, int wo, const float* scale,
+                                                                    const float* shift, ET* y, unsigned char* amax, ET* pz) {
+    constexpr int VC = 16 / (int)sizeof(ET);
+    const int ncg = c / VC, bwn = wo >> 1, bhn = ho >> 1;
+    const long total = (long)n * bhn * bwn * ncg;
+    for (long i = (long)blockIdx.x * blockDim.x + threadIdx.x; i < total; i += (long)gridDim.x * blockDim.x) {
+        const int cq = (int)(i % ncg);
+        long t = i / ncg;
+        const int bw = (int)(t % bwn); t /= bwn;
+        const int bh = (int)(t % bhn);
+        const int img = (int)(t / bhn);
+        float sc[VC], sh[VC];
+#pragma unroll
+        for (int j = 0; j < VC; ++j) { sc[j] = scale[cq * VC + j]; sh[j] = shift[cq * VC + j]; }
+        uint4 u[5][5];
+#pragma unroll
+        for (int r = 0; r < 5; ++r)
+#pragma unroll
+            for (int q = 0; q < 5; ++q) {
+                const int ih = 4 * bh - 1 + r, iw = 4 * bw - 1 + q;
+                const int ihc = min(max(ih, 0), h - 1), iwc = min(max(iw, 0), w - 1);
+                u[r][q] = *reinterpret_cast<const uint4*>(z + (((long)img * h + ihc) * w + iwc) * c + cq * VC);
+            }
+#pragma unroll
+        for (int p = 0; p < 4; ++p) {
+            const int oh = 2 * bh + (p >> 1), ow = 2 * bw + (p & 1);
+            float m[VC], zf[VC];
+            unsigned am[VC];
+#pragma unroll
+            for (int j = 0; j < VC; ++j) { m[j] = -INFINITY; am[j] = 0; zf[j] = 0.f; }
+#pragma unroll
+            for (int k = 0; k < 9; ++k) {
+                const int r = 2 * (p >> 1) + k / 3, q = 2 * (p & 1) + k % 3;
+                const int ih = oh * 2 - 1 + k / 3, iw = ow * 2 - 1 + k % 3;
+                const bool in = (unsigned)ih < (unsigned)h && (unsigned)iw < (unsigned)w;
+                const uint4 v = u[r][q];
+                float f[VC];
+                if constexpr (sizeof(ET) == 4) {
+                    f[0] = __uint_as_float(v.x); f[1] = __uint_as_float(v.y); f[2] = __uint_as_float(v.z); f[3] = __uint_as_float(v.w);
+                } else {
+                    f[0] = __uint_as_float(v.x << 16); f[1] = __uint_as_float(v.x & 0xffff0000u); f[2] = __uint_as_float(v.y << 16); f[3] = __uint_as_float(v.y & 0xffff0000u);
+                    f[4] = __uint_as_float(v.z << 16); f[5] = __uint_as_float(v.z & 0xffff0000u); f[6] = __uint_as_float(v.w << 16); f[7] = __uint_as_float(v.w & 0xffff0000u);
+                }
+#pragma unroll
+                for (int j = 0; j < VC; ++j) {
+                    const float act = fmaxf(f[j] * sc[j] + sh[j], 0.f);
+                    if (k == 0) zf[j] = f[j];
+                    if (in && act > m[j]) { m[j] = act; am[j] = k; zf[j] = f[j]; }
+                }
+            }
+            const long oidx = (((long)img * ho + oh) * wo + ow) * c + cq * VC;
+            uint4 uy, uz;
+            if constexpr (sizeof(ET) == 4) {
+                uy = make_uint4(__float_as_uint(m[0]), __float_as_uint(m[1]), __float_as_uint(m[2]), __float_as_uint(m[3]));
+                uz = make_uint4(__float_as_uint(zf[0]), __float_as_uint(zf[1]), __float_as_uint(zf[2]), __float_as_uint(zf[3]));
+            } else {
+                uy = make_uint4(pack_bf16x2(m[0], m[1]), pack_bf16x2(m[2], m[3]), pack_bf16x2(m[4], m[5]), pack_bf16x2(m[6], m[7]));
+                uz = make_uint4((__float_as_uint(zf[0]) >> 16) | (__float_as_uint(zf[1]) & 0xffff0000u), (__float_as_uint(zf[2]) >> 16) | (__float_as_uint(zf[3]) & 0xffff0000u),
+                                (__float_as_uint(zf[4]) >> 16) | (__float_as_uint(zf[5]) & 0xffff0000u), (__float_as_uint(zf[6]) >> 16) | (__float_as_uint(zf[7]) & 0xffff0000u));
+            }
+            *reinterpret_cast<uint4*>(y + oidx) = uy;
+            *reinterpret_cast<uint4*>(pz + oidx) = uz;
+            if constexpr (VC == 8)
+                *reinterpret_cast<uint2*>(amax + oidx) = make_uint2(am[0] | (am[1] << 8) | (am[2] << 16) | (am[3] << 24), am[4] | (am[5] << 8) | (am[6] << 16) | (am[7] << 24));
+            else
+                *reinterpret_cast<unsigned*>(amax + oidx) = am[0] | (am[1] << 8) | (am[2] << 16) | (am[3] << 24);
+        }
+    }
+}
+
+constexpr int kPoolSumRows = 512;
+template <typename ET>
+__global__ __launch_bounds__(256) void maxpool_bn_bwd_pooled_sums_kernel(const ET* g, const ET* pz, long m, int c, const float* mean, const float* invstd,
+                                                                         const float* scale, const float* shift, float* part, int nblk) {
+    constexpr int VC = 16 / (int)sizeof(ET);
+    __shared__ float red[256 * 2 * VC];
+    const int ncg = c / VC, rl = 256 / ncg;
+    const int cq = threadIdx.x % ncg, lr = threadIdx.x / ncg;
+    float scv[VC], shv[VC], muv[VC], rsv[VC], s1[VC], s2[VC];
+#pragma unroll
+    for (int j = 0; j < VC; ++j) {
+        const int ch = cq * VC + j;
+        scv[j] = scale[ch]; shv[j] = shift[ch]; muv[j] = mean[ch]; rsv[j] = invstd[ch];
+        s1[j] = 0.f; s2[j] = 0.f;
+    }
+    auto ldv = [](const ET* p, float (&f)[VC]) {
+        const uint4 u = *reinterpret_cast<const uint4*>(p);
+        if constexpr (sizeof(ET) == 4) {
+            f[0] = __uint_as_float(u.x); f[1] = __uint_as_float(u.y); f[2] = __uint_as_float(u.z); f[3] = __uint_as_float(u.w);
+        } else {
+            f[0] = __uint_as_float(u.x << 16); f[1] = __uint_as_float(u.x & 0xffff0000u); f[2] = __uint_as_float(u.y << 16); f[3] = __uint_as_float(u.y & 0xffff0000u);
+            f[4] = __uint_as_float(u.z << 16); f[5] = __uint_as_float(u.z & 0xffff0000u); f[6] = __uint_as_float(u.w << 16); f[7] = __uint_as_float(u.w & 0xffff0000u);
+        }
+    };
+    auto add = [&](const float (&gv)[VC], const float (&zv)[VC]) {
+#pragma unroll
+        for (int j = 0; j < VC; ++j) {
+            const float gm = (zv[j] * scv[j] + shv[j]) > 0.f ? gv[j] : 0.f;
+            s1[j] += gm;
+            s2[j] += gm * ((zv[j] - muv[j]) * rsv[j]);
+        }
+    };
+    const long r0 = (long)blockIdx.x * kPoolSumRows, r1 = min(m, r0 + kPoolSumRows);
+    long row = r0 + lr;
+    for (; row + rl < r1; row += 2 * rl) {
+        float g0[VC], z0[VC], g1[VC], z1[VC];
+        ldv(g + row * c + cq * VC, g0);
+        ldv(pz + row * c + cq * VC, z0);
+        ldv(g + (row + rl) * c + cq * VC, g1);
+        ldv(pz + (row + rl) * c + cq * VC, z1);
+        add(g0, z0);
+        add(g1, z1);
+    }
+    for (; row < r1; row += rl) {
+        float g0[VC], z0[VC];
+        ldv(g + row * c + cq * VC, g0);
+        ldv(pz + row * c + cq * VC, z0);
+        add(g0, z0);
+    }
+#pragma unroll
+    for (int j = 0; j < VC; ++j) {
+        red[(2 * j) * 256 + threadIdx.x] = s1[j];
+        red[(2 * j + 1) * 256 + threadIdx.x] = s2[j];
+    }
+    __syncthreads();
+    if ((int)threadIdx.x < c) {
+        const int q = threadIdx.x / VC, j = threadIdx.x - q * VC;
+        float a = 0.f, b = 0.f;
+        for (int t = q; t < 256; t += ncg) {
+            a += red[(2 * j) * 256 + t];
+            b += red[(2 * j + 1) * 256 + t];
+        }
+        reinterpret_cast<float2*>(part)[(long)threadIdx.x * nblk + blockIdx.x] = make_float2(a, b);
     }
 }
 
@@ -1870,6 +2007,53 @@
     return MVF_OK;
 }
 
+static bool pool_pz_ok(int n, int h, int w, int c, int dtype) {
+    static const int on = mvf_policy_int("pool_fwd_block", 1);
+    const int vc = dtype == MVF_F32 ? 4 : 8;
+    return on && (dtype == MVF_F32 || dtype == MVF_BF16) && n > 0 && h > 0 && w > 0 && c > 0 && h % 4 == 0 && w % 4 == 0 && c % vc == 0 && 256 % (c / vc) == 0 && c <= 256;
+}
+
+int mvf_maxpool_bwd_sums_pooled_rows(int n, int h, int w, int c, int dtype) {
+    if (!pool_pz_ok(n, h, w, c, dtype)) return 0;
+    const long rows = ((long)n * (h / 2) * (w / 2) + kPoolSumRows - 1) / kPoolSumRows;
+    return rows < (1L << 31) ? (int)rows : 0;
+}
+
+int mvf_maxpool_bn_relu_fwd_pz(const void* z, int n, int h, int w, int c, const float* scale, const float* shift, void* y, unsigned char* argmax, void* pz, int dtype,
+                               void* stream) {
+    MVF_REQUIRE(z && y && argmax && pz && scale && shift && n > 0 && h > 0 && w > 0 && c > 0 && c % 4 == 0, MVF_EINVAL, "maxpool_bn_relu_fwd_pz: bad argument");
+    MVF_REQUIRE(pool_pz_ok(n, h, w, c, dtype) && ((uintptr_t)z | (uintptr_t)y | (uintptr_t)pz) % 16 == 0 && (uintptr_t)argmax % 8 == 0, MVF_EUNSUPPORTED,
+                "maxpool_bn_relu_fwd_pz: needs h, w multiples of 4 and 16-byte channel groups that divide 256 (n=%d h=%d w=%d c=%d): use mvf_maxpool_bn_relu_fwd", n, h, w, c);
+    const int ho = h / 2, wo = w / 2, vc = dtype == MVF_F32 ? 4 : 8;
+    const long tb = (long)n * (ho / 2) * (wo / 2) * (c / vc);
+    if (dtype == MVF_F32)
+        hipLaunchKernelGGL(maxpool_bn_fwd_blk_pz_kernel<float>, dim3(grid_for(tb, 256 * 8)), dim3(256), 0, (hipStream_t)stream, (const float*)z, n, h, w, c, ho, wo, scale, shift,
+                           (float*)y, argmax, (float*)pz);
+    else
+        hipLaunchKernelGGL(maxpool_bn_fwd_blk_pz_kernel<bf16_t>, dim3(grid_for(tb, 256 * 8)), dim3(256), 0, (hipStream_t)stream, (const bf16_t*)z, n, h, w, c, ho, wo, scale, shift,
+                           (bf16_t*)y, argmax, (bf16_t*)pz);
+    MVF_LAUNCH_CHECK();
+    return MVF_OK;
+}
+
+int mvf_maxpool_bn_relu_bwd_sums_pooled(const void* g, const void* pz, int n, int h, int w, int c, const float* mean, const float* invstd, const float* scale,
+                                        const float* shift, float* sums_part, int dtype, void* stream) {
+    MVF_REQUIRE(g && pz && mean && invstd && scale && shift && sums_part && n > 0 && h > 0 && w > 0 && c > 0, MVF_EINVAL, "maxpool_bn_relu_bwd_sums_pooled: bad argument");
+    const int nblk = mvf_maxpool_bwd_sums_pooled_rows(n, h, w, c, dtype);
+    MVF_REQUIRE(nblk > 0 && ((uintptr_t)g | (uintptr_t)pz) % 16 == 0, MVF_EUNSUPPORTED,
+                "maxpool_bn_relu_bwd_sums_pooled: needs h, w multiples of 4 and 16-byte channel groups that divide 256 (n=%d h=%d w=%d c=%d): use mvf_maxpool_bn_relu_bwd_sums",
+                n, h, w, c);
+    const long m = (long)n * (h / 2) * (w / 2);
+    if (dtype == MVF_F32)
+        hipLaunchKernelGGL(maxpool_bn_bwd_pooled_sums_kernel<float>, dim3(nblk), dim3(256), 0, (hipStream_t)stream, (const float*)g, (const float*)pz, m, c, mean, invstd, scale,
+                           shift, sums_part, nblk);
+    else
+        hipLaunchKernelGGL(maxpool_bn_bwd_pooled_sums_kernel<bf16_t>, dim3(nblk), dim3(256), 0, (hipStream_t)stream, (const bf16_t*)g, (const bf16_t*)pz, m, c, mean, invstd,
+                           scale, shift, sums_part, nblk);
+    MVF_LAUNCH_CHECK();
+    return MVF_OK;
+}
+
 int mvf_maxpool_bn_relu_bwd(const unsigned char* argmax, const void* g, int n, int h, int w, int c, void* ga, int dtype, void* stream) {
     MVF_REQUIRE(argmax && g && ga && n > 0 && h > 0 && w > 0 && c > 0 && c % 4 == 0, MVF_EINVAL, "maxpool_bn_relu_bwd: bad argument");
     const int ho = (h - 1) / 2 + 1, wo = (w - 1) / 2 + 1;
diff --git a/mvfnet_amd/csrc/wgrad_nhwc.hip b/mvfnet_amd/csrc/wgrad_nhwc.hip
--- a/mvfnet_amd/csrc/wgrad_nhwc.hip
+++ b/mvfnet_amd/csrc/wgrad_nhwc.hip
@@ -1311,6 +1311,33 @@
     return wgrad_impl(d, dz, x, x2, kw_real, cin_real, kw_packed, cin_packed, dw_oihw, ws, ws_bytes, stream, wgs);
 }
 
+static bool stem_bnapply_ok(int n, int h, int w, int ho, int wo, int c, int dtype) {
+    static const int pool_blk = mvf_policy_int("pool_bwd_block", 1);
+    return dtype == MVF_BF16 && c == 64 && pool_blk && n > 0 && mvf_internal::wgrad_stem_bn_ok(n, h, w, ho, wo);
+}
+
+size_t mvf_stem_wgrad_bnapply_workspace_bytes(int n, int h, int w, int ho, int wo, int c, int dtype) {
+    if (!stem_bnapply_ok(n, h, w, ho, wo, c, dtype)) return 0;
+    return align_up((size_t)mvf_internal::wgrad_stem_wgs(n, ho) * 64 * 224 * sizeof(float), 256);
+}
+
+int mvf_stem_wgrad_bnapply(const unsigned char* argmax, const void* g, const void* z, const void* x, int n, int h, int w, int ho, int wo, int c, const float* gamma,
+                           const float* mean, const float* invstd, const float* scale, const float* shift, const float* dgamma, const float* dbeta, float* dw_oihw,
+                           void* ws, size_t ws_bytes, int dtype, void* stream) {
+    MVF_REQUIRE(argmax && g && z && x && gamma && mean && invstd && scale && shift && dgamma && dbeta && dw_oihw && n > 0 && h > 0 && w > 0 && ho > 0 && wo > 0 && c > 0,
+                MVF_EINVAL, "stem_wgrad_bnapply: bad argument");
+    MVF_REQUIRE(stem_bnapply_ok(n, h, w, ho, wo, c, dtype), MVF_EUNSUPPORTED,
+                "stem_wgrad_bnapply: bf16, 64 channels, even ho, wo %% 16 == 0 (n=%d h=%d w=%d ho=%d wo=%d c=%d): use mvf_maxpool_bn_relu_bwd_apply + mvf_conv2d_nhwc_wgrad",
+                n, h, w, ho, wo, c);
+    MVF_REQUIRE(((uintptr_t)g | (uintptr_t)z | (uintptr_t)x) % 16 == 0 && (uintptr_t)argmax % 8 == 0, MVF_EUNSUPPORTED, "stem_wgrad_bnapply: 16-byte aligned tensors");
+    MVF_REQUIRE(ws && ws_bytes >= mvf_stem_wgrad_bnapply_workspace_bytes(n, h, w, ho, wo, c, dtype), MVF_EWS, "stem_wgrad_bnapply: workspace too small");
+    const WgradStemArgs a = {z, x, (float*)ws, n, h, w, ho, wo, mvf_internal::wgrad_stem_wgs(n, ho)};
+    const WgradStemBnArgs b = {argmax, g, gamma, mean, invstd, scale, shift, dgamma, dbeta};
+    const int rc = mvf_internal::wgrad_stem_bn_launch(a, &b, (hipStream_t)stream);
+    if (rc != MVF_OK) return rc;
+    return launch_wgrad_reduce((const float*)ws, a.nwg, 64, 3, 7, 7, 8, 4, dw_oihw, (hipStream_t)stream);
+}
+
 int mvf_conv2d_wgrad_last_launch(mvf_wgrad_launch_info_t* out) {
     MVF_REQUIRE(out, MVF_EINVAL, "conv2d_wgrad_last_launch: NULL argument");
     *out = t_last_wgrad;
diff --git a/mvfnet_amd/csrc/wgrad_stem.hip b/mvfnet_amd/csrc/wgrad_stem.hip
--- a/mvfnet_amd/csrc/wgrad_stem.hip
+++ b/mvfnet_amd/csrc/wgrad_stem.hip
@@ -23,8 +23,16 @@
 __device__ __forceinline__ int fdiv(int n, unsigned mul, unsigned shr) { return (int)((__umulhi((unsigned)n, mul) + (unsigned)n) >> shr); }
 __device__ __forceinline__ int swzf(int pixel) { return ((pixel >> 1) & 1) << 2; }
 
-template <int kR>
-__global__ __launch_bounds__(256, 2) void wgrad_stem_kernel(KArgs a) {
+struct BnArgs {
+    const unsigned char* amax;
+    const char* g;
+    const float *gamma, *mean, *invstd, *scale, *shift, *dgamma, *dbeta;
+    float inv_m;
+};
+constexpr int kBnCoefBytes = 6 * 64 * 4;
+
+template <int kR, bool kBN>
+__device__ __forceinline__ void wgrad_stem_body(const KArgs& a, const BnArgs& q) {
     extern __shared__ __attribute__((aligned(16))) char smem[];
     char* Xs = smem;
     char* Ds = smem + (a.xbytes + 1023) / 1024 * 1024;
@@ -61,6 +69,78 @@
 #pragma unroll
         for (int r = 0; r < 16; ++r) acc[t][r] = 0.f;
 
+    float* Cs = reinterpret_cast<float*>(Ds + a.dpix * 128);
+    const int ho2 = a.Ho >> 1, wo2 = a.Wo >> 1, items = wo2 * 8;
+    auto gather_win = [&](int i, int img, int bh, int arow, uint4 (&ga)[4]) {
+        const int cq = i & 7, bw = i >> 3;
+        const bool ok[4] = {true, bw + 1 < wo2, bh + 1 < ho2, bh + 1 < ho2 && bw + 1 < wo2};
+        uint2 am[4];
+        uint4 gw[4];
+#pragma unroll
+        for (int k = 0; k < 4; ++k) {
+            const long oidx = (((long)img * ho2 + min(bh + (k >> 1), ho2 - 1)) * wo2 + min(bw + (k & 1), wo2 - 1)) * 64 + cq * 8;
+            am[k] = *reinterpret_cast<const uint2*>(q.amax + oidx);
+            gw[k] = *reinterpret_cast<const uint4*>(q.g + oidx * 2);
+        }
+#pragma unroll
+        for (int p = 0; p < 4; ++p) {
+            const int pa = p >> 1, pb = p & 1;
+            if (kR == 1 && pa != arow) continue;
+            float acc[8] = {0.f, 0.f, 0.f, 0.f, 0.f, 0.f, 0.f, 0.f};
+#pragma unroll
+            for (int k = 0; k < 4; ++k) {
+                const int wi = k >> 1, wj = k & 1;
+                if ((wi == 1 && pa == 0) || (wj == 1 && pb == 0)) continue;
+                const unsigned me = (unsigned)(pa + 1 - 2 * wi) * 3u + (unsigned)(pb + 1 - 2 * wj);
+                const unsigned gwd[4] = {gw[k].x, gw[k].y, gw[k].z, gw[k].w};
+#pragma unroll
+                for (int j = 0; j < 8; ++j) {
+                    const unsigned amb = ((j < 4 ? am[k].x : am[k].y) >> (8 * (j & 3))) & 255u;
+                    const float gv = __uint_as_float((j & 1) ? (gwd[j >> 1] & 0xffff0000u) : (gwd[j >> 1] << 16));
+                    if (ok[k] && amb == me) acc[j] += gv;
+                }
+            }
+            ga[p] = make_uint4(pack_bf16x2(acc[0], acc[1]), pack_bf16x2(acc[2], acc[3]), pack_bf16x2(acc[4], acc[5]), pack_bf16x2(acc[6], acc[7]));
+        }
+    };
+    auto apply_win = [&](int i, int arow, const uint4 (&ga)[4]) {
+        const int cq = i & 7, bw = i >> 3;
+#pragma unroll
+        for (int jh = 0; jh < 2; ++jh) {
+            const float* cf = Cs + cq * 8 + jh * 4;
+            const float4 sc = *reinterpret_cast<const float4*>(cf), sh = *reinterpret_cast<const float4*>(cf + 64), mu = *reinterpret_cast<const float4*>(cf + 128);
+            const float4 c1 = *reinterpret_cast<const float4*>(cf + 192), c2 = *reinterpret_cast<const float4*>(cf + 256), c3 = *reinterpret_cast<const float4*>(cf + 320);
+            const float scv[4] = {sc.x, sc.y, sc.z, sc.w}, shv[4] = {sh.x, sh.y, sh.z, sh.w}, muv[4] = {mu.x, mu.y, mu.z, mu.w};
+            const float k1[4] = {c1.x, c1.y, c1.z, c1.w}, k2[4] = {c2.x, c2.y, c2.z, c2.w}, k3[4] = {c3.x, c3.y, c3.z, c3.w};
+#pragma unroll
+            for (int p = 0; p < 4; ++p) {
+                const int pa = p >> 1, pb = p & 1;
+                if (kR == 1 && pa != arow) continue;
+                const int P = (kR == 2 ? pa * a.Wo : 0) + 2 * bw + pb;
+                uint2* zp = reinterpret_cast<uint2*>(Ds + P * 128 + ((cq ^ swzf(P)) << 4) + jh * 8);
+                const uint2 zr = *zp;
+                const float zv[4] = {__uint_as_float(zr.x << 16), __uint_as_float(zr.x & 0xffff0000u), __uint_as_float(zr.y << 16), __uint_as_float(zr.y & 0xffff0000u)};
+                const unsigned g01 = jh ? ga[p].z : ga[p].x, g23 = jh ? ga[p].w : ga[p].y;
+                const float acc[4] = {__uint_as_float(g01 << 16), __uint_as_float(g01 & 0xffff0000u), __uint_as_float(g23 << 16), __uint_as_float(g23 & 0xffff0000u)};
+                float o[4];
+#pragma unroll
+                for (int j = 0; j < 4; ++j) {
+                    const float gm = (zv[j] * scv[j] + shv[j]) > 0.f ? acc[j] : 0.f;
+                    o[j] = k1[j] * (gm - k2[j] - (zv[j] - muv[j]) * k3[j]);
+                }
+                *zp = make_uint2(pack_bf16x2(o[0], o[1]), pack_bf16x2(o[2], o[3]));
+            }
+        }
+    };
+    if constexpr (kBN) {
+        if (tid < 64) {
+            Cs[tid] = q.scale[tid]; Cs[64 + tid] = q.shift[tid]; Cs[128 + tid] = q.mean[tid];
+            Cs[192 + tid] = q.gamma[tid] * q.invstd[tid];
+            Cs[256 + tid] = q.dbeta[tid] * q.inv_m;
+            Cs[320 + tid] = q.invstd[tid] * q.dgamma[tid] * q.inv_m;
+        }
+    }
+
     const int nks = a.dpix >> 4;
     for (int b = blockIdx.x; b < a.bands; b += gridDim.x) {
         const int img = fdiv(b, a.fd_bpf_mul, a.fd_bpf_shr);
@@ -78,8 +158,23 @@
                 glds16(gs_d, lds_d + (unsigned)(i * 1024), (unsigned)(dbase + p * 128 + ((lu ^ swzf(p)) << 4)));
             }
         }
+        uint4 ga0[4], ga1[4];
+        const int bh = oh0 >> 1, arow = oh0 & 1;
+        if constexpr (kBN) {
+            if (tid < items) gather_win(tid, img, bh, arow, ga0);
+            if (tid + 256 < items) gather_win(tid + 256, img, bh, arow, ga1);
+        }
         asm volatile("s_waitcnt vmcnt(0)" ::: "memory");
         __syncthreads();
+        if constexpr (kBN) {
+            if (tid < items) apply_win(tid, arow, ga0);
+            if (tid + 256 < items) apply_win(tid + 256, arow, ga1);
+            for (int i = tid + 512; i < items; i += 256) {
+                gather_win(i, img, bh, arow, ga0);
+                apply_win(i, arow, ga0);
+            }
+            __syncthreads();
+        }
         for (int ks = 0; ks < nks; ++ks) {
             const int r = fdiv(ks, a.fd_ksr_mul, a.fd_ksr_shr), ow0 = (ks - r * a.ksr) * 16;
             const bf16x8_t fa = gather(Ds + ks * 2048 + offA, Ds + ks * 2048 + offA + 4 * 128);
@@ -110,6 +205,16 @@
     }
 }
 
+template <int kR>
+__global__ __launch_bounds__(256, 2) void wgrad_stem_kernel(KArgs a) {
+    wgrad_stem_body<kR, false>(a, BnArgs{});
+}
+
+template <int kR>
+__global__ __launch_bounds__(256, 3) void wgrad_stem_bn_kernel(KArgs a, BnArgs q) {
+    wgrad_stem_body<kR, true>(a, q);
+}
+
 inline void fd_make(unsigned d, unsigned& mul, unsigned& shr) {
     unsigned l = 0;
     while ((1ull << l) < d) ++l;
@@ -138,7 +243,13 @@
     return (int)std::min<long>(env, (long)n * (ho / band_rows()));
 }
 
-int wgrad_stem_launch(const WgradStemArgs& w, hipStream_t st) {
+bool wgrad_stem_bn_ok(int n, int h, int w, int ho, int wo) {
+    return wgrad_stem_ok(n, h, w, ho, wo) && (2 * 2 + 5) * w * 8 + 1024 + 2 * wo * 128 + kBnCoefBytes <= 72 * 1024;
+}
+
+int wgrad_stem_launch(const WgradStemArgs& w, hipStream_t st) { return wgrad_stem_bn_launch(w, nullptr, st); }
+
+int wgrad_stem_bn_launch(const WgradStemArgs& w, const WgradStemBnArgs* bn, hipStream_t st) {
     KArgs a = {};
     a.dz = (const char*)w.dz; a.x = (const char*)w.x; a.part = w.part;
     a.N = w.N; a.H = w.H; a.W = w.W; a.Ho = w.Ho; a.Wo = w.Wo;
@@ -156,9 +267,16 @@
     if (!attr) {
         MVF_HIP_OK(hipFuncSetAttribute((const void*)wgrad_stem_kernel<1>, hipFuncAttributeMaxDynamicSharedMemorySize, 72 * 1024));
         MVF_HIP_OK(hipFuncSetAttribute((const void*)wgrad_stem_kernel<2>, hipFuncAttributeMaxDynamicSharedMemorySize, 72 * 1024));
+        MVF_HIP_OK(hipFuncSetAttribute((const void*)wgrad_stem_bn_kernel<1>, hipFuncAttributeMaxDynamicSharedMemorySize, 72 * 1024));
+        MVF_HIP_OK(hipFuncSetAttribute((const void*)wgrad_stem_bn_kernel<2>, hipFuncAttributeMaxDynamicSharedMemorySize, 72 * 1024));
         attr = true;
     }
-    if (kR == 1) hipLaunchKernelGGL(wgrad_stem_kernel<1>, dim3(w.nwg), dim3(256), lds, st, a);
+    if (bn) {
+        const BnArgs q = {bn->amax, (const char*)bn->g, bn->gamma, bn->mean, bn->invstd, bn->scale, bn->shift, bn->dgamma, bn->dbeta,
+                          1.0f / (float)((long)w.N * w.Ho * w.Wo)};
+        if (kR == 1) hipLaunchKernelGGL(wgrad_stem_bn_kernel<1>, dim3(w.nwg), dim3(256), lds + kBnCoefBytes, st, a, q);
+        else hipLaunchKernelGGL(wgrad_stem_bn_kernel<2>, dim3(w.nwg), dim3(256), lds + kBnCoefBytes, st, a, q);
+    } else if (kR == 1) hipLaunchKernelGGL(wgrad_stem_kernel<1>, dim3(w.nwg), dim3(256), lds, st, a);
     else hipLaunchKernelGGL(wgrad_stem_kernel<2>, dim3(w.nwg), dim3(256), lds, st, a);
     MVF_LAUNCH_CHECK();
     return MVF_OK;
diff --git a/mvfnet_amd/train_engine.py b/mvfnet_amd/train_engine.py
--- a/mvfnet_amd/train_engine.py
+++ b/mvfnet_amd/train_engine.py
@@ -993,6 +993,7 @@
     pair_ds_sums = _policy("pair_ds_sums", 3)
     z3_free_ds = _policy("z3_free_ds", 1)
     fuse_c3_bwd = _policy("fuse_c3_bwd", 1)
+    stem_bwd_fused = _policy("stem_bwd_fused", 2)
     fuse_mvf_stats = _policy("fuse_mvf_stats", 1) != 0
     dzfree = _policy("dzfree", 2)
     gate_producer = _policy("gate_producer", 1) != 0
@@ -1812,8 +1813,15 @@
         h2, w2 = (ho - 1) // 2 + 1, (wo - 1) // 2 + 1
         p0 = self.buf("p0", (nt * h2 * w2, 64))
         amax = self.buf("amax", (nt * h2 * w2, 64), torch.uint8)
-        check(lib.mvf_maxpool_bn_relu_fwd(_p(z0), nt, ho, wo, 64, _p(self.stem_bn.scale), _p(self.stem_bn.shift), _p(p0), _p(amax), self.dt, _st()), "maxpool fwd")
-        self.saved = dict(xp=xp, z0=z0, amax=amax, nt=nt, hp=hp, wp=wp, ho=ho, wo=wo, t=t, b=b)
+        fused = self._stem_bwd_fused(nt, hp, wp, ho, wo)
+        pz0 = None
+        if fused & 2:
+            pz0 = self.buf("pz0", (nt * h2 * w2, 64))
+            check(lib.mvf_maxpool_bn_relu_fwd_pz(_p(z0), nt, ho, wo, 64, _p(self.stem_bn.scale), _p(self.stem_bn.shift), _p(p0), _p(amax), _p(pz0), self.dt, _st()),
+                  "maxpool fwd + pz0")
+        else:
+            check(lib.mvf_maxpool_bn_relu_fwd(_p(z0), nt, ho, wo, 64, _p(self.stem_bn.scale), _p(self.stem_bn.shift), _p(p0), _p(amax), self.dt, _st()), "maxpool fwd")
+        self.saved = dict(xp=xp, z0=z0, amax=amax, nt=nt, hp=hp, wp=wp, ho=ho, wo=wo, t=t, b=b, pz0=pz0, stem_fused=fused)
         if stages is not None:
             stages["maxpool"] = p0.view(nt, h2, w2, 64)
         xcur, hc, wc, cc = p0, h2, w2, 64
@@ -1876,6 +1884,16 @@
         with _on_stream(self._main, main=True):
             self._backward()
 
+    def _stem_bwd_fused(self, nt, hp, wp, ho, wo):
+        f, bn = int(self.stem_bwd_fused), self.stem_bn
+        if not f or self.tdtype != torch.bfloat16 or bn.frozen or not (self.stem.w.requires_grad and bn.gamma.requires_grad and bn.beta.requires_grad):
+            return 0
+        if (f & 1) and not lib.mvf_stem_wgrad_bnapply_workspace_bytes(nt, hp, wp, ho, wo, 64, self.dt):
+            f &= ~1
+        if (f & 2) and not lib.mvf_maxpool_bwd_sums_pooled_rows(nt, ho, wo, 64, self.dt):
+            f &= ~2
+        return f & 3
+
     def _backward(self):
         s = self.saved
         if getattr(self, "_packs_on_side", False):
@@ -1894,17 +1912,31 @@
                 self._launch_tail_allreduce()
         ho, wo = s["ho"], s["wo"]
         bn = self.stem_bn
-        rows = lib.mvf_maxpool_bwd_sums_rows(nt, ho)
-        part = self.buf("stem_bnsums", (64, rows, 2), torch.float32)
-        check(lib.mvf_maxpool_bn_relu_bwd_sums(_p(s["amax"]), _p(g), nt, ho, wo, 64, None, _p(s["z0"]), _p(bn.mean), _p(bn.invstd),
-                                               _p(bn.scale), _p(bn.shift), _p(part), self.dt, _st()), "maxpool bwd + bn sums")
+        fused = s.get("stem_fused", 0)
+        if fused & 2:
+            rows = lib.mvf_maxpool_bwd_sums_pooled_rows(nt, ho, wo, 64, self.dt)
+            part = self.buf("stem_bnsums_pooled", (64, rows, 2), torch.float32)
+            check(lib.mvf_maxpool_bn_relu_bwd_sums_pooled(_p(g), _p(s["pz0"]), nt, ho, wo, 64, _p(bn.mean), _p(bn.invstd), _p(bn.scale), _p(bn.shift), _p(part),
+                                                          self.dt, _st()), "maxpool bwd: bn sums from pooled tensors")
+        else:
+            rows = lib.mvf_maxpool_bwd_sums_rows(nt, ho)
+            part = self.buf("stem_bnsums", (64, rows, 2), torch.float32)
+            check(lib.mvf_maxpool_bn_relu_bwd_sums(_p(s["amax"]), _p(g), nt, ho, wo, 64, None, _p(s["z0"]), _p(bn.mean), _p(bn.invstd),
+                                                   _p(bn.scale), _p(bn.shift), _p(part), self.dt, _st()), "maxpool bwd + bn sums")
         check(lib.mvf_bn_bwd_finalize(_p(part), rows, 64, _p(bn.dgamma), _p(bn.dbeta), _st()), "bn bwd finalize")
-        dz0 = self.buf((id(bn), "dz"), s["z0"].shape, s["z0"].dtype)
-        sg, sb = (bn._zero, bn._zero) if bn.frozen else (bn.dgamma, bn.dbeta)
-        check(lib.mvf_maxpool_bn_relu_bwd_apply(_p(s["amax"]), _p(g), nt, ho, wo, 64, _p(s["z0"]), _p(bn.gamma), _p(bn.mean), _p(bn.invstd), _p(bn.scale),
-                                                _p(bn.shift), _p(sg), _p(sb), _p(dz0), self.dt, _st()), "maxpool bwd + bn apply")
-        self.flush_side()
-        self.stem.wgrad(dz0, s["xp"], nt, s["hp"], s["wp"], ho, wo, self, on_main=True)
+        if fused & 1:
+            self.flush_side()
+            ws = self.workspace(lib.mvf_stem_wgrad_bnapply_workspace_bytes(nt, s["hp"], s["wp"], ho, wo, 64, self.dt))
+            check(lib.mvf_stem_wgrad_bnapply(_p(s["amax"]), _p(g), _p(s["z0"]), _p(s["xp"]), nt, s["hp"], s["wp"], ho, wo, 64, _p(bn.gamma), _p(bn.mean), _p(bn.invstd),
+                                             _p(bn.scale), _p(bn.shift), _p(bn.dgamma), _p(bn.dbeta), _p(self.stem.dw), _p(ws), ws.numel(), self.dt, _st()),
+                  "stem wgrad + bn apply")
+        else:
+            dz0 = self.buf((id(bn), "dz"), s["z0"].shape, s["z0"].dtype)
+            sg, sb = (bn._zero, bn._zero) if bn.frozen else (bn.dgamma, bn.dbeta)
+            check(lib.mvf_maxpool_bn_relu_bwd_apply(_p(s["amax"]), _p(g), nt, ho, wo, 64, _p(s["z0"]), _p(bn.gamma), _p(bn.mean), _p(bn.invstd), _p(bn.scale),
+                                                    _p(bn.shift), _p(sg), _p(sb), _p(dz0), self.dt, _st()), "maxpool bwd + bn apply")
+            self.flush_side()
+            self.stem.wgrad(dz0, s["xp"], nt, s["hp"], s["wp"], ho, wo, self, on_main=True)
         self.join_side()
         if self.keep_io:
             self.io = dict(p0=self.buf("p0", (g.shape[0], 64)), g_p0=g, gfeat=self.buf("gfeat", tuple(s["feat_shape"])), nt=nt, b=b, t=t)
```

After: 1790 clips/s (median of 6 runs). No clear change (+0.2%).
